# akashsengupta1997/STRAPS-3DHumanShapePose

Measured on AMD Instinct MI355X. Metric: bodies/sec, higher is better.
Workload: dtype fp32 (encoder convolutions as exact bf16x3 operand splits (six bf16 products per term); in-step SMPL blend contraction and skinning as 3-product fp16 splits (fp16x3_lbs: 22-bit operands); fp32 accumulate throughout)

## Files before the change

include/straps_hip.h:

```cpp
#ifndef STRAPS_HIP_H
#define STRAPS_HIP_H

#include <stddef.h>
#include <stdint.h>

#ifdef __cplusplus
extern "C" {
#endif

#define STRAPS_ABI_VERSION 12

#define STRAPS_OK 0
#define STRAPS_EINVAL 1
#define STRAPS_EHIP 2
#define STRAPS_EUNSUPPORTED 3

int straps_abi_version(void);
int straps_selftest_mfma_peak(const float* seed512, float* out, int blocks, int iters, void* stream);
int straps_selftest_mfma_bf16(float* out, unsigned long long* clk2, int blocks, int iters, void* stream);
int straps_selftest_mfma_bf16_dense(float* out, unsigned long long* clk2, int blocks, int iters, int data, void* stream);
const char* straps_last_error(void);
int straps_device_count(void);
int straps_wall_clock_khz(void);
int straps_set_clock_accumulator(unsigned long long* acc2);
// ... 85 lines not shown
#define STRAPS_SMPL_V 6890
#define STRAPS_SMPL_VPAD 6912
#define STRAPS_SMPL_TILES 216
#define STRAPS_SMPL_KP 224
#define STRAPS_SMPL_NJ 24
#define STRAPS_SMPL_NEXTRA 45
#define STRAPS_SMPL_NPICK 21
#define STRAPS_SMPL_NJOINTS_OUT 90

typedef struct {
    const float* blend_frag;
    const float* j_template;
    const float* j_shapedirs;
    const int32_t* parents;
    const int32_t* depth;
    int32_t max_depth;
    int32_t skin_k;
    const float* skin_w;
    const int32_t* skin_j;
    const int32_t* vj_ptr;
    int32_t n_tiles;
    int32_t reserved0;
    const int32_t* pick_ids;
    const float* blend_frag_t;
    const int32_t* children;
    const int32_t* jrt_ptr;
    const int32_t* jrt_code;
    const float* jrt_w;
    const int32_t* dj_ptr;
    const int32_t* dj_code;
    const float* dj_w;
    const void* blend_frag_h;
    float blend_h_unscale;
    int32_t reserved1;
    const void* skin_frag_p;
} straps_smpl_model_t;

#define STRAPS_SMPL_KERNEL_WIDE 0x100
#define STRAPS_SMPL_KERNEL_NARROW 0x200
#define STRAPS_SMPL_KERNEL_WIDE_BUILTIN 0x400
#define STRAPS_SMPL_EXACT_F32 0
#define STRAPS_SMPL_SPLIT_F16 1
#define STRAPS_SMPL_SPLIT_F16_LBS 2
#define STRAPS_SMPL_SPLIT_F16_LBS_PD16 3
#define STRAPS_SMPL_SPLIT_F16_LBS_P16 4

size_t straps_smpl_workspace_bytes(const straps_smpl_model_t* model, long long batch);
int straps_smpl_fwd(const straps_smpl_model_t* model, const float* betas, const float* rotmats,
                    float* verts, float* joints, void* workspace, long long batch, int chunks, int mode,
                    void* stream);

size_t straps_smpl_bwd_workspace_bytes(long long batch, int chunks);
int straps_smpl_bwd(const straps_smpl_model_t* model, const float* betas, const float* rotmats,
                    const float* dverts, const float* djoints, float* dbetas, float* drotmats,
                    void* workspace, long long batch, int chunks, void* stream);
int straps_smpl_bwd_aa(const straps_smpl_model_t* model, const float* betas, const float* rotmats,
                       const float* full_pose_aa, const float* dverts, const float* djoints, float* dbetas,
                       float* dfull_pose_aa, float* drotmats, void* workspace, long long batch, int chunks,
                       void* stream);

int straps_conv_dgrad(const float* dy_nhwc, const float* w_crsk, const float* addend,
                      float* dx_nhwc, int batch, int h, int w, int cin, int cout, int kh, int kw,
                      int stride, int pad, int tile_cfg, void* stream);

int straps_split3_bf16(const float* x, unsigned short* planes, long long n, long long plane_stride,
                       void* stream);
int straps_split3_bf16_cm(const float* x, unsigned short* planes, long long rows, int c,
                          long long plane_stride, void* stream);
int straps_conv_x3_stat_blocks(int batch, int h, int w, int cin, int cout, int kh, int kw, int stride,
                               int pad, int tile_cfg);

int straps_conv_x3f_supported(int cin, int cout, int kh, int kw, int stride, int pad);
int straps_conv_fwd_x3f(const float* x, const float* a_scale, const float* a_shift, int a_relu, const unsigned short* w3,
                        long long w_plane_stride, const float* scale, const float* shift, const float* residual, int relu,
                        float* y, float* stats_partial, int batch, int h, int w, int cin, int cout, int kh, int kw, int stride,
                        int pad, int tile_cfg, void* stream);
int straps_conv_x3f_stat_blocks(int batch, int h, int w, int cin, int cout, int kh, int kw, int stride, int pad, int tile_cfg);
int straps_conv_dgrad_x3f(const float* dy, const unsigned short* w3_crsk, long long w_plane_stride, const float* addend,
                          const unsigned* addend_bits, float* dx, int batch, int h, int w, int cin, int cout, int kh, int kw,
                          int stride, int pad, int tile_cfg, const float* bn_raw, const unsigned* bn_out_bits,
                          const float* bn_mask_scale, const float* bn_mask_shift, const float* bn_mean, const float* bn_invstd,
                          double* bn_partials, void* stream);
int straps_conv_dgrad_x3f_bn_blocks(int batch, int h, int w, int cin, int cout, int kh, int kw, int stride, int pad, int tile_cfg);
size_t straps_conv_wgrad_x3f_workspace_bytes(int batch, int h, int w, int cin, int cout, int kh, int kw, int stride, int pad);
int straps_conv_wgrad_x3f(const float* x, const float* a_scale, const float* a_shift, int a_relu, const float* dy, float* dw_oihw,
                          void* workspace, int batch, int h, int w, int cin, int cout, int kh, int kw, int stride, int pad,
                          int accumulate, void* stream);
int straps_conv_fwd_x3(const unsigned short* x3, long long x_plane_stride,
                       const unsigned short* w3_krsc, long long w_plane_stride, const float* scale,
                       const float* shift, const float* residual, int relu, float* y_nhwc,
                       float* stats_partial, int batch, int h, int w, int cin, int cout, int kh,
                       int kw, int stride, int pad, int tile_cfg, void* stream);
int straps_conv_fwd_x3p(const unsigned short* x3, long long x_plane_stride,
                        const unsigned short* w3_krsc, long long w_plane_stride, const float* scale,
                        const float* shift, const float* residual, int relu, float* y_nhwc,
                        unsigned short* y_planes, long long y_plane_stride, int batch, int h, int w,
                        int cin, int cout, int kh, int kw, int stride, int pad, int tile_cfg, void* stream);
int straps_split_bf16_cm(const float* x, unsigned short* plane, long long rows, int c, void* stream);
int straps_pack_conv_weight_bf16(const float* w_oihw, unsigned short* w_plane, int cout, int cin, int kh, int kw, void* stream);
int straps_conv_bf16_tile_choice(int batch, int h, int w, int cin, int cout, int kh, int kw, int stride, int pad);
int straps_conv_fwd_bf16(const unsigned short* x1, const unsigned short* w1_krsc, const float* scale, const float* shift,
                         const float* residual, int relu, float* y_nhwc, unsigned short* y_plane, int batch, int h, int w,
                         int cin, int cout, int kh, int kw, int stride, int pad, int tile_cfg, void* stream);
int straps_conv_dgrad_x3(const unsigned short* dy3, long long dy_plane_stride,
                         const unsigned short* w3_crsk, long long w_plane_stride,
                         const float* addend, float* dx_nhwc, int batch, int h, int w, int cin,
                         int cout, int kh, int kw, int stride, int pad, int tile_cfg, void* stream);
int straps_bn_apply_x3(const float* raw, const float* scale, const float* shift, const float* residual,
                       int relu, float* y, unsigned short* y_planes, long long plane_stride,
                       long long rows, int c, void* stream);
int straps_bn_relu_maxpool_fwd_x3(const float* raw, const float* scale, const float* shift,
                                  float* y_pool, uint8_t* idx, unsigned short* y_planes,
                                  long long plane_stride, int batch, int h, int w, int c, void* stream);
int straps_bn_bwd_x3(const float* dy, const float* yact, const float* raw, const float* save_mean,
                     const float* save_invstd, const float* gamma, const float* mask_scale,
                     const float* mask_shift, float* dgamma, float* dbeta, float* draw, float* dz_out,
                     unsigned short* draw_planes, long long plane_stride, void* workspace,
                     long long rows, int c, int accumulate, void* stream);
int straps_conv_dgrad_x3_bn_blocks(int batch, int h, int w, int cin, int cout, int kh, int kw, int stride,
                                   int pad, int tile_cfg);
int straps_conv_dgrad_x3_bn(const unsigned short* dy3, long long dy_plane_stride,
                            const unsigned short* w3_crsk, long long w_plane_stride, const float* addend,
                            float* dx_nhwc, int batch, int h, int w, int cin, int cout, int kh, int kw,
                            int stride, int pad, int tile_cfg, const float* bn_raw, const float* bn_out,
                            const float* bn_mask_scale, const float* bn_mask_shift, const float* bn_mean,
                            const float* bn_invstd, double* bn_partials, void* stream);
int straps_bn_bwd_finish_x3(const float* dy, const float* yact, const float* raw, const float* save_mean,
                            const float* save_invstd, const float* gamma, const float* mask_scale,
                            const float* mask_shift, float* dgamma, float* dbeta, float* draw, float* dz_out,
                            unsigned short* draw_planes, long long plane_stride, const double* partials,
                            int nblk, void* workspace, long long rows, int c, int accumulate, void* stream);
int straps_bn_apply_bits_x3(const float* raw, const float* scale, const float* shift, const float* residual, float* y,
                            unsigned short* y_planes, long long plane_stride, unsigned* relu_bits, long long rows,
                            int c, void* stream);
int straps_bn_bwd_bits_x3(const float* dy, const unsigned* relu_bits, const float* raw, const float* save_mean,
                          const float* save_invstd, const float* gamma, float* dgamma, float* dbeta, float* draw,
                          unsigned short* draw_planes, long long plane_stride, void* workspace, long long rows, int c,
                          int accumulate, void* stream);
int straps_bn_bwd_finish_bits_x3(const float* dy, const unsigned* relu_bits, const float* raw, const float* save_mean,
                                 const float* save_invstd, const float* gamma, float* dgamma, float* dbeta, float* draw,
                                 unsigned short* draw_planes, long long plane_stride, const double* partials, int nblk,
                                 void* workspace, long long rows, int c, int accumulate, void* stream);
int straps_conv_dgrad_x3_bits(const unsigned short* dy3, long long dy_plane_stride, const unsigned short* w3_crsk,
                              long long w_plane_stride, const float* addend, float* dx_nhwc, int batch, int h, int w,
                              int cin, int cout, int kh, int kw, int stride, int pad, int tile_cfg,
                              const unsigned* addend_bits, void* stream);
int straps_conv_dgrad_x3_bn_bits(const unsigned short* dy3, long long dy_plane_stride,
                                 const unsigned short* w3_crsk, long long w_plane_stride, const float* addend,
                                 float* dx_nhwc, int batch, int h, int w, int cin, int cout, int kh, int kw,
                                 int stride, int pad, int tile_cfg, const float* bn_raw, const float* bn_out,
                                 const float* bn_mask_scale, const float* bn_mask_shift, const float* bn_mean,
                                 const float* bn_invstd, double* bn_partials, const unsigned* addend_bits,
                                 const unsigned* bn_out_bits, void* stream);
int straps_conv_wgrad_x3_on_planes(int batch, int h, int w, int cin, int cout, int kh, int kw,
                                   int stride, int pad);
int straps_conv_wgrad_x3(const float* x_nhwc, const float* dy_nhwc, const unsigned short* x3,
                         long long x_plane_stride, const unsigned short* dy3, long long dy_plane_stride,
                         float* dw_oihw, void* workspace, int batch, int h, int w, int cin, int cout,
                         int kh, int kw, int stride, int pad, int accumulate, void* stream);


size_t straps_conv_wgrad_workspace_bytes(int batch, int h, int w, int cin, int cout, int kh,
                                         int kw, int stride, int pad);
int straps_conv_wgrad(const float* x_nhwc, const float* dy_nhwc, float* dw_oihw, void* workspace,
                      int batch, int h, int w, int cin, int cout, int kh, int kw, int stride,
                      int pad, int accumulate, void* stream);
size_t straps_stem_wgrad_workspace_bytes(int batch, int cin, int h, int w);
int straps_stem_wgrad(const float* x_nchw, const float* dy_nhwc, float* dw_oihw, void* workspace,
                      const uint32_t* nzmask , int batch, int cin,
                      int h, int w, int accumulate, void* stream);
#define STRAPS_STEM_DGRAD_MAX_CIN 64
size_t straps_stem_dgrad_weight_floats(int cin);
int straps_pack_stem_dgrad_weight(const float* w_oihw, float* w_pk, int cin, void* stream);
int straps_stem_dgrad(const float* dy_nhwc, const float* w_pk, float* dx_nchw, int batch, int cin, int h, int w,
                      int accumulate, void* stream);
int straps_bn_bwd_blocks(long long rows, int c);
size_t straps_bn_bwd_workspace_bytes(long long rows, int c);
int straps_bn_bwd(const float* dy, const float* yact, const float* raw, const float* save_mean,
                  const float* save_invstd, const float* gamma, const float* mask_scale,
                  const float* mask_shift, float* dgamma, float* dbeta, float* draw, float* dz_out,
                  void* workspace, long long rows, int c, int accumulate, void* stream);
int straps_bn_relu_maxpool_fwd(const float* raw_nhwc, const float* scale, const float* shift,
                               float* y_pool_nhwc, uint8_t* idx, int batch, int h, int w, int c,
                               void* stream);
int straps_bn_bwd_pooled(const float* dy_pool_nhwc, const uint8_t* idx, const float* raw,
                         const float* save_mean, const float* save_invstd, const float* gamma,
                         const float* mask_scale, const float* mask_shift, float* dgamma, float* dbeta,
                         float* draw, void* workspace, int batch, int h, int w, int c, int accumulate,
                         void* stream);
size_t straps_stem_tiles(int batch, int in_h, int in_w);
int straps_stem_tile_activity(const uint32_t* nzmask, uint8_t* tile_active, int batch, int cin, int in_h,
                              int in_w, void* stream);
int straps_bn_bwd_pooled_sparse(const float* dy_pool_nhwc, const uint8_t* idx, const float* raw,
                                const float* save_mean, const float* save_invstd, const float* gamma,
                                const float* mask_scale, const float* mask_shift, float* dgamma,
                                float* dbeta, float* draw, void* workspace, int batch, int h, int w, int c,
                                int accumulate, const uint8_t* tile_active, void* stream);
int straps_maxpool_fwd_idx(const float* x_nhwc, float* y_nhwc, uint8_t* idx, int batch, int h,
                           int w, int c, void* stream);
int straps_maxpool_bwd(const float* dy_nhwc, const uint8_t* idx, float* dx_nhwc, int batch, int h,
                       int w, int c, void* stream);
int straps_gap_bwd(const float* dfeat, float* dx_nhwc, int batch, int hw, int c, void* stream);
int straps_masked_copy(const float* x, int ldx, const float* mask, int ldmask, float* y, int ldy,
                       int m, int n, int accumulate, void* stream);
int straps_rot6d_bwd(const float* x6, long long ld, int per_row, const float* drot, float* dx6,
                     long long ldd, long long rows, void* stream);

int straps_build_proxy_input(const float* seg, const float* joints2d, float* out_nchw, int batch,
                             int nj, int wh, void* stream);
int straps_build_proxy_input_std(const float* seg, const float* joints2d, float* out_nchw, int batch,
                                 int nj, int wh, int std, void* stream);
int straps_build_proxy_input_nz(const float* seg, const float* joints2d, float* out_nchw, uint32_t* nzmask,
                                int batch, int nj, int wh, int std, void* stream);
size_t straps_loss_workspace_bytes(long long batch);
int straps_loss_fwd_bwd(const float* pred_verts, const float* pred_joints, const float* est,
                        int ld_est, const float* pred_rot, const float* tgt_verts,
                        const float* tgt_joints2d, const float* tgt_joints3d,
                        const float* tgt_shape, const float* tgt_rot, const float* log_vars,
                        float* loss_out, float* dverts, float* djoints, float* dest, float* drot,
                        float* dlogvar, void* workspace, long long batch, int img_wh, void* stream);
int straps_loss_fwd_bwd_gm(const float* pred_verts, const float* pred_joints, const float* est, int ld_est,
                           const float* pred_rot, const float* tgt_verts, const float* tgt_joints2d,
                           const float* tgt_joints3d, const float* tgt_shape, const float* tgt_rot,
                           const float* log_vars, float* loss_out, float* dverts, float* djoints, float* dest,
                           float* drot, float* dlogvar, void* workspace, long long batch, int img_wh,
                           const float* j2d_count_global, float count_scale, void* stream);
int straps_count_visible(const float* tgt_joints2d, float* out_count, long long batch, int nj, int img_wh,
                         void* stream);
int straps_mse_fwd(const float* pred, const float* tgt, const uint8_t* row_mask, long long rows,
                   int cols, float tgt_scale, float tgt_shift, float* out3, void* workspace,
                   void* stream);
int straps_mse_bwd(const float* pred, const float* tgt, const uint8_t* row_mask, long long rows,
                   int cols, float tgt_scale, float tgt_shift, const float* coef, float* grad,
                   void* stream);
int straps_augment_seg(const float* seg, const float* uniforms, const float* remove_prob,
                       float occlude_prob, int box_dim, float* out, int batch, int wh, void* stream);
int straps_philox_fill(unsigned long long seed, const long long* step_dev, long long step_host,
                       unsigned substream, float* out, long long n, int kind, void* stream);
int straps_counter_add(long long* counters, int n, long long delta, void* stream);
int straps_gather_f32(const float* src, const int* index, float* dst, int n, void* stream);
int straps_memset_zero(void* ptr, size_t bytes, void* stream);
int straps_augment_smpl(const float* pose_rows, long long n_rows, const float* u_index,
                        const float* orig_shape, const float* mean_shape, const float* shape_draws,
                        int shape_mode, const float* std_vector, double range_lo, double range_hi,
                        float* out_shape, float* out_rotmats, float* out_pose, long long batch,
                        void* stream);
int straps_augment_cam_t(const float* mean_cam_t, const float* normals_xy, const float* uniform_z,
                         double xy_std, double z_lo, double z_hi, float* out_cam_t, long long batch,
                         void* stream);
int straps_deviate_joints2d(const float* joints2d, const float* uniforms, double lo, double hi,
                            double hip_lo, double hip_hi, float* out, long long batch, void* stream);
int straps_deviate_verts2d(const float* verts, const float* uniforms, double lo, double hi, float* out,
                           long long nverts_total, void* stream);
int straps_project_targets(const float* joints, const float* cam_t, float fx, float fy, float cx,
                           float cy, float* joints2d, float* joints3d, long long batch, void* stream);
size_t straps_rasterize_workspace_bytes(long long batch, int nverts, int wh);
int straps_rasterize_parts(const float* verts, const int32_t* faces, const uint8_t* face_parts,
                           const float* cam_K, const float* cam_R, const float* cam_t, float* parts,
                           float* depth, void* workspace, long long batch, int nverts, int nfaces, int wh,
                           int cam_per_body, float near, float far, const float* vert_noise_u, double noise_lo,
                           double noise_hi, void* stream);
int straps_crop_resize(const float* seg, const float* joints2d, const float* uniforms,
                       double orig_scale_factor, double delta_scale_lo, double delta_scale_hi,
                       double delta_centre_lo, double delta_centre_hi, float* out_seg,
                       float* out_joints2d, int* boxes, int batch, int wh, int out_wh, int nj,
                       void* stream);
int straps_point_metrics(const float* pred, const float* target, float* out3, long long batch,
                         int npoints, void* stream);
int straps_adam_step(float* params, const float* grads, float* exp_avg, float* exp_avg_sq,
                     long long n, int step, float lr, float beta1, float beta2, float eps,
                     float grad_scale, const long long* step_dev, void* stream);

typedef struct {
    int layers;
    int in_channels;
    int ief_iters;
    int precision;
} straps_regressor_desc_t;
size_t straps_regressor_param_floats(const straps_regressor_desc_t* desc);
size_t straps_regressor_prepared_bytes(const straps_regressor_desc_t* desc);
int straps_regressor_prepare(const straps_regressor_desc_t* desc, const float* params, void* prepared, void* stream);
size_t straps_regressor_workspace_bytes(const straps_regressor_desc_t* desc, int batch, int h, int w);
int straps_regressor_fwd_infer(const straps_regressor_desc_t* desc, const void* prepared, const float* x, int batch, int h, int w,
                               float* est, int ld_est, float* rotmats, void* workspace, size_t workspace_bytes, void* stream);

size_t straps_regressor_train_param_floats(const straps_regressor_desc_t* desc);
size_t straps_regressor_bn_state_floats(const straps_regressor_desc_t* desc);
size_t straps_regressor_train_workspace_bytes(const straps_regressor_desc_t* desc, int batch, int h, int w);
int straps_regressor_fwd_train(const straps_regressor_desc_t* desc, const float* params, float* bn_state, const float* init_est,
                               const float* x, int batch, int h, int w, float* est, int ld_est,
                               void* workspace, size_t workspace_bytes, void* stream);
int straps_regressor_bwd(const straps_regressor_desc_t* desc, const float* params, const float* x, int batch, int h, int w,
                         const float* dest, int ld_dest, float* grads, float* dx,
                         void* workspace, size_t workspace_bytes, void* stream);
int straps_regressor_export_infer_params(const straps_regressor_desc_t* desc, const float* params, const float* bn_state,
                                         const float* init_est, float* infer_params, void* stream);

#define STRAPS_COMM_ID_BYTES 128
int straps_comm_unique_id(void* id128);
int straps_comm_init_rank(const void* id128, int nranks, int rank, void** comm);
int straps_comm_destroy(void* comm);
int straps_comm_size(void* comm);
const char* straps_comm_library(void);
int straps_allreduce_grads(float* flat_g, long long n, void* comm, void* stream);

#ifdef __cplusplus
// ... 4 lines not shown
```

straps-3dhumanshapepose_amd/autograd_ops.py:

```python
import ctypes as C

import torch

from . import hipabi
from .encoder_exec import encoder_forward
from .ief_module import EST_LD


def _empty_like(t):
    return torch.empty_like(t, memory_format=torch.contiguous_format)


class GradSink(dict):

    def __init__(self, views=None):
        super().__init__()
        self.views = views

    def buf(self, p, zero=False):
        if self.views is not None and p in self.views:
            return self.views[p]
        return torch.zeros_like(p) if zero else torch.empty_like(p)


class _SideStream:

    def __init__(self, stream):
        self.s, self.keep = stream, []

    def run(self, fn, *tensors):
        if self.s is None:
            return fn()
        self.keep.extend(tensors)
        self.s.wait_stream(torch.cuda.current_stream())
        with torch.cuda.stream(self.s):
            return fn()

    def join(self):
        if self.s is not None:
            torch.cuda.current_stream().wait_stream(self.s)
            self.keep.clear()


_FUSE_BN_SUMS = True
_SPARSE_STEM_TAIL = True


def _packed_dgrad_weight(net, conv):
    w = conv.weight

    def make():
        wd = w.detach().contiguous()
        out = torch.empty(wd.numel(), device=wd.device, dtype=torch.float32)
        hipabi.check(hipabi.lib().straps_pack_conv_weight_dgrad(hipabi.ptr(wd), hipabi.ptr(out), wd.shape[0], wd.shape[1], wd.shape[2],
                                                                wd.shape[3], hipabi.stream_ptr()), 'straps_pack_conv_weight_dgrad')
        return out
    return net._cached(('wd', id(conv)), [w], make)


def _bn_bwd(L, rec, dy, masked, want_dz, grads, planes_sink=None, keep_fp32=True, mask_bits=None):
    bn = rec['bn']
    raw, ss = rec['raw'], rec['stats']
    rows, Cc = raw.numel() // raw.shape[-1], raw.shape[-1]
    ws = torch.empty(L.straps_bn_bwd_workspace_bytes(rows, Cc) // 4, device=raw.device, dtype=torch.float32)
    dgamma, dbeta = grads.buf(bn.weight), grads.buf(bn.bias)
    keep_fp32 = keep_fp32 or planes_sink is None
    draw = _empty_like(raw) if keep_fp32 else raw.new_empty(0)
    dz = _empty_like(raw) if want_dz else None
    from_raw = masked and rec.get('residual') is None
    bits = mask_bits if mask_bits is not None else (rec.get('bits') if masked and not from_raw else None)
    if bits is not None and want_dz:
        raise RuntimeError('BatchNorm backward on ReLU bits writes no masked gradient (dz)')
    planes, ps = None, 0
    if planes_sink is not None:
        ps = (raw.numel() + 7) // 8 * 8
        planes = torch.empty(3, ps, device=raw.device, dtype=torch.int16)
        planes_sink[id(draw)] = (draw, planes, ps)
    flags = 2 if rec.get('frozen') else 0
    fused = rec.pop('bwd_partials', None)
    if bits is not None:
        args = (hipabi.ptr(dy), hipabi.ptr(bits), hipabi.ptr(raw), hipabi.ptr(ss[2]), hipabi.ptr(ss[3]), hipabi.ptr(bn.weight), hipabi.ptr(dgamma),
                hipabi.ptr(dbeta), hipabi.ptr(draw if keep_fp32 else None), hipabi.ptr(planes), ps)
        if fused is not None and fused[2] is dy and masked:
            hipabi.check(L.straps_bn_bwd_finish_bits_x3(*args, hipabi.ptr(fused[0]), fused[1], hipabi.ptr(ws), rows, Cc, flags, hipabi.stream_ptr()),
                         'straps_bn_bwd_finish_bits_x3')
        else:
            hipabi.check(L.straps_bn_bwd_bits_x3(*args, hipabi.ptr(ws), rows, Cc, flags, hipabi.stream_ptr()), 'straps_bn_bwd_bits_x3')
    elif fused is not None and fused[2] is dy and masked:
        hipabi.check(L.straps_bn_bwd_finish_x3(hipabi.ptr(dy), hipabi.ptr(rec['out'] if not from_raw else None), hipabi.ptr(raw), hipabi.ptr(ss[2]),
                                               hipabi.ptr(ss[3]), hipabi.ptr(bn.weight), hipabi.ptr(ss[0] if from_raw else None),
                                               hipabi.ptr(ss[1] if from_raw else None), hipabi.ptr(dgamma), hipabi.ptr(dbeta),
                                               hipabi.ptr(draw if keep_fp32 else None), hipabi.ptr(dz), hipabi.ptr(planes), ps, hipabi.ptr(fused[0]),
                                               fused[1], hipabi.ptr(ws), rows, Cc, flags, hipabi.stream_ptr()), 'straps_bn_bwd_finish_x3')
    else:
        hipabi.check(L.straps_bn_bwd_x3(hipabi.ptr(dy), hipabi.ptr(rec['out'] if masked and not from_raw else None), hipabi.ptr(raw), hipabi.ptr(ss[2]),
                                        hipabi.ptr(ss[3]), hipabi.ptr(bn.weight), hipabi.ptr(ss[0] if from_raw else None),
                                        hipabi.ptr(ss[1] if from_raw else None), hipabi.ptr(dgamma), hipabi.ptr(dbeta), hipabi.ptr(draw if keep_fp32 else None),
                                        hipabi.ptr(dz), hipabi.ptr(planes), ps, hipabi.ptr(ws), rows, Cc, flags, hipabi.stream_ptr()), 'straps_bn_bwd')
    grads[bn.weight] = dgamma
    grads[bn.bias] = dbeta
    return draw, dz


def _conv_wgrad(L, rec, draw, grads, planes_sink=None):
    conv = rec['conv']
    B, H, W, Cin, Cout, k, stride, pad, Ho, Wo = rec['geom']
    dw = grads.buf(conv.weight)
    if rec.get('fmode'):
        a_bn = rec.get('a_bn')
        wsf = torch.empty(max(L.straps_conv_wgrad_x3f_workspace_bytes(B, H, W, Cin, Cout, k, k, stride, pad) // 4, 1), device=draw.device, dtype=torch.float32)
        hipabi.check(L.straps_conv_wgrad_x3f(hipabi.ptr(rec['x']), hipabi.ptr(a_bn[0] if a_bn is not None else None), hipabi.ptr(a_bn[1] if a_bn is not None else None),
                                             int(a_bn is not None), hipabi.ptr(draw), hipabi.ptr(dw), hipabi.ptr(wsf), B, H, W, Cin, Cout, k, k, stride, pad, 0,
                                             hipabi.stream_ptr()), 'straps_conv_wgrad_x3f')
        grads[conv.weight] = dw
        return
    ws = torch.empty(L.straps_conv_wgrad_workspace_bytes(B, H, W, Cin, Cout, k, k, stride, pad) // 4, device=draw.device, dtype=torch.float32)
    fp = lambda t: hipabi.ptr(t if t is not None and t.numel() else None)
    xh = rec.get('x3')
    gh = planes_sink.get(id(draw)) if planes_sink is not None else None
    if xh is not None and gh is not None and xh[0] is rec['x'] and gh[0] is draw:
        hipabi.check(L.straps_conv_wgrad_x3(fp(rec['x']), fp(draw), hipabi.ptr(xh[1]), xh[2], hipabi.ptr(gh[1]), gh[2], hipabi.ptr(dw),
                                            hipabi.ptr(ws), B, H, W, Cin, Cout, k, k, stride, pad, 0, hipabi.stream_ptr()), 'straps_conv_wgrad_x3')
    else:
        hipabi.check(L.straps_conv_wgrad(hipabi.ptr(rec['x']), hipabi.ptr(draw), hipabi.ptr(dw), hipabi.ptr(ws), B, H, W, Cin, Cout, k, k, stride,
                                         pad, 0, hipabi.stream_ptr()), 'straps_conv_wgrad')
    grads[conv.weight] = dw


def _conv_dgrad(L, net, rec, draw, addend, planes_sink=None, bn_next=None, addend_bits=None):
    conv = rec['conv']
    B, H, W, Cin, Cout, k, stride, pad, Ho, Wo = rec['geom']
    dx = torch.empty(B, H, W, Cin, device=draw.device, dtype=torch.float32)
    if rec.get('fmode'):
        if not draw.numel():
            raise RuntimeError('fp32-operand data gradient: the fp32 gradient was not materialised')
        w3, wps = net._packed_weight_x3(conv, dgrad=True)
        raw = nbits = msc = msh = mean = invstd = part = None
        if bn_next is not None and _FUSE_BN_SUMS:
            ssn = bn_next['stats']
            from_raw = bn_next.get('residual') is None
            nbits = None if from_raw else bn_next.get('bits')
            if from_raw or nbits is not None:
                nblk = L.straps_conv_dgrad_x3f_bn_blocks(B, H, W, Cin, Cout, k, k, stride, pad, 0)
                part = torch.empty(nblk, Cin, 2, device=dx.device, dtype=torch.float64)
                raw, mean, invstd = bn_next['raw'], ssn[2], ssn[3]
                if from_raw:
                    msc, msh = ssn[0], ssn[1]
        if bn_next is None or not _FUSE_BN_SUMS or part is not None:
            hipabi.check(L.straps_conv_dgrad_x3f(hipabi.ptr(draw), hipabi.ptr(w3), wps, hipabi.ptr(addend), hipabi.ptr(addend_bits), hipabi.ptr(dx), B, H, W, Cin, Cout,
                                                 k, k, stride, pad, 0, hipabi.ptr(raw), hipabi.ptr(nbits), hipabi.ptr(msc), hipabi.ptr(msh), hipabi.ptr(mean),
                                                 hipabi.ptr(invstd), hipabi.ptr(part), hipabi.stream_ptr()), 'straps_conv_dgrad_x3f')
            if part is not None:
                bn_next['bwd_partials'] = (part, nblk, dx)
            return dx
    if getattr(net, 'conv_precision', 'fp32') == 'bf16x3':
        if not draw.numel() and (planes_sink is None or planes_sink.get(id(draw)) is None):
            raise RuntimeError('data gradient: neither the fp32 gradient nor its planes exist')
        hit = planes_sink.get(id(draw)) if planes_sink is not None else None
        if hit is not None and hit[0] is draw:
            g3, gps = hit[1], hit[2]
        else:
            from .encoder_exec import split3
            g3, gps = split3(L, draw)
        w3, wps = net._packed_weight_x3(conv, dgrad=True)
        if bn_next is not None and _FUSE_BN_SUMS:
            ssn = bn_next['stats']
            from_raw = bn_next.get('residual') is None
            nblk = L.straps_conv_dgrad_x3_bn_blocks(B, H, W, Cin, Cout, k, k, stride, pad, 0)
            part = torch.empty(nblk, Cin, 2, device=dx.device, dtype=torch.float64)
            nbits = None if from_raw else bn_next.get('bits')
            if addend_bits is not None or nbits is not None:
                hipabi.check(L.straps_conv_dgrad_x3_bn_bits(hipabi.ptr(g3), gps, hipabi.ptr(w3), wps, hipabi.ptr(addend), hipabi.ptr(dx), B, H, W, Cin,
                                                            Cout, k, k, stride, pad, 0, hipabi.ptr(bn_next['raw']),
                                                            hipabi.ptr(None if from_raw or nbits is not None else bn_next['out']),
                                                            hipabi.ptr(ssn[0] if from_raw else None), hipabi.ptr(ssn[1] if from_raw else None),
                                                            hipabi.ptr(ssn[2]), hipabi.ptr(ssn[3]), hipabi.ptr(part), hipabi.ptr(addend_bits),
                                                            hipabi.ptr(nbits), hipabi.stream_ptr()), 'straps_conv_dgrad_x3_bn_bits')
                bn_next['bwd_partials'] = (part, nblk, dx)
                return dx
            hipabi.check(L.straps_conv_dgrad_x3_bn(hipabi.ptr(g3), gps, hipabi.ptr(w3), wps, hipabi.ptr(addend), hipabi.ptr(dx), B, H, W, Cin, Cout,
                                                   k, k, stride, pad, 0, hipabi.ptr(bn_next['raw']), hipabi.ptr(None if from_raw else bn_next['out']),
                                                   hipabi.ptr(ssn[0] if from_raw else None), hipabi.ptr(ssn[1] if from_raw else None),
                                                   hipabi.ptr(ssn[2]), hipabi.ptr(ssn[3]), hipabi.ptr(part), hipabi.stream_ptr()),
                         'straps_conv_dgrad_x3_bn')
            bn_next['bwd_partials'] = (part, nblk, dx)
            return dx
        if addend_bits is not None:
            hipabi.check(L.straps_conv_dgrad_x3_bits(hipabi.ptr(g3), gps, hipabi.ptr(w3), wps, hipabi.ptr(addend), hipabi.ptr(dx), B, H, W, Cin, Cout,
                                                     k, k, stride, pad, 0, hipabi.ptr(addend_bits), hipabi.stream_ptr()), 'straps_conv_dgrad_x3_bits')
            return dx
        hipabi.check(L.straps_conv_dgrad_x3(hipabi.ptr(g3), gps, hipabi.ptr(w3), wps, hipabi.ptr(addend), hipabi.ptr(dx), B, H, W, Cin, Cout,
                                            k, k, stride, pad, 0, hipabi.stream_ptr()), 'straps_conv_dgrad_x3')
        return dx
    if addend_bits is not None:
        raise RuntimeError('ReLU bits exist only on the bf16x3 route')
    hipabi.check(L.straps_conv_dgrad(hipabi.ptr(draw), hipabi.ptr(_packed_dgrad_weight(net, conv)), hipabi.ptr(addend), hipabi.ptr(dx), B, H, W,
                                     Cin, Cout, k, k, stride, pad, 0, hipabi.stream_ptr()), 'straps_conv_dgrad')
    return dx


def encoder_backward(net, tape, dfeat, views=None, side_stream=None, after_layer3=None, want_dx=False, param_grads=True):
    L = hipabi.lib()
    grads = GradSink(views)
    side = _SideStream(side_stream)
    sink = {} if getattr(net, 'conv_precision', 'fp32') == 'bf16x3' else None

    def sink_of(rec):
        return None if rec.get('fmode') else sink

    def keep(rec):
        if sink is None or rec.get('x3') is None:
            return True
        B, H, W, Cin, Cout, k, stride, pad, Ho, Wo = rec['geom']
        return not L.straps_conv_wgrad_x3_on_planes(B, H, W, Cin, Cout, k, k, stride, pad)
    rec = tape['gap']
    B, HW, Cf = rec['geom']
    dy = _empty_like(rec['x'])
    hipabi.check(L.straps_gap_bwd(hipabi.ptr(dfeat.contiguous()), hipabi.ptr(dy), B, HW, Cf, hipabi.stream_ptr()), 'straps_gap_bwd')
    units = [u for li in range(1, 5) for u in getattr(net, 'layer%d' % li)]
    for li in range(4, 0, -1):
        for unit in reversed(list(getattr(net, 'layer%d' % li))):
            pairs = unit.conv_bn_pairs()
            ui = units.index(unit)
            prev_last = tape[id(units[ui - 1].conv_bn_pairs()[-1][0])] if ui > 0 else None
            rec = tape[id(pairs[-1][0])]
            ubits = rec.get('bits') if sink is not None else None
            dskip_bits = None
            if ubits is not None:
                draw, _ = _bn_bwd(L, rec, dy, True, False, grads, sink_of(rec), keep(rec))
                dz = dy
            else:
                draw, dz = _bn_bwd(L, rec, dy, True, True, grads, sink_of(rec), keep(rec))
            if param_grads:
                side.run(lambda rec=rec, draw=draw: _conv_wgrad(L, rec, draw, grads, sink), draw)
            if unit.downsample is not None:
                recd = tape[id(unit.downsample[0])]
                drawd, _ = _bn_bwd(L, recd, dz, False, False, grads, sink_of(recd), keep(recd), mask_bits=ubits)
                if param_grads:
                    side.run(lambda recd=recd, drawd=drawd: _conv_wgrad(L, recd, drawd, grads, sink), drawd)
                dskip = _conv_dgrad(L, net, recd, drawd, None, sink)
            else:
                dskip, dskip_bits = dz, ubits
            for ci in range(len(pairs) - 1, 0, -1):
                rec_prev = tape[id(pairs[ci - 1][0])]
                dt = _conv_dgrad(L, net, tape[id(pairs[ci][0])], draw, None, sink, bn_next=rec_prev if sink is not None else None)
                rec = rec_prev
                draw, _ = _bn_bwd(L, rec, dt, True, False, grads, sink_of(rec), keep(rec))
                if param_grads:
                    side.run(lambda rec=rec, draw=draw: _conv_wgrad(L, rec, draw, grads, sink), draw)
            dy = _conv_dgrad(L, net, tape[id(pairs[0][0])], draw, dskip, sink, bn_next=prev_last if sink is not None else None,
                             addend_bits=dskip_bits)
        if li == 3 and after_layer3 is not None:
            side.join()
            after_layer3()
    rec = tape['maxpool']
    B, H, W, Cc, Hp, Wp = rec['geom']
    if rec['kind'] == 'maxpool_fused':
        idx = rec['idx']
        rec = tape['stem']
        bn, raw, ss = rec['bn'], rec['raw'], rec['stats']
        ws = torch.empty(L.straps_bn_bwd_workspace_bytes(B * H * W, Cc) // 4, device=raw.device, dtype=torch.float32)
        dgamma, dbeta = grads.buf(bn.weight), grads.buf(bn.bias)
        draw = _empty_like(raw)
        tact = None
        if rec.get('nzmask') is not None and _SPARSE_STEM_TAIL and not want_dx:
            _, Cin0, Hin, Win = rec['geom'][:4]
            tact = torch.empty(L.straps_stem_tiles(B, Hin, Win), device=raw.device, dtype=torch.uint8)
            hipabi.check(L.straps_stem_tile_activity(hipabi.ptr(rec['nzmask']), hipabi.ptr(tact), B, Cin0, Hin, Win, hipabi.stream_ptr()),
                         'straps_stem_tile_activity')
        hipabi.check(L.straps_bn_bwd_pooled_sparse(hipabi.ptr(dy), hipabi.ptr(idx), hipabi.ptr(raw), hipabi.ptr(ss[2]), hipabi.ptr(ss[3]),
                                                   hipabi.ptr(bn.weight), hipabi.ptr(ss[0]), hipabi.ptr(ss[1]), hipabi.ptr(dgamma), hipabi.ptr(dbeta),
                                                   hipabi.ptr(draw), hipabi.ptr(ws), B, H, W, Cc, 2 if rec.get('frozen') else 0, hipabi.ptr(tact),
                                                   hipabi.stream_ptr()), 'straps_bn_bwd_pooled_sparse')
        grads[bn.weight] = dgamma
        grads[bn.bias] = dbeta
    else:
        dstem = _empty_like(rec['x'])
        hipabi.check(L.straps_maxpool_bwd(hipabi.ptr(dy), hipabi.ptr(rec['idx']), hipabi.ptr(dstem), B, H, W, Cc, hipabi.stream_ptr()),
                     'straps_maxpool_bwd')
        rec = tape['stem']
        draw, _ = _bn_bwd(L, rec, dstem, True, False, grads)
    B, Cin, H, W, Ho, Wo = rec['geom']
    dx = None
    if want_dx:
        dx = torch.empty(B, Cin, H, W, device=draw.device, dtype=torch.float32)
        hipabi.check(L.straps_stem_dgrad(hipabi.ptr(draw), hipabi.ptr(net._packed_stem_dgrad_weight()), hipabi.ptr(dx), B, Cin, H, W, 0,
                                         hipabi.stream_ptr()), 'straps_stem_dgrad')
    if param_grads:
        ws = torch.empty(L.straps_stem_wgrad_workspace_bytes(B, Cin, H, W) // 4, device=draw.device, dtype=torch.float32)
        dw = grads.buf(net.conv1.weight)
        hipabi.check(L.straps_stem_wgrad(hipabi.ptr(rec['x']), hipabi.ptr(draw), hipabi.ptr(dw), hipabi.ptr(ws), hipabi.ptr(rec.get('nzmask')),
                                         B, Cin, H, W, 0, hipabi.stream_ptr()), 'straps_stem_wgrad')
        grads[net.conv1.weight] = dw
    side.join()
    return (grads, dx) if want_dx else grads


def ief_backward(ief, feat, tape, dest, views=None, param_grads=True):
    sink = GradSink(views)
    L, st = hipabi.lib(), hipabi.stream_ptr()
    pk = ief._packed(feat.device)
    B, F = feat.shape
    H1, H2, P = ief.fc1.out_features, ief.fc2.out_features, ief.num_output_params
    dev = feat.device
    T = len(tape)
    e = lambda *s: torch.empty(*s, device=dev, dtype=torch.float32)
    D = hipabi.gemm_desc
    ests, h1s, h2s = tape[0]['stacks']
    assert ests.shape == (T + 1, B, EST_LD) and h1s.shape == (T, B, H1) and h2s.shape == (T, B, H2)
    dW3, db3 = sink.buf(ief.fc3.weight), sink.buf(ief.fc3.bias)
    dW2, db2 = sink.buf(ief.fc2.weight), sink.buf(ief.fc2.bias)
    dW1, db1 = sink.buf(ief.fc1.weight), sink.buf(ief.fc1.bias)
    dests = e(T + 1, B, EST_LD)
    dsrc = dest if dest.stride(-1) == 1 and dest.dim() == 2 else dest.contiguous()
    hipabi.check(L.straps_masked_copy(hipabi.ptr(dsrc), dsrc.stride(0), None, 0, hipabi.ptr(dests[T]), EST_LD, B, EST_LD, 0, st), 'ief dest slot')
    dh2s, dh1s, dc1 = e(T, B, H2), e(T, B, H1), e(B, H1)
    w3, w2 = ief.fc3.weight, ief.fc2.weight
    for it in reversed(range(T)):
        hipabi.gemm_multi([D(dests[it + 1], EST_LD, 1, w3, H2, 1, dh2s[it], H2, B, H2, P, mask=h2s[it], ldmask=H2)])
        hipabi.gemm_multi([D(dh2s[it], H2, 1, w2, H1, 1, dh1s[it], H1, B, H1, H2, mask=h1s[it], ldmask=H1,
                             c2=dc1, ldc2=H1, accumulate2=int(it != T - 1))])
        hipabi.gemm_multi([D(dh1s[it], H1, 1, pk['w1e'], EST_LD, 1, dests[it], EST_LD, B, P, H1, addend=dests[it + 1], ldadd=EST_LD)])
    one = pk['one']
    dfeat = e(B, F)
    if not param_grads:
        hipabi.gemm_multi([D(dc1, H1, 1, pk['w1f'], F, 1, dfeat, F, B, F, H1)])
        return dfeat, {}
    KB = T * B
    hipabi.gemm_multi([
        D(dh2s, 1, H2, h1s, H1, 1, dW2, H1, H2, H1, KB),
        D(dc1, 1, H1, feat, F, 1, dW1, F + P, H1, F, B),
        D(dh1s, 1, H1, ests, EST_LD, 1, dW1.data_ptr() + 4 * F, F + P, H1, P, KB),
        D(dests[1], 1, EST_LD, h2s, H2, 1, dW3, H2, P, H2, KB),
        D(dc1, H1, 1, pk['w1f'], F, 1, dfeat, F, B, F, H1),
        D(one, 0, 0, dh2s, H2, 1, db2, H2, 1, H2, KB),
        D(one, 0, 0, dests[1], EST_LD, 1, db3, P, 1, P, KB),
        D(one, 0, 0, dc1, H1, 1, db1, H1, 1, H1, B)])
    grads = {ief.fc1.weight: dW1, ief.fc1.bias: db1, ief.fc2.weight: dW2, ief.fc2.bias: db2, ief.fc3.weight: dW3, ief.fc3.bias: db3}
    return dfeat, grads


class _RegressorFn(torch.autograd.Function):

    @staticmethod
    def forward(ctx, reg, x, *params):
        enc_tape, ief_tape = {}, []
        with torch.no_grad():
            feat = encoder_forward(reg.image_encoder, x, enc_tape)
            est = reg.ief_module.forward_estimate(feat, ief_tape)
        ctx.reg, ctx.feat, ctx.enc_tape, ctx.ief_tape, ctx.params = reg, feat, enc_tape, ief_tape, params
        return est

    @staticmethod
    def backward(ctx, dest):
        reg = ctx.reg
        want_dx, pg = ctx.needs_input_grad[1], any(ctx.needs_input_grad[2:])
        dfeat, g_ief = ief_backward(reg.ief_module, ctx.feat, ctx.ief_tape, dest, param_grads=pg)
        g_enc = encoder_backward(reg.image_encoder, ctx.enc_tape, dfeat, want_dx=want_dx, param_grads=pg)
        g_enc, dx = g_enc if want_dx else (g_enc, None)
        g_enc.update(g_ief)
        out = [g_enc.get(p) if need else None for p, need in zip(ctx.params, ctx.needs_input_grad[2:])]
        ctx.enc_tape = ctx.ief_tape = None
        return (None, dx) + tuple(out)


def regressor_autograd(reg, x):
    hipabi.require_gpu_tensor(x, 'regressor input', torch.float32)
    params = list(reg.parameters())
    est = _RegressorFn.apply(reg, x, *params)
    P = reg.ief_module.num_output_params
    return est[:, :3], est[:, 3:3 + 24 * 6], est[:, 3 + 24 * 6:P]


class _EncoderFn(torch.autograd.Function):

    @staticmethod
    def forward(ctx, net, x, *params):
        tape = {}
        with torch.no_grad():
            feat = encoder_forward(net, x, tape)
        ctx.net, ctx.tape, ctx.params = net, tape, params
        return feat

    @staticmethod
    def backward(ctx, dfeat):
        want_dx = ctx.needs_input_grad[1]
        g = encoder_backward(ctx.net, ctx.tape, dfeat, want_dx=want_dx, param_grads=any(ctx.needs_input_grad[2:]))
        g, dx = g if want_dx else (g, None)
        ctx.tape = None
        return (None, dx) + tuple(g.get(p) if need else None for p, need in zip(ctx.params, ctx.needs_input_grad[2:]))


def encoder_autograd(net, x):
    hipabi.require_gpu_tensor(x, 'encoder input', torch.float32)
    return _EncoderFn.apply(net, x, *list(net.parameters()))


class _IefFn(torch.autograd.Function):
    @staticmethod
    def forward(ctx, ief, feat, *params):
        tape = []
        with torch.no_grad():
            est = ief.forward_estimate(feat, tape)
        ctx.ief, ctx.feat, ctx.tape, ctx.params = ief, feat.detach().contiguous(), tape, params
# ... 119 lines not shown
```

straps-3dhumanshapepose_amd/csrc/conv_igemm.h:

```cpp
#pragma once
#include "common.h"
#include <type_traits>
#include <utility>

namespace {

struct ConvP {
    const float* x;
    const float* w;
    const float* scale;
    const float* shift;
    const float* res;
    float* y;
    float* stats;
    int H, W, Cin, Cout, relu;
    int stride;
    int OH, OW, omul;
    int NT, wtaps;
    long long xps, wps;
    int xrows, yrows;
    const float* bnr_raw;
    const float* bnr_out;
    const float* bnr_sc;
    const float* bnr_sh;
    const float* bnr_mean;
    const float* bnr_invstd;
    double* bnr_part;
    const unsigned* bnr_bits;
    const unsigned* res_bits;
    int bnr_base[4];
    unsigned short* yplanes;
    long long yps;
    const float* a_scale;
    const float* a_shift;
    int a_relu;
    int abl;
    unsigned long long* clk;
    int epi;
    struct Class {
        int Mh, Mw;
        int M, MT;
        int oah, oaw;
        int ntaps;
        int tap_w[9], tap_dh[9], tap_dw[9];
    } cls[4];
    int ncls;
};

struct ClkSample { unsigned long long c0, w0; };
__device__ __forceinline__ void clk_begin(const ConvP& p, ClkSample& s) {
    s.c0 = 0; s.w0 = 0;
    if (p.clk) { s.c0 = __builtin_amdgcn_s_memtime(); s.w0 = __builtin_amdgcn_s_memrealtime(); }
}
__device__ __forceinline__ void clk_end(const ConvP& p, const ClkSample& s) {
    if (p.clk && blockIdx.x == 0 && blockIdx.y == 0 && threadIdx.x == 0) {
        atomicAdd(p.clk, (unsigned long long)__builtin_amdgcn_s_memtime() - s.c0);
        atomicAdd(p.clk + 1, (unsigned long long)__builtin_amdgcn_s_memrealtime() - s.w0);
    }
}

__device__ __forceinline__ void epi_lds_barrier() {
    asm volatile("s_waitcnt lgkmcnt(0)" ::: "memory");
    __builtin_amdgcn_s_barrier();
    asm volatile("" ::: "memory");
}

template <int BM, int BN, int WGM, int WGN, bool BNR, int NYPL = 3>
__device__ __forceinline__ void igemm_store_rows_impl(const ConvP& p, const ConvP::Class& c, const f32x16 (&acc)[BM / WGM / 32][BN / WGN / 32], int m0,
                                                      int n0, float (&s1)[BN / WGN / 32], float (&s2)[BN / WGN / 32], double (&d1)[BN / WGN / 32],
                                                      double (&d2)[BN / WGN / 32]) {
    constexpr int WTM = BM / WGM, WTN = BN / WGN, MI = WTM / 32, NI = WTN / 32;
    const int tid = threadIdx.x, lane = tid & 63, wave = tid >> 6;
    const int wm = wave / WGN, wn = wave % WGN;
    const int cMh = c.Mh, cMw = c.Mw, cM = c.M, coah = c.oah, coaw = c.oaw;
    const int MhMw = cMh * cMw;
    const bool remap = p.omul != 1 || coah != 0 || coaw != 0 || p.OH != cMh || p.OW != cMw;
    float sc[NI], sh[NI];
#pragma unroll
    for (int j = 0; j < NI; ++j) {
        const int n = n0 + wn * WTN + j * 32 + (lane & 31);
        sc[j] = p.scale ? p.scale[n] : 1.f;
        sh[j] = p.shift ? p.shift[n] : 0.f;
        s1[j] = 0.f;
        s2[j] = 0.f;
    }
    [[maybe_unused]] float bsc[NI], bsh[NI], bmu[NI];
    [[maybe_unused]] const bool bnr = BNR && p.bnr_raw != nullptr;
    if constexpr (BNR) {
        if (bnr) {
#pragma unroll
            for (int j = 0; j < NI; ++j) {
                const int n = n0 + wn * WTN + j * 32 + (lane & 31);
                bsc[j] = (p.bnr_out || p.bnr_bits) ? 0.f : p.bnr_sc[n];
                bsh[j] = (p.bnr_out || p.bnr_bits) ? 0.f : p.bnr_sh[n];
                bmu[j] = p.bnr_mean[n];
                d1[j] = 0.0;
                d2[j] = 0.0;
            }
        }
    }
    const bool full = m0 + BM <= cM;
    auto rows = [&](auto full_c) {
        constexpr bool FULL = decltype(full_c)::value;
#pragma unroll
        for (int i = 0; i < MI; ++i) {
            const int mb = m0 + wm * WTM + i * 32 + 4 * (lane >> 5);
            int b_ = 0, ho_ = 0, wo_ = 0;
            if (remap) {
                b_ = mb / MhMw;
                const int rem = mb - b_ * MhMw;
                ho_ = rem / cMw;
                wo_ = rem - ho_ * cMw;
            }
            int pixr[16];
#pragma unroll
            for (int r = 0; r < 16; ++r) {
                pixr[r] = mb + (r & 3) + 8 * (r >> 2);
                if (remap) {
                    pixr[r] = (b_ * p.OH + ho_ * p.omul + coah) * p.OW + wo_ * p.omul + coaw;
                    wo_ += (r & 3) == 3 ? 5 : 1;
                    while (wo_ >= cMw) {
                        wo_ -= cMw;
                        if (++ho_ == cMh) { ho_ = 0; ++b_; }
                    }
                }
            }
            float rv[16][NI];
            if (p.res) {
#pragma unroll
                for (int r = 0; r < 16; ++r)
#pragma unroll
                    for (int j = 0; j < NI; ++j) {
                        const int m = mb + (r & 3) + 8 * (r >> 2);
                        rv[r][j] = (FULL || m < cM) ? p.res[pixr[r] * p.Cout + n0 + wn * WTN + j * 32 + (lane & 31)] : 0.f;
                    }
                if (p.res_bits) {
#pragma unroll
                    for (int r = 0; r < 16; ++r)
#pragma unroll
                        for (int j = 0; j < NI; ++j) {
                            const int m = mb + (r & 3) + 8 * (r >> 2);
                            const unsigned wd = (FULL || m < cM) ? p.res_bits[pixr[r] * (p.Cout >> 5) + ((n0 + wn * WTN + j * 32) >> 5)] : 0u;
                            rv[r][j] = ((wd >> (lane & 31)) & 1u) ? rv[r][j] : 0.f;
                        }
                }
            }
#pragma unroll
            for (int hb = 0; hb < 2; ++hb) {
                [[maybe_unused]] float xr[8][NI], yo[8][NI];
                if constexpr (BNR) {
                    if (bnr) {
#pragma unroll
                        for (int q = 0; q < 8; ++q)
#pragma unroll
                            for (int j = 0; j < NI; ++j) {
                                const int r = hb * 8 + q;
                                const int m = mb + (r & 3) + 8 * (r >> 2);
                                const int o = pixr[r] * p.Cout + n0 + wn * WTN + j * 32 + (lane & 31);
                                xr[q][j] = (FULL || m < cM) ? p.bnr_raw[o] : 0.f;
                                if (p.bnr_bits)
                                    yo[q][j] = (FULL || m < cM) ? __uint_as_float(p.bnr_bits[pixr[r] * (p.Cout >> 5) + ((n0 + wn * WTN + j * 32) >> 5)]) : 0.f;
                                else
                                    yo[q][j] = (p.bnr_out && (FULL || m < cM)) ? p.bnr_out[o] : 0.f;
                            }
                    }
                }
#pragma unroll
                for (int q = 0; q < 8; ++q) {
                    const int r = hb * 8 + q;
                    const int m = mb + (r & 3) + 8 * (r >> 2);
                    if (FULL || m < cM) {
#pragma unroll
                        for (int j = 0; j < NI; ++j) {
                            const int o = pixr[r] * p.Cout + n0 + wn * WTN + j * 32 + (lane & 31);
                            float v = acc[i][j][r];
                            s1[j] += v;
                            s2[j] = fmaf(v, v, s2[j]);
                            if (p.scale) v = fmaf(v, sc[j], sh[j]);
                            if (p.res) v += rv[r][j];
                            if (p.relu) v = fmaxf(v, 0.f);
                            if (!BNR || p.y) p.y[o] = v;
                            if constexpr (BNR) {
                                if (p.yplanes) {
                                    if constexpr (NYPL == 1) {
                                        p.yplanes[cm_index(pixr[r], n0 + wn * WTN + j * 32 + (lane & 31), p.yrows)] = bf16_rn(v);
                                    } else {
                                    u16 b1, b2, b3;
                                    split3(v, b1, b2, b3);
                                    const long long oc = cm_index(pixr[r], n0 + wn * WTN + j * 32 + (lane & 31), p.yrows);
                                    p.yplanes[oc] = b1;
                                    p.yplanes[p.yps + oc] = b2;
                                    p.yplanes[2 * p.yps + oc] = b3;
                                    }
                                }
                                if (bnr) {
                                    const bool on = p.bnr_bits ? (((__float_as_uint(yo[q][j]) >> (lane & 31)) & 1u) != 0)
                                                               : (p.bnr_out ? yo[q][j] > 0.f : fmaf(xr[q][j], bsc[j], bsh[j]) > 0.f);
                                    const float g = on ? v : 0.f;
                                    d1[j] += (double)g;
// ... 260 lines not shown
        d2[j] = 0.0;
    }
    auto pixel = [&](int m) {
        m = m < M ? m : M - 1;
        if (!remap) return m;
        const int MhMw = c.Mh * c.Mw;
        const int b_ = m / MhMw, rem = m - b_ * MhMw;
        const int ho_ = rem / c.Mw, wo_ = rem - ho_ * c.Mw;
        return (b_ * p.OH + ho_ * p.omul + c.oah) * p.OW + wo_ * p.omul + c.oaw;
    };
#pragma unroll
    for (int g = 0; g < NU / UG; ++g) {
        float rv[UG][16], xr[UG][16];
        unsigned aw[UG], ow[UG];
        int po[UG][16];
#pragma unroll
        for (int u = 0; u < UG; ++u) {
            const int i = (g * UG + u) / NI, j = (g * UG + u) % NI;
            const int mrow = m0 + wm * WTM + i * 32;
            aw[u] = 0xffffffffu; ow[u] = 0xffffffffu;
            {
                const long long wi = (long long)pixel(mrow + (lane & 31)) * CW + ((cb + j * 32) >> 5);
                if (has_abits) aw[u] = p.res_bits[wi];
                if (has_obits) ow[u] = p.bnr_bits[wi];
            }
            const int coff = cb + j * 32 + (lane & 31);
            if (!remap && full) {
#pragma unroll
                for (int r = 0; r < 16; ++r) po[u][r] = (mrow + (r & 3) + 8 * (r >> 2) + half4) * Cout + coff;
            } else {
#pragma unroll
                for (int r = 0; r < 16; ++r) po[u][r] = pixel(mrow + (r & 3) + 8 * (r >> 2) + half4) * Cout + coff;
            }
#pragma unroll
            for (int r = 0; r < 16; ++r) {
                rv[u][r] = has_add ? p.res[po[u][r]] : 0.f;
                xr[u][r] = bnr ? p.bnr_raw[po[u][r]] : 0.f;
            }
        }
#pragma unroll
        for (int u = 0; u < UG; ++u) {
            const int i = (g * UG + u) / NI, j = (g * UG + u) % NI;
            const int mrow = m0 + wm * WTM + i * 32;
            float sg = 0.f, sgx = 0.f;
#pragma unroll
            for (int r = 0; r < 16; ++r) {
                const int rr = (r & 3) + 8 * (r >> 2);
                const unsigned long long am = (unsigned long long)(unsigned)__builtin_amdgcn_readlane((int)aw[u], rr) |
                                              ((unsigned long long)(unsigned)__builtin_amdgcn_readlane((int)aw[u], rr + 4) << 32);
                const float v = acc[i][j][r] + lane_masked(rv[u][r], am);
                const bool ok = full || mrow + rr + half4 < M;
                if (bnr) {
                    float gq;
                    if (has_obits) {
                        const unsigned long long om = (unsigned long long)(unsigned)__builtin_amdgcn_readlane((int)ow[u], rr) |
                                                      ((unsigned long long)(unsigned)__builtin_amdgcn_readlane((int)ow[u], rr + 4) << 32);
                        gq = lane_masked(v, om);
                    } else {
                        gq = fmaf(xr[u][r], bsc[j], bsh[j]) > 0.f ? v : 0.f;
                    }
                    if (!ok) gq = 0.f;
                    sg += gq;
                    sgx = fmaf(gq, xr[u][r] - bmu[j], sgx);
                }
                if (ok) p.y[po[u][r]] = v;
            }
            d1[j] += (double)sg;
            d2[j] += (double)sgx;
        }
    }
}

template <int BM, int BN, int WGM, int WGN, bool PRESUM = false>
struct LeanDgradEpilogue {
    static constexpr int WTM = BM / WGM, WTN = BN / WGN, MI = WTM / 32, NI = WTN / 32, NU = MI * NI, DEPTH = NU > 1 ? 2 : 1;
    static constexpr int PF = (WGM * WGN >= 8 && NU > 2) ? 1 : DEPTH;
    struct Unit { float rv[16], xr[16]; unsigned aw, ow; };
    Unit u[DEPTH];
    int m0, n0, lane, wm, wn, M, Cout, half4, cb;
    bool full, remap, has_add, has_abits, bnr, has_obits, pre;
    const float *g_res, *g_raw;
    const unsigned *g_abits, *g_obits;
    float* g_y;
    int cMh, cMw, OH, OW, omul, oah, oaw;

    __device__ __forceinline__ void init(const ConvP& p, const ConvP::Class& c, int m0_, int n0_) {
        const int wave = threadIdx.x >> 6;
        m0 = m0_; n0 = n0_; lane = threadIdx.x & 63;
        wm = __builtin_amdgcn_readfirstlane(wave / WGN); wn = __builtin_amdgcn_readfirstlane(wave % WGN);
        M = c.M; Cout = p.Cout; half4 = 4 * (lane >> 5); cb = n0 + wn * WTN;
        full = m0 + BM <= M;
        remap = p.omul != 1 || c.oah != 0 || c.oaw != 0 || p.OH != c.Mh || p.OW != c.Mw;
        has_add = p.res != nullptr; has_abits = p.res_bits != nullptr; bnr = p.bnr_raw != nullptr; has_obits = p.bnr_bits != nullptr;
        g_res = p.res; g_raw = p.bnr_raw; g_abits = p.res_bits; g_obits = p.bnr_bits; g_y = p.y;
        cMh = c.Mh; cMw = c.Mw; OH = p.OH; OW = p.OW; omul = p.omul; oah = c.oah; oaw = c.oaw;
        pre = false;
    }
    __device__ __forceinline__ int pixel(int m) const {
        m = m < M ? m : M - 1;
        if (!remap) return m;
        const int MhMw = cMh * cMw;
        const int b_ = m / MhMw, rem = m - b_ * MhMw;
        const int ho_ = rem / cMw, wo_ = rem - ho_ * cMw;
        return (b_ * OH + ho_ * omul + oah) * OW + wo_ * omul + oaw;
    }
    __device__ __forceinline__ void issue(int k, Unit& un) const {
        const int i = k / NI, j = k % NI;
        const int mrow = m0 + wm * WTM + i * 32;
        un.aw = 0xffffffffu; un.ow = 0xffffffffu;
        {
            const long long wi = (long long)pixel(mrow + (lane & 31)) * (Cout >> 5) + ((cb + j * 32) >> 5);
            if (has_abits) un.aw = g_abits[wi];
            if (has_obits) un.ow = g_obits[wi];
        }
        const int coff = cb + j * 32 + (lane & 31);
        int pix[16];
        pixels(mrow, pix);
#pragma unroll
        for (int r = 0; r < 16; ++r) {
            un.rv[r] = has_add ? g_res[pix[r] * Cout + coff] : 0.f;
            un.xr[r] = bnr ? g_raw[pix[r] * Cout + coff] : 0.f;
        }
    }
    __device__ __forceinline__ void pixels(int mrow, int (&pix)[16]) const {
        const int mb = mrow + half4;
        if (!remap) {
#pragma unroll
            for (int r = 0; r < 16; ++r) { const int m = mb + (r & 3) + 8 * (r >> 2); pix[r] = (full || m < M) ? m : M - 1; }
        } else {
            const int MhMw = cMh * cMw;
            int mm = mb < M ? mb : M - 1;
            int b_ = mm / MhMw;
            const int rem = mm - b_ * MhMw;
            int ho_ = rem / cMw, wo_ = rem - ho_ * cMw;
            const int plast = full ? 0 : pixel(M - 1);
#pragma unroll
            for (int r = 0; r < 16; ++r) {
                pix[r] = (full || mb + (r & 3) + 8 * (r >> 2) < M) ? (b_ * OH + ho_ * omul + oah) * OW + wo_ * omul + oaw : plast;
                wo_ += (r & 3) == 3 ? 5 : 1;
                while (wo_ >= cMw) {
                    wo_ -= cMw;
                    if (++ho_ == cMh) { ho_ = 0; ++b_; }
                }
            }
        }
    }
    __device__ __forceinline__ void prefetch() {
        epi_static_for<PF>([&](auto kc) { issue(decltype(kc)::value, u[decltype(kc)::value]); });
        pre = true;
    }
    template <bool PRE = true>
    __device__ __forceinline__ void finish(const ConvP& p, const ConvP::Class&, const f32x16 (&acc)[MI][NI], float (&)[NI], float (&)[NI], double (&d1)[NI],
                                           double (&d2)[NI]) {
        float bmu[NI], bsc[NI], bsh[NI];
#pragma unroll
        for (int j = 0; j < NI; ++j) {
            const int n = cb + j * 32 + (lane & 31);
            bmu[j] = bnr ? p.bnr_mean[n] : 0.f;
            bsc[j] = (bnr && !has_obits) ? p.bnr_sc[n] : 0.f;
            bsh[j] = (bnr && !has_obits) ? p.bnr_sh[n] : 0.f;
            d1[j] = 0.0;
            d2[j] = 0.0;
        }
        if (!pre) epi_static_for<PF>([&](auto kc) { issue(decltype(kc)::value, u[decltype(kc)::value]); });
        epi_static_for<DEPTH - PF>([&](auto kc) { issue(decltype(kc)::value + PF, u[decltype(kc)::value + PF]); });
        epi_static_for<NU>([&](auto kc) {
            constexpr int k = decltype(kc)::value, i = k / NI, j = k % NI;
            Unit& un = u[k % DEPTH];
            const int mrow = m0 + wm * WTM + i * 32;
            const int coff = cb + j * 32 + (lane & 31);
            int pix[16];
            pixels(mrow, pix);
            float sg = 0.f, sgx = 0.f;
            epi_static_for<16>([&](auto rc) {
                constexpr int r = decltype(rc)::value, rr = (r & 3) + 8 * (r >> 2);
                const unsigned long long am = (unsigned long long)(unsigned)__builtin_amdgcn_readlane((int)un.aw, rr) |
                                              ((unsigned long long)(unsigned)__builtin_amdgcn_readlane((int)un.aw, rr + 4) << 32);
                const float v = acc[i][j][r] + lane_masked(un.rv[r], am);
                const bool ok = full || mrow + rr + half4 < M;
                if (bnr) {
                    float gq;
                    if (has_obits) {
                        const unsigned long long om = (unsigned long long)(unsigned)__builtin_amdgcn_readlane((int)un.ow, rr) |
                                                      ((unsigned long long)(unsigned)__builtin_amdgcn_readlane((int)un.ow, rr + 4) << 32);
                        gq = lane_masked(v, om);
                    } else {
                        gq = fmaf(un.xr[r], bsc[j], bsh[j]) > 0.f ? v : 0.f;
                    }
                    if (!ok) gq = 0.f;
                    if constexpr (PRESUM) {
                        sg += gq;
                        sgx = fmaf(gq, un.xr[r] - bmu[j], sgx);
                    } else {
                        d1[j] += (double)gq;
                        d2[j] += (double)gq * ((double)un.xr[r] - (double)bmu[j]);
                    }
                }
                if (ok) g_y[pix[r] * Cout + coff] = v;
            });
            if constexpr (PRESUM) { d1[j] += (double)sg; d2[j] += (double)sgx; }
            if constexpr (k + DEPTH < NU) issue(k + DEPTH, un);
        });
    }
};

inline int lean_epilogue_choice(const ConvP& p) {
    if (p.yplanes || p.bnr_out || !p.y || p.scale || p.relu) return 0;
    const ConvP::Class& c = p.cls[0];
    const bool remap = p.omul != 1 || c.oah != 0 || c.oaw != 0 || p.OH != c.Mh || p.OW != c.Mw;
    if (!p.res && !p.bnr_raw && !p.res_bits) return (p.ncls == 1 && !remap) ? 1 : 0;
    if (!p.stats && (p.res || p.bnr_raw) && (!p.res_bits || p.res)) {
        for (int i = 0; i < p.ncls; ++i)
            if (p.cls[i].ntaps == 0) return 0;
        return 2;
    }
    return 0;
}

template <int BM, int BN, int WGM, int WGN, int EPI>
struct X3Epilogue {
    __device__ __forceinline__ void init(const ConvP&, const ConvP::Class&, int, int) {}
    __device__ __forceinline__ void prefetch() {}
    template <bool PRE = true>
    __device__ __forceinline__ void finish(const ConvP&, const ConvP::Class&, const f32x16 (&)[BM / WGM / 32][BN / WGN / 32], float (&)[BN / WGN / 32],
                                           float (&)[BN / WGN / 32], double (&)[BN / WGN / 32], double (&)[BN / WGN / 32]) {}
};
template <int BM, int BN, int WGM, int WGN>
struct X3Epilogue<BM, BN, WGM, WGN, 0> : IgemmEpilogue<BM, BN, WGM, WGN> {};
template <int BM, int BN, int WGM, int WGN>
struct X3Epilogue<BM, BN, WGM, WGN, 2> : LeanDgradEpilogue<BM, BN, WGM, WGN, false> {};
template <int BM, int BN, int WGM, int WGN>
struct X3Epilogue<BM, BN, WGM, WGN, 3> : IgemmEpilogue<BM, BN, WGM, WGN> {
    template <bool PRE = true>
    __device__ __forceinline__ void finish(const ConvP& p, const ConvP::Class& c, const f32x16 (&acc)[BM / WGM / 32][BN / WGN / 32], float (&s1)[BN / WGN / 32],
                                           float (&s2)[BN / WGN / 32], double (&d1)[BN / WGN / 32], double (&d2)[BN / WGN / 32]) {
        if (!this->look) {
            igemm_store_rows_impl<BM, BN, WGM, WGN, true, 1>(p, c, acc, this->m0, this->n0, s1, s2, d1, d2);
            return;
        }
        this->template run<PRE>(acc, s1, s2, d1, d2);
    }
};

template <int BM, int BN, int WGM = 2, int WGN = 2>
__device__ __forceinline__ void igemm_store_rows(const ConvP& p, const ConvP::Class& c, const f32x16 (&acc)[BM / WGM / 32][BN / WGN / 32], int m0, int n0,
                                                 float (&s1)[BN / WGN / 32], float (&s2)[BN / WGN / 32]) {
    double d1[BN / WGN / 32], d2[BN / WGN / 32];
    igemm_store_rows_impl<BM, BN, WGM, WGN, false>(p, c, acc, m0, n0, s1, s2, d1, d2);
}

template <int BM, int BN, int WGM = 2, int WGN = 2>
__device__ __forceinline__ void igemm_store_bnr(const ConvP& p, const double (&bd1)[BN / WGN / 32], const double (&bd2)[BN / WGN / 32], int blk, int n0,
                                                float* smem) {
    constexpr int WTN = BN / WGN, NI = WTN / 32;
    const int tid = threadIdx.x, lane = tid & 63, wave = tid >> 6;
    const int wm = wave / WGN, wn = wave % WGN;
    if (!p.bnr_raw) return;
    epi_lds_barrier();
    double* red = reinterpret_cast<double*>(smem);
#pragma unroll
    for (int j = 0; j < NI; ++j) {
        const double u1 = bd1[j] + __shfl_xor(bd1[j], 32, 64);
        const double u2 = bd2[j] + __shfl_xor(bd2[j], 32, 64);
        if (lane < 32) {
            const int c = wn * WTN + j * 32 + lane;
            red[(wm * BN + c) * 2 + 0] = u1;
            red[(wm * BN + c) * 2 + 1] = u2;
        }
    }
    epi_lds_barrier();
    if (tid < BN) {
        double t1 = red[tid * 2 + 0], t2 = red[tid * 2 + 1];
#pragma unroll
        for (int w = 1; w < WGM; ++w) { t1 += red[(w * BN + tid) * 2 + 0]; t2 += red[(w * BN + tid) * 2 + 1]; }
        double* o = p.bnr_part + ((long long)blk * p.Cout + n0 + tid) * 2;
        o[0] = t1;
        o[1] = t2 * (double)p.bnr_invstd[n0 + tid];
    }
}

template <int BM, int BN, int WGM = 2, int WGN = 2>
__device__ __forceinline__ void igemm_store_stats(const ConvP& p, const float (&s1)[BN / WGN / 32], const float (&s2)[BN / WGN / 32], int mt, int n0, float* smem) {
    constexpr int WTN = BN / WGN, NI = WTN / 32;
    const int tid = threadIdx.x, lane = tid & 63, wave = tid >> 6;
    const int wm = wave / WGN, wn = wave % WGN;
    if (p.stats) {
        epi_lds_barrier();
        float* red = smem;
#pragma unroll
        for (int j = 0; j < NI; ++j) {
            const float u1 = s1[j] + __shfl_xor(s1[j], 32, 64);
            const float u2 = s2[j] + __shfl_xor(s2[j], 32, 64);
            if (lane < 32) {
                const int c = wn * WTN + j * 32 + lane;
                red[(wm * BN + c) * 2 + 0] = u1;
                red[(wm * BN + c) * 2 + 1] = u2;
            }
        }
        epi_lds_barrier();
        if (tid < BN) {
            float* o = p.stats + ((long long)mt * p.Cout + n0 + tid) * 2;
            float t1 = red[tid * 2 + 0], t2 = red[tid * 2 + 1];
#pragma unroll
            for (int w = 1; w < WGM; ++w) { t1 += red[(w * BN + tid) * 2 + 0]; t2 += red[(w * BN + tid) * 2 + 1]; }
            o[0] = t1;
            o[1] = t2;
        }
    }
}

inline int conv_fwd_problem(ConvP& p, const float* scale, const float* shift, const float* residual, int relu, float* y, float* stats_partial,
                            int batch, int h, int wdt, int cin, int cout, int kh, int kw, int stride, int pad) {
    p.scale = scale; p.shift = shift; p.res = residual; p.y = y; p.stats = stats_partial;
    p.bnr_raw = p.bnr_out = p.bnr_sc = p.bnr_sh = p.bnr_mean = p.bnr_invstd = nullptr; p.bnr_part = nullptr; p.bnr_bits = p.res_bits = nullptr;
    p.yplanes = nullptr; p.yps = 0; p.clk = straps_clk_acc_current(); p.epi = STRAPS_TOOL_ENV_INT("STRAPS_EPI", 1);
    p.a_scale = p.a_shift = nullptr; p.a_relu = 0; p.abl = 0;
    p.H = h; p.W = wdt; p.Cin = cin; p.Cout = cout; p.relu = relu; p.stride = stride;
    ConvP::Class& c = p.cls[0];
    p.ncls = 1;
    c.Mh = (h + 2 * pad - kh) / stride + 1;
    c.Mw = (wdt + 2 * pad - kw) / stride + 1;
    p.OH = c.Mh; p.OW = c.Mw; p.omul = 1; c.oah = 0; c.oaw = 0;
    c.ntaps = p.wtaps = kh * kw;
    for (int r = 0; r < kh; ++r)
        for (int s = 0; s < kw; ++s) { c.tap_w[r * kw + s] = r * kw + s; c.tap_dh[r * kw + s] = r - pad; c.tap_dw[r * kw + s] = s - pad; }
    const long long M = (long long)batch * c.Mh * c.Mw;
    STRAPS_REQUIRE(M < (1LL << 31) && (long long)batch * h * wdt * cin < (1LL << 31) && M * cout < (1LL << 31),
                   "straps_conv_fwd: tensors must stay below 2^31 elements (32-bit offsets)");
    c.M = (int)M;
    p.xrows = batch * h * wdt;
    p.yrows = (int)M;
    return STRAPS_OK;
}

inline int conv_dgrad_problem(ConvP& p, const float* addend, float* dx, int batch, int h, int wdt, int cin, int cout, int kh, int kw,
                              int stride, int pad) {
    const int ho = (h + 2 * pad - kh) / stride + 1, wo = (wdt + 2 * pad - kw) / stride + 1;
    const int padh = kh - 1 - pad, padw = kw - 1 - pad;
    p.scale = nullptr; p.shift = nullptr; p.res = addend; p.y = dx; p.stats = nullptr;
    p.bnr_raw = p.bnr_out = p.bnr_sc = p.bnr_sh = p.bnr_mean = p.bnr_invstd = nullptr; p.bnr_part = nullptr; p.bnr_bits = p.res_bits = nullptr;
    p.yplanes = nullptr; p.yps = 0; p.clk = straps_clk_acc_current(); p.epi = STRAPS_TOOL_ENV_INT("STRAPS_EPI", 1);
    p.a_scale = p.a_shift = nullptr; p.a_relu = 0; p.abl = 0;
    p.H = ho; p.W = wo; p.Cin = cout; p.Cout = cin; p.relu = 0; p.stride = 1;
    p.OH = h; p.OW = wdt; p.wtaps = kh * kw;
    p.omul = stride;
    p.xrows = batch * ho * wo;
    p.yrows = batch * h * wdt;
    p.ncls = 0;
    for (int ph = 0; ph < stride; ++ph) {
        for (int pw = 0; pw < stride; ++pw) {
            ConvP::Class& c = p.cls[p.ncls];
            c.Mh = (h - ph + stride - 1) / stride;
            c.Mw = (wdt - pw + stride - 1) / stride;
            if (c.Mh <= 0 || c.Mw <= 0) continue;
            c.oah = ph; c.oaw = pw;
            c.ntaps = 0;
            for (int r = 0; r < kh; ++r) {
                const int nh = ph - padh + r;
                if (((nh % stride) + stride) % stride) continue;
                for (int s = 0; s < kw; ++s) {
                    const int nw = pw - padw + s;
                    if (((nw % stride) + stride) % stride) continue;
                    c.tap_w[c.ntaps] = r * kw + s;
                    c.tap_dh[c.ntaps] = (nh - (((nh % stride) + stride) % stride)) / stride;
                    c.tap_dw[c.ntaps] = (nw - (((nw % stride) + stride) % stride)) / stride;
                    if (nh < 0) c.tap_dh[c.ntaps] = -((-nh) / stride);
                    if (nw < 0) c.tap_dw[c.ntaps] = -((-nw) / stride);
                    ++c.ntaps;
                }
            }
            const long long M = (long long)batch * c.Mh * c.Mw;
            STRAPS_REQUIRE(M < (1LL << 31) && (long long)batch * ho * wo * cout < (1LL << 31) && (long long)batch * h * wdt * cin < (1LL << 31),
                           "straps_conv_dgrad: tensors must stay below 2^31 elements (32-bit offsets)");
            c.M = (int)M;
            ++p.ncls;
        }
    }
    for (int a = 1; a < p.ncls; ++a)
        for (int b = a; b > 0 && (long long)p.cls[b].ntaps * p.cls[b].M > (long long)p.cls[b - 1].ntaps * p.cls[b - 1].M; --b) {
            const ConvP::Class t = p.cls[b];
            p.cls[b] = p.cls[b - 1];
            p.cls[b - 1] = t;
        }
    return STRAPS_OK;
}

}
```

straps-3dhumanshapepose_amd/csrc/conv_x3.hip:

```cpp
#include "conv_x3_kernels.h"

int straps_internal_dispatch_x3_lean(const void* p, int halo, int cfg, int epi, hipStream_t st);

namespace {

inline int pick_tile_x3(int cfg, long long M, int cout, int kdim, int& bm, int& bn, int ncls = 1, bool one_tap = false) {
    (void)kdim;
    cfg &= 15;
    if (cfg == 6) cfg = 4;
    if (cfg == 0) {
        const long long t128 = ((M + 127) / 128) * (cout / 128);
        if (cout % 128 != 0) cfg = 11;
        else if (t128 / ncls < STRAPS_TOOL_ENV_INT("STRAPS_X3_SMALL_T128", 128)) cfg = 3;
        else if (ncls > 1) cfg = t128 / ncls >= 512 ? 12 : t128 / ncls >= 256 ? (one_tap ? 9 : 12) : 11;
        else cfg = t128 >= 512 ? 12 : t128 >= 256 ? 5 : 7;
        {
            const int f = STRAPS_TOOL_ENV_INT("STRAPS_X3_RULE_CFG", 0);
            if (f > 0 && cout % 128 == 0 && t128 / ncls >= 128) cfg = f;
            const int lo = STRAPS_TOOL_ENV_INT("STRAPS_X3_LOW_CFG", 0);
            if (lo > 0 && ncls == 1 && cout % 128 == 0 && t128 >= 128 && t128 < 256) cfg = lo;
        }
    }
    if (cout % 128 != 0 && cfg != 3 && cfg != 7 && cfg != 10 && cfg != 11) cfg = 2;
    bm = (cfg == 4 || cfg == 6 || cfg == 12) ? 256 : cfg == 3 ? 64 : 128;
    bn = (cfg == 2 || cfg == 3 || cfg == 7 || cfg == 10 || cfg == 11) ? 64 : 128;
    return cfg;
}

inline int halo_choice(const ConvP& p, int tile_cfg) {
    if ((tile_cfg & 15) != 0 || (tile_cfg & 256)) return 0;
    const int slots = halo_patch_slots(p);
    const bool all = (tile_cfg & 512) != 0;
    const long long t128 = (long long)(p.cls[0].M / 128) * (p.Cout / 128);
    if (slots > 0 && p.Cout % 128 != 0 && slots <= 272 && (!all || (tile_cfg & 1024))) return 3;
    if (slots > 0 && p.Cout % 128 == 0 && slots <= 208 && (all || (t128 >= 256 && t128 < 512))) return 1;
    if (slots > 0 && p.Cout % 128 != 0 && slots <= 272 && all) return 2;
    return 0;
}

template <int ABL>
int dispatch_x3_abl(const ConvP& p, int cfg, hipStream_t st) {
    switch (cfg) {
        case 1: return launch_x3<128, 128, 4, 2, 3, ABL>(p, st);
        case 2: return launch_x3<128, 64, 2, 2, 2, ABL>(p, st);
        case 3: return launch_x3<64, 64, 2, 2, 3, ABL>(p, st);
        case 4: return launch_x3<256, 128, 4, 2, 2, ABL>(p, st);
        case 5: return launch_x3<128, 128, 2, 2, 3, ABL>(p, st);
        case 8: return launch_x3<128, 128, 2, 2, 3, 0, true>(p, st);
        case 9: return launch_x3<128, 128, 4, 2, 3, 0, true>(p, st);
        case 10: return launch_x3<128, 64, 2, 2, 3, 0, true>(p, st);
        case 11: return launch_x3<128, 64, 2, 2, 2, 0, true>(p, st);
        case 12: return launch_x3<256, 128, 4, 2, 2, 0, true>(p, st);
        default: return launch_x3<128, 64, 2, 2, 3, ABL>(p, st);
    }
}

int dispatch_x3(const ConvP& p, int tile_cfg, hipStream_t st) {
    int bm, bn, kdim = 0;
    long long M = 0;
    for (int i = 0; i < p.ncls; ++i) {
        M += p.cls[i].M;
        if (p.cls[i].ntaps * p.Cin > kdim) kdim = p.cls[i].ntaps * p.Cin;
    }
    const int halo = halo_choice(p, tile_cfg);
    if ((tile_cfg & 15) == 0 && !(tile_cfg & (64 | 128)) && STRAPS_TOOL_ENV_INT("STRAPS_X3_LEAN", 1)) {
        int epi = lean_epilogue_choice(p);
        if (epi == 2 && !STRAPS_TOOL_ENV_INT("STRAPS_X3_LEAN_DGRAD", 1)) epi = 0;
        if (epi) {
            const int cfg = halo ? 0 : pick_tile_x3(tile_cfg, M, p.Cout, kdim, bm, bn, p.ncls, kdim == p.Cin);
            if (halo == 1 || halo == 3 || (!halo && (cfg == 3 || cfg == 5 || cfg == 7 || cfg == 9 || cfg == 11 || cfg == 12)))
                return straps_internal_dispatch_x3_lean(&p, halo, cfg, epi, st);
        }
    }
    if (halo == 1) return launch_x3h<128, 128, 2, 2, 3, 208>(p, st);
    if (halo == 2) return launch_x3h<128, 64, 2, 2, 3, 272>(p, st);
    if (halo == 3) return launch_x3h<128, 64, 2, 2, 2, 272, 1>(p, st);
    const int cfg = pick_tile_x3(tile_cfg, M, p.Cout, kdim, bm, bn, p.ncls, kdim == p.Cin);
#ifdef STRAPS_TOOLS
    if ((tile_cfg & 192) == 192) return dispatch_x3_abl<3>(p, cfg, st);
    if (tile_cfg & 64) return dispatch_x3_abl<1>(p, cfg, st);
    if (tile_cfg & 128) return dispatch_x3_abl<2>(p, cfg, st);
#endif
    return dispatch_x3_abl<0>(p, cfg, st);
}

__global__ __launch_bounds__(256) void split3_kernel(const float* __restrict__ x, u16* __restrict__ o, long long n, long long ps) {
    const long long i4 = ((long long)blockIdx.x * 256 + threadIdx.x) * 4;
    if (i4 + 3 < n) {
        store_planes4(o, ps, i4, *reinterpret_cast<const f32x4*>(x + i4));
    } else {
        for (long long i = i4; i < n; ++i) {
            u16 b1, b2, b3;
            split3(x[i], b1, b2, b3);
            o[i] = b1; o[ps + i] = b2; o[2 * ps + i] = b3;
        }
    }
}

__global__ __launch_bounds__(256) void split3_cm_kernel(const float* __restrict__ x, u16* __restrict__ o, long long rows, int C, long long ps) {
    const int C4 = C >> 2;
    const long long n4 = rows * C4;
    for (long long i = (long long)blockIdx.x * 256 + threadIdx.x; i < n4; i += (long long)gridDim.x * 256) {
        const long long r = i / C4;
        const int c4 = (int)(i - r * C4);
        store_planes4_cm(o, ps, r, c4 * 4, rows, *reinterpret_cast<const f32x4*>(x + i * 4));
    }
}

}

extern "C" int straps_split3_bf16_cm(const float* x, unsigned short* planes, long long rows, int c, long long plane_stride, void* stream) {
    STRAPS_REQUIRE(x && planes, "straps_split3_bf16_cm: null pointer");
    STRAPS_REQUIRE(rows > 0 && c > 0 && c % 32 == 0, "straps_split3_bf16_cm: need rows > 0 and c %% 32 == 0 (rows=%lld c=%d)", rows, c);
    STRAPS_REQUIRE(plane_stride >= rows * c && plane_stride % 8 == 0, "straps_split3_bf16_cm: plane_stride must be >= rows*c and a multiple of 8");
    STRAPS_REQUIRE((reinterpret_cast<uintptr_t>(x) & 15) == 0 && (reinterpret_cast<uintptr_t>(planes) & 15) == 0, "straps_split3_bf16_cm: pointers must be 16-byte aligned");
    const long long n4 = rows * (c >> 2);
    const long long g = (n4 + 255) / 256;
    hipLaunchKernelGGL(split3_cm_kernel, dim3((unsigned)(g > 16384 ? 16384 : g)), dim3(256), 0, (hipStream_t)stream, x, planes, rows, c, plane_stride);
    STRAPS_CHECK_LAUNCH("split3_cm_kernel");
    return STRAPS_OK;
}

extern "C" int straps_split3_bf16(const float* x, unsigned short* planes, long long n, long long plane_stride, void* stream) {
    STRAPS_REQUIRE(x && planes, "straps_split3_bf16: null pointer");
    STRAPS_REQUIRE(n >= 0 && plane_stride >= n && plane_stride % 8 == 0, "straps_split3_bf16: plane_stride must be >= n and a multiple of 8");
    if (n == 0) return STRAPS_OK;
    STRAPS_REQUIRE((reinterpret_cast<uintptr_t>(x) & 15) == 0 && (reinterpret_cast<uintptr_t>(planes) & 15) == 0, "straps_split3_bf16: pointers must be 16-byte aligned");
    hipLaunchKernelGGL(split3_kernel, dim3(cdiv(n, 1024)), dim3(256), 0, (hipStream_t)stream, x, planes, n, plane_stride);
    STRAPS_CHECK_LAUNCH("split3_kernel");
    return STRAPS_OK;
}

extern "C" int straps_conv_fwd_x3(const unsigned short* x3, long long x_plane_stride, const unsigned short* w3, long long w_plane_stride,
                                  const float* scale, const float* shift, const float* residual, int relu, float* y, float* stats_partial,
                                  int batch, int h, int wdt, int cin, int cout, int kh, int kw, int stride, int pad, int tile_cfg, void* stream) {
    STRAPS_REQUIRE(x3 && w3 && y, "straps_conv_fwd_x3: null pointer");
    STRAPS_REQUIRE(batch > 0 && h > 0 && wdt > 0, "straps_conv_fwd_x3: empty input %dx%dx%d", batch, h, wdt);
    STRAPS_REQUIRE(cin % 32 == 0 && cout % 64 == 0, "straps_conv_fwd_x3: need cin%%32==0 and cout%%64==0 (cin=%d cout=%d)", cin, cout);
    STRAPS_REQUIRE(kh >= 1 && kw >= 1 && kh * kw <= 9 && stride >= 1 && pad >= 0, "straps_conv_fwd_x3: bad filter geometry");
    STRAPS_REQUIRE((scale == nullptr) == (shift == nullptr), "straps_conv_fwd_x3: scale and shift must be given together");
    STRAPS_REQUIRE(x_plane_stride % 8 == 0 && w_plane_stride % 8 == 0, "straps_conv_fwd_x3: plane strides must be multiples of 8 elements");
    ConvP p;
    p.x = reinterpret_cast<const float*>(x3); p.w = reinterpret_cast<const float*>(w3);
    p.xps = x_plane_stride; p.wps = w_plane_stride;
    const int rc = conv_fwd_problem(p, scale, shift, residual, relu, y, stats_partial, batch, h, wdt, cin, cout, kh, kw, stride, pad);
    if (rc != STRAPS_OK) return rc;
    return dispatch_x3(p, tile_cfg, (hipStream_t)stream);
}

extern "C" int straps_conv_fwd_x3p(const unsigned short* x3, long long x_plane_stride, const unsigned short* w3, long long w_plane_stride,
                                   const float* scale, const float* shift, const float* residual, int relu, float* y, unsigned short* y_planes,
                                   long long y_plane_stride, int batch, int h, int wdt, int cin, int cout, int kh, int kw, int stride, int pad,
                                   int tile_cfg, void* stream) {
    STRAPS_REQUIRE(x3 && w3 && y_planes, "straps_conv_fwd_x3p: null pointer");
    STRAPS_REQUIRE(batch > 0 && h > 0 && wdt > 0, "straps_conv_fwd_x3p: empty input %dx%dx%d", batch, h, wdt);
    STRAPS_REQUIRE(cin % 32 == 0 && cout % 64 == 0, "straps_conv_fwd_x3p: need cin%%32==0 and cout%%64==0 (cin=%d cout=%d)", cin, cout);
    STRAPS_REQUIRE(kh >= 1 && kw >= 1 && kh * kw <= 9 && stride >= 1 && pad >= 0, "straps_conv_fwd_x3p: bad filter geometry");
    STRAPS_REQUIRE((scale == nullptr) == (shift == nullptr), "straps_conv_fwd_x3p: scale and shift must be given together");
    STRAPS_REQUIRE(x_plane_stride % 8 == 0 && w_plane_stride % 8 == 0 && y_plane_stride % 8 == 0, "straps_conv_fwd_x3p: plane strides must be multiples of 8 elements");
    ConvP p;
    p.x = reinterpret_cast<const float*>(x3); p.w = reinterpret_cast<const float*>(w3);
    p.xps = x_plane_stride; p.wps = w_plane_stride;
    const int rc = conv_fwd_problem(p, scale, shift, residual, relu, y, nullptr, batch, h, wdt, cin, cout, kh, kw, stride, pad);
    if (rc != STRAPS_OK) return rc;
    STRAPS_REQUIRE(y_plane_stride >= (long long)p.cls[0].M * cout, "straps_conv_fwd_x3p: y_plane_stride smaller than the output");
    p.yplanes = y_planes; p.yps = y_plane_stride;
    return dispatch_x3(p, tile_cfg, (hipStream_t)stream);
}

static int conv_dgrad_x3_impl(const unsigned short* dy3, long long dy_plane_stride, const unsigned short* w3_crsk, long long w_plane_stride,
                              const float* addend, const unsigned* addend_bits, float* dx, int batch, int h, int wdt, int cin, int cout, int kh, int kw,
                              int stride, int pad, int tile_cfg, void* stream) {
    STRAPS_REQUIRE(dy3 && w3_crsk && dx, "straps_conv_dgrad_x3: null pointer");
    STRAPS_REQUIRE(!addend_bits || (addend && cin % 32 == 0), "straps_conv_dgrad_x3_bits: the ReLU bits mask an addend (and need cin %% 32 == 0)");
    STRAPS_REQUIRE(cout % 32 == 0 && cin % 64 == 0, "straps_conv_dgrad_x3: need cout%%32==0 and cin%%64==0 (cin=%d cout=%d)", cin, cout);
    STRAPS_REQUIRE(stride == 1 || stride == 2, "straps_conv_dgrad_x3: stride must be 1 or 2");
    STRAPS_REQUIRE(kh * kw <= 9 && kh - 1 - pad >= 0 && kw - 1 - pad >= 0, "straps_conv_dgrad_x3: unsupported filter geometry");
    STRAPS_REQUIRE(dy_plane_stride % 8 == 0 && w_plane_stride % 8 == 0, "straps_conv_dgrad_x3: plane strides must be multiples of 8 elements");
    ConvP p;
    p.x = reinterpret_cast<const float*>(dy3); p.w = reinterpret_cast<const float*>(w3_crsk);
    p.xps = dy_plane_stride; p.wps = w_plane_stride;
    const int rc = conv_dgrad_problem(p, addend, dx, batch, h, wdt, cin, cout, kh, kw, stride, pad);
    if (rc != STRAPS_OK) return rc;
    p.res_bits = addend_bits;
    return p.ncls ? dispatch_x3(p, tile_cfg, (hipStream_t)stream) : STRAPS_OK;
}

extern "C" int straps_conv_dgrad_x3(const unsigned short* dy3, long long dy_plane_stride, const unsigned short* w3_crsk, long long w_plane_stride,
                                    const float* addend, float* dx, int batch, int h, int wdt, int cin, int cout, int kh, int kw, int stride,
                                    int pad, int tile_cfg, void* stream) {
    return conv_dgrad_x3_impl(dy3, dy_plane_stride, w3_crsk, w_plane_stride, addend, nullptr, dx, batch, h, wdt, cin, cout, kh, kw, stride, pad, tile_cfg,
                              stream);
}

extern "C" int straps_conv_dgrad_x3_bits(const unsigned short* dy3, long long dy_plane_stride, const unsigned short* w3_crsk, long long w_plane_stride,
                                         const float* addend, float* dx, int batch, int h, int wdt, int cin, int cout, int kh, int kw, int stride,
                                         int pad, int tile_cfg, const unsigned* addend_bits, void* stream) {
    STRAPS_REQUIRE(addend_bits, "straps_conv_dgrad_x3_bits: null bit mask");
    return conv_dgrad_x3_impl(dy3, dy_plane_stride, w3_crsk, w_plane_stride, addend, addend_bits, dx, batch, h, wdt, cin, cout, kh, kw, stride, pad,
                              tile_cfg, stream);
}

static int dgrad_x3_blocks(const ConvP& p, int tile_cfg) {
    if (halo_choice(p, tile_cfg)) return p.cls[0].M / 128;
    int bm, bn, kdim = 0;
    long long M = 0;
    for (int i = 0; i < p.ncls; ++i) {
        M += p.cls[i].M;
        if (p.cls[i].ntaps * p.Cin > kdim) kdim = p.cls[i].ntaps * p.Cin;
    }
    pick_tile_x3(tile_cfg, M, p.Cout, kdim, bm, bn, p.ncls, kdim == p.Cin);
    int blocks = 0;
    for (int i = 0; i < p.ncls; ++i) blocks += (p.cls[i].M + bm - 1) / bm;
    return blocks;
}

extern "C" int straps_conv_dgrad_x3_bn_blocks(int batch, int h, int w, int cin, int cout, int kh, int kw, int stride, int pad, int tile_cfg) {
    ConvP p;
    p.x = nullptr; p.w = nullptr; p.xps = p.wps = 0;
    if (!(stride == 1 || stride == 2) || kh * kw > 9 || kh - 1 - pad < 0 || kw - 1 - pad < 0) return -1;
    if (conv_dgrad_problem(p, nullptr, nullptr, batch, h, w, cin, cout, kh, kw, stride, pad) != STRAPS_OK) return -1;
    return dgrad_x3_blocks(p, tile_cfg);
}

static int conv_dgrad_x3_bn_impl(const unsigned short* dy3, long long dy_plane_stride, const unsigned short* w3_crsk, long long w_plane_stride,
                                 const float* addend, const unsigned* addend_bits, float* dx, int batch, int h, int wdt, int cin, int cout, int kh, int kw,
                                 int stride, int pad, int tile_cfg, const float* bn_raw, const float* bn_out, const unsigned* bn_out_bits,
                                 const float* bn_mask_scale, const float* bn_mask_shift, const float* bn_mean, const float* bn_invstd,
                                 double* bn_partials, void* stream) {
    STRAPS_REQUIRE(dy3 && w3_crsk && dx, "straps_conv_dgrad_x3_bn: null pointer");
    STRAPS_REQUIRE(bn_raw && bn_mean && bn_invstd && bn_partials && (bn_out || bn_out_bits || (bn_mask_scale && bn_mask_shift)),
                   "straps_conv_dgrad_x3_bn: the BatchNorm tensors (raw, mean, invstd, partials, and out / its bits or mask scale / shift) are required");
    STRAPS_REQUIRE(!addend_bits || addend, "straps_conv_dgrad_x3_bn_bits: the ReLU bits mask an addend");
    STRAPS_REQUIRE(!(addend_bits || bn_out_bits) || cin % 32 == 0, "straps_conv_dgrad_x3_bn_bits: bit masks need cin %% 32 == 0 (cin=%d)", cin);
    STRAPS_REQUIRE(cout % 32 == 0 && cin % 64 == 0, "straps_conv_dgrad_x3_bn: need cout%%32==0 and cin%%64==0 (cin=%d cout=%d)", cin, cout);
    STRAPS_REQUIRE(stride == 1 || stride == 2, "straps_conv_dgrad_x3_bn: stride must be 1 or 2");
    STRAPS_REQUIRE(kh * kw <= 9 && kh - 1 - pad >= 0 && kw - 1 - pad >= 0, "straps_conv_dgrad_x3_bn: unsupported filter geometry");
    STRAPS_REQUIRE(dy_plane_stride % 8 == 0 && w_plane_stride % 8 == 0, "straps_conv_dgrad_x3_bn: plane strides must be multiples of 8 elements");
    ConvP p;
    p.x = reinterpret_cast<const float*>(dy3); p.w = reinterpret_cast<const float*>(w3_crsk);
    p.xps = dy_plane_stride; p.wps = w_plane_stride;
    const int rc = conv_dgrad_problem(p, addend, dx, batch, h, wdt, cin, cout, kh, kw, stride, pad);
    if (rc != STRAPS_OK) return rc;
    p.bnr_raw = bn_raw; p.bnr_out = bn_out; p.bnr_sc = bn_mask_scale; p.bnr_sh = bn_mask_shift; p.bnr_mean = bn_mean; p.bnr_invstd = bn_invstd;
    p.bnr_part = bn_partials;
    p.bnr_bits = bn_out_bits; p.res_bits = addend_bits;
    return p.ncls ? dispatch_x3(p, tile_cfg, (hipStream_t)stream) : STRAPS_OK;
}

extern "C" int straps_conv_dgrad_x3_bn(const unsigned short* dy3, long long dy_plane_stride, const unsigned short* w3_crsk, long long w_plane_stride,
                                       const float* addend, float* dx, int batch, int h, int wdt, int cin, int cout, int kh, int kw, int stride,
                                       int pad, int tile_cfg, const float* bn_raw, const float* bn_out, const float* bn_mask_scale,
                                       const float* bn_mask_shift, const float* bn_mean, const float* bn_invstd, double* bn_partials, void* stream) {
    return conv_dgrad_x3_bn_impl(dy3, dy_plane_stride, w3_crsk, w_plane_stride, addend, nullptr, dx, batch, h, wdt, cin, cout, kh, kw, stride, pad, tile_cfg,
                                 bn_raw, bn_out, nullptr, bn_mask_scale, bn_mask_shift, bn_mean, bn_invstd, bn_partials, stream);
}

extern "C" int straps_conv_dgrad_x3_bn_bits(const unsigned short* dy3, long long dy_plane_stride, const unsigned short* w3_crsk, long long w_plane_stride,
                                            const float* addend, float* dx, int batch, int h, int wdt, int cin, int cout, int kh, int kw, int stride,
                                            int pad, int tile_cfg, const float* bn_raw, const float* bn_out, const float* bn_mask_scale,
                                            const float* bn_mask_shift, const float* bn_mean, const float* bn_invstd, double* bn_partials,
                                            const unsigned* addend_bits, const unsigned* bn_out_bits, void* stream) {
    return conv_dgrad_x3_bn_impl(dy3, dy_plane_stride, w3_crsk, w_plane_stride, addend, addend_bits, dx, batch, h, wdt, cin, cout, kh, kw, stride, pad,
                                 tile_cfg, bn_raw, bn_out, bn_out_bits, bn_mask_scale, bn_mask_shift, bn_mean, bn_invstd, bn_partials, stream);
}

extern "C" int straps_conv_x3_stat_blocks(int batch, int h, int w, int cin, int cout, int kh, int kw, int stride, int pad, int tile_cfg) {
    ConvP p;
    p.x = nullptr; p.w = nullptr; p.xps = p.wps = 0;
    if (conv_fwd_problem(p, nullptr, nullptr, nullptr, 0, nullptr, nullptr, batch, h, w, cin, cout, kh, kw, stride, pad) != STRAPS_OK) return -1;
    const long long M = p.cls[0].M;
    if (halo_choice(p, tile_cfg)) return (int)(M / 128);
    int bm, bn;
    pick_tile_x3(tile_cfg, M, cout, kh * kw * cin, bm, bn);
    return (int)((M + bm - 1) / bm);
}
```

straps-3dhumanshapepose_amd/csrc/conv_x3_kernels.h:

```cpp
#pragma once
#include "conv_igemm.h"

namespace {

typedef __bf16 bf16x8 __attribute__((ext_vector_type(8)));

__device__ __forceinline__ f32x16 mfma_bf16(bf16x8 a, bf16x8 b, f32x16 c) { return __builtin_amdgcn_mfma_f32_32x32x16_bf16(a, b, c, 0, 0, 0); }

__device__ __attribute__((aligned(16))) float k_zero16_x3[4] = {0.f, 0.f, 0.f, 0.f};

__device__ __forceinline__ int swz3(int r) { return (r >> 3) & 3; }

template <int BM, int BN, int WGM, int WGN, int NST, int ABL = 0, bool PIPE = false, int EPI = 0, int PL = 0>
__global__ __launch_bounds__(64 * WGM * WGN) void conv_igemm_x3_kernel(ConvP p) {
    const ConvP::Class& c = p.cls[blockIdx.y];
    const int cMh = c.Mh, cMw = c.Mw, cM = c.M, cMT = c.MT, cntaps = c.ntaps;
    if ((int)blockIdx.x >= cMT * p.NT) return;
    ClkSample clk;
    clk_begin(p, clk);
    constexpr int NW = WGM * WGN, RPP = 16 * NW;
    constexpr int WTM = BM / WGM, WTN = BN / WGN, MI = WTM / 32, NI = WTN / 32;
    constexpr int AP = BM / RPP, BP = BN / RPP;
    static_assert(BM % RPP == 0 && BN % RPP == 0 && WTM % 32 == 0 && WTN % 32 == 0, "tile / wave grid mismatch");
    constexpr int NSB = PL ? PL : 3;
    constexpr int NPROD = PL ? PL : 6;
    constexpr int KD = PL ? PL : 1;
    constexpr int NPIECE = NSB * (AP + BP);
    constexpr int NMFMA = 2 * NPROD * MI * NI;
    constexpr int GAP = NMFMA / NPIECE > 0 ? NMFMA / NPIECE : 1;
    extern __shared__ __attribute__((aligned(16))) float smem[];
    u16* As = reinterpret_cast<u16*>(smem);
    u16* Bs = As + NST * NSB * BM * 32;

    const int tid = threadIdx.x, lane = tid & 63, wave = tid >> 6;
    const int wm = wave / WGN, wn = wave % WGN;
    const int bid = xcd_remap(blockIdx.x, cMT * p.NT);
    const int nt = bid % p.NT, mt = bid / p.NT;
    const int m0 = mt * BM, n0 = nt * BN;
    const int lr = tid >> 2;
    const int lc = (tid & 3) ^ swz3(lr);
    const u16* xg = reinterpret_cast<const u16*>(p.x);
    const u16* wg = reinterpret_cast<const u16*>(p.w);
    X3Epilogue<BM, BN, WGM, WGN, EPI> ep;
    ep.init(p, c, m0, n0);

    int a_hi0[AP], a_wi0[AP], a_base[AP];
    const int MhMw = cMh * cMw;
#pragma unroll
    for (int q = 0; q < AP; ++q) {
        const int m = m0 + lr + RPP * q;
        if (m < cM) {
            const int b = m / MhMw;
            const int rem = m - b * MhMw;
            const int ho = rem / cMw, wo = rem - ho * cMw;
            a_hi0[q] = ho * p.stride;
            a_wi0[q] = wo * p.stride;
            a_base[q] = ((b * p.H + a_hi0[q]) * p.W + a_wi0[q]) * 32 + lc * 8;
        } else {
            a_hi0[q] = -(1 << 28);
            a_wi0[q] = 0;
            a_base[q] = 0;
        }
    }
    const u16* wrow[BP];
#pragma unroll
    for (int q = 0; q < BP; ++q) wrow[q] = wg + (n0 + lr + RPP * q) * 32 + lc * 8;

    const int cchunks = (p.Cin >> 5) / KD;
    const int nchunks = cntaps * cchunks;
    const int wave_u = __builtin_amdgcn_readfirstlane(wave);
    const int a_cstep = p.xrows * 32 * KD, b_cstep = p.Cout * 32 * KD;

    const u16* a_src[AP];
    long long a_ps[AP];
    int a_inc[AP];
    const u16* b_src[BP];
    int n_tap = 0, n_cc = 0;
    const int tl = lane < 9 ? lane : 0;
    const int v_dh = c.tap_dh[tl], v_dw = c.tap_dw[tl], v_tw = c.tap_w[tl];
    const u16* zsrc = reinterpret_cast<const u16*>(k_zero16_x3);
    asm volatile("" : "+s"(zsrc));
    auto setup_tap = [&](int tap) {
        const int dh = __builtin_amdgcn_readlane(v_dh, tap), dw = __builtin_amdgcn_readlane(v_dw, tap), tw = __builtin_amdgcn_readlane(v_tw, tap);
        const int toff = (dh * p.W + dw) * 32;
#pragma unroll
        for (int i = 0; i < AP; ++i) {
            const int hi = a_hi0[i] + dh, wi = a_wi0[i] + dw;
            const bool ok = (unsigned)hi < (unsigned)p.H && (unsigned)wi < (unsigned)p.W;
            a_src[i] = ok ? xg + (a_base[i] + toff) : zsrc;
            a_ps[i] = ok ? p.xps : 0;
            a_inc[i] = ok ? a_cstep : 0;
        }
#pragma unroll
        for (int i = 0; i < BP; ++i) b_src[i] = wrow[i] + (long long)tw * cchunks * b_cstep;
    };
    auto piece = [&](int stage, int idx) {
        if constexpr (ABL == 2 || ABL == 3) return;
        const int plane = idx / (AP + BP), r = idx % (AP + BP);
        if (r < AP) {
            __builtin_amdgcn_global_load_lds((const __attribute__((address_space(1))) void*)(a_src[r] + plane * a_ps[r]),
                                             (__attribute__((address_space(3))) void*)(As + ((stage * NSB + plane) * BM + RPP * r + 16 * wave_u) * 32), 16, 0, 0);
        } else {
            __builtin_amdgcn_global_load_lds((const __attribute__((address_space(1))) void*)(b_src[r - AP] + plane * p.wps),
                                             (__attribute__((address_space(3))) void*)(Bs + ((stage * NSB + plane) * BN + RPP * (r - AP) + 16 * wave_u) * 32), 16, 0, 0);
        }
    };
    auto advance = [&]() {
#pragma unroll
        for (int i = 0; i < AP; ++i) a_src[i] += a_inc[i];
#pragma unroll
        for (int i = 0; i < BP; ++i) b_src[i] += b_cstep;
        if (++n_cc == cchunks) {
            n_cc = 0;
            if (++n_tap < cntaps) setup_tap(n_tap);
        }
    };

    f32x16 acc[MI][NI];
#pragma unroll
    for (int i = 0; i < MI; ++i)
#pragma unroll
        for (int j = 0; j < NI; ++j)
#pragma unroll
            for (int r = 0; r < 16; ++r) acc[i][j][r] = 0.f;

    if (nchunks > 0) setup_tap(0);
#pragma unroll
    for (int s = 0; s < (PIPE ? NST : NST - 1); ++s)
        if (s < nchunks) {
#pragma unroll
            for (int idx = 0; idx < NPIECE; ++idx) piece(s, idx);
            advance();
        }
    int fo[2];
#pragma unroll
    for (int kk = 0; kk < 2; ++kk) fo[kk] = (lane & 31) * 32 + (((kk * 2 + (lane >> 5)) ^ swz3(lane & 31)) << 3);

    constexpr int TA[6] = {1, 0, 2, 0, 1, 0};
    constexpr int TB[6] = {1, 2, 0, 1, 0, 0};

    auto chunk = [&](int stage, int nstage, auto more_c, auto inflight_c, auto last_c) {
        constexpr bool MORE = decltype(more_c)::value;
        constexpr int INFLIGHT = decltype(inflight_c)::value;
        asm volatile("s_waitcnt vmcnt(%0)" ::"n"(INFLIGHT) : "memory");
        __builtin_amdgcn_s_barrier();
        asm volatile("" ::: "memory");
        if constexpr (decltype(last_c)::value) ep.prefetch();
        const u16* Ab = As + (stage * NSB * BM + wm * WTM) * 32;
        const u16* Bb = Bs + (stage * NSB * BN + wn * WTN) * 32;
        int cnt = 0;
#pragma unroll
        for (int kk = 0; kk < 2; ++kk) {
            bf16x8 a[MI][NSB], b[NI][NSB];
            if constexpr (ABL == 3) {
#pragma unroll
                for (int pl = 0; pl < NSB; ++pl) {
#pragma unroll
                    for (int i = 0; i < MI; ++i) asm volatile("" : "=v"(a[i][pl]));
#pragma unroll
                    for (int j = 0; j < NI; ++j) asm volatile("" : "=v"(b[j][pl]));
                }
            }
#pragma unroll
            for (int pl = 0; pl < NSB && ABL != 3; ++pl) {
#pragma unroll
                for (int i = 0; i < MI; ++i) a[i][pl] = *reinterpret_cast<const bf16x8*>(Ab + (pl * BM + i * 32) * 32 + fo[kk]);
#pragma unroll
                for (int j = 0; j < NI; ++j) b[j][pl] = *reinterpret_cast<const bf16x8*>(Bb + (pl * BN + j * 32) * 32 + fo[kk]);
            }
#pragma unroll
            for (int t = 0; t < NPROD; ++t)
#pragma unroll
                for (int i = 0; i < MI; ++i)
#pragma unroll
                    for (int j = 0; j < NI; ++j) {
                        if constexpr (ABL != 1) acc[i][j] = mfma_bf16(a[i][PL ? t : TA[t]], b[j][PL ? t : TB[t]], acc[i][j]);
                        if (MORE && cnt % GAP == GAP - 1 && cnt / GAP < NPIECE) piece(nstage, cnt / GAP);
                        ++cnt;
                    }
        }
        if (MORE) {
#pragma unroll
            for (int idx = NMFMA / GAP; idx < NPIECE; ++idx) piece(nstage, idx);
            advance();
        }
    };
    if constexpr (PIPE) {
        bf16x8 fa[2][MI][NSB], fb[2][NI][NSB];
        auto load_frags = [&](int stage, int kk, int set) {
            const u16* Ab = As + (stage * NSB * BM + wm * WTM) * 32;
            const u16* Bb = Bs + (stage * NSB * BN + wn * WTN) * 32;
#pragma unroll
            for (int pl = 0; pl < NSB; ++pl) {
#pragma unroll
                for (int i = 0; i < MI; ++i) fa[set][i][pl] = *reinterpret_cast<const bf16x8*>(Ab + (pl * BM + i * 32) * 32 + fo[kk]);
#pragma unroll
                for (int j = 0; j < NI; ++j) fb[set][j][pl] = *reinterpret_cast<const bf16x8*>(Bb + (pl * BN + j * 32) * 32 + fo[kk]);
            }
        };
        constexpr int HALF = NMFMA / 2, GAP2 = HALF / NPIECE > 0 ? HALF / NPIECE : 1;
        auto mfma_block = [&](int set, int nstage, auto more_c) {
            constexpr bool more = decltype(more_c)::value;
            int cnt = 0;
#pragma unroll
            for (int t = 0; t < NPROD; ++t)
#pragma unroll
                for (int i = 0; i < MI; ++i)
#pragma unroll
                    for (int j = 0; j < NI; ++j) {
                        acc[i][j] = mfma_bf16(fa[set][i][PL ? t : TA[t]], fb[set][j][PL ? t : TB[t]], acc[i][j]);
                        if (set == 1 && cnt % GAP2 == GAP2 - 1 && cnt / GAP2 < NPIECE) { if (more) piece(nstage, cnt / GAP2); }
                        ++cnt;
                    }
            if (set == 1 && more) {
#pragma unroll
                for (int idx = HALF / GAP2; idx < NPIECE; ++idx) piece(nstage, idx);
                advance();
            }
        };
        if (nchunks > 0) {
            if (nchunks >= NST) asm volatile("s_waitcnt vmcnt(%0)" ::"n"((NST - 1) * NPIECE) : "memory");
            else asm volatile("s_waitcnt vmcnt(0)" ::: "memory");
            __builtin_amdgcn_s_barrier();
            asm volatile("" ::: "memory");
            load_frags(0, 0, 0);
        }
        int stage = 0;
        auto body = [&](int q, auto more_c, auto last_c) {
            const int nxt = stage + 1 == NST ? 0 : stage + 1;
            load_frags(stage, 1, 1);
            __builtin_amdgcn_sched_barrier(0);
            mfma_block(0, 0, std::false_type{});
            __builtin_amdgcn_sched_barrier(0);
            if constexpr (!decltype(last_c)::value) {
                if (q + NST - 1 < nchunks) asm volatile("s_waitcnt vmcnt(%0)" ::"n"((NST - 2) * NPIECE) : "memory");
                else asm volatile("s_waitcnt vmcnt(0)" ::: "memory");
                asm volatile("s_waitcnt lgkmcnt(0)" ::: "memory");
                __builtin_amdgcn_s_barrier();
                asm volatile("" ::: "memory");
                load_frags(nxt, 0, 0);
            } else {
                ep.prefetch();
            }
            __builtin_amdgcn_sched_barrier(0);
            mfma_block(1, stage, more_c);
            __builtin_amdgcn_sched_barrier(0);
            stage = nxt;
        };
        int q = 0;
        for (; q + NST < nchunks; ++q) body(q, std::true_type{}, std::false_type{});
        for (; q + 1 < nchunks; ++q) body(q, std::false_type{}, std::false_type{});
        if (q < nchunks) body(q, std::false_type{}, std::true_type{});
    } else {
    int stage = 0, nstage = NST - 1;
    auto next = [&]() {
        stage = stage + 1 == NST ? 0 : stage + 1;
        nstage = nstage + 1 == NST ? 0 : nstage + 1;
    };
    int q = 0;
    for (; q + NST - 1 < nchunks; ++q) { chunk(stage, nstage, std::true_type{}, std::integral_constant<int, (NST - 2) * NPIECE>{}, std::false_type{}); next(); }
    if constexpr (NST == 3) {
        if (q + 1 < nchunks) { chunk(stage, nstage, std::false_type{}, std::integral_constant<int, NPIECE>{}, std::false_type{}); next(); ++q; }
    }
    if (q < nchunks) chunk(stage, nstage, std::false_type{}, std::integral_constant<int, 0>{}, std::true_type{});
    }

    float s1[NI], s2[NI];
    double bd1[NI], bd2[NI];
    if constexpr (EPI == 1) {
        lean_epilogue_fwd<BM, BN, WGM, WGN>(p, acc, m0, n0, c.M, s1, s2);
        igemm_store_stats<BM, BN, WGM, WGN>(p, s1, s2, mt, n0, smem);
    } else if constexpr (EPI == 2) {
        ep.finish(p, c, acc, s1, s2, bd1, bd2);
        igemm_store_bnr<BM, BN, WGM, WGN>(p, bd1, bd2, p.bnr_base[blockIdx.y] + mt, n0, smem);
    } else {
        ep.finish(p, c, acc, s1, s2, bd1, bd2);
        igemm_store_stats<BM, BN, WGM, WGN>(p, s1, s2, mt, n0, smem);
        igemm_store_bnr<BM, BN, WGM, WGN>(p, bd1, bd2, p.bnr_base[blockIdx.y] + mt, n0, smem);
    }
    clk_end(p, clk);
}

template <int BM, int BN, int WGM, int WGN, int NST, int PS, int PBUF = 2, int EPI = 0, int PL = 0>
__global__ __launch_bounds__(64 * WGM * WGN) void conv_igemm_x3h_kernel(ConvP p) {
    const ConvP::Class& c = p.cls[0];
    const int cntaps = c.ntaps;
    ClkSample clk;
    clk_begin(p, clk);
    constexpr int NW = WGM * WGN, NTH = 64 * NW, RPP = 16 * NW;
    constexpr int WTM = BM / WGM, WTN = BN / WGN, MI = WTM / 32, NI = WTN / 32;
    constexpr int BP = BN / RPP;
    static_assert(BN % RPP == 0 && WTM % 32 == 0 && WTN % 32 == 0 && PS % 16 == 0, "tile / wave grid mismatch");
    constexpr int NSB = PL ? PL : 3;
    constexpr int NPROD = PL ? PL : 6;
    constexpr int KD = PL ? PL : 1;
    constexpr int NPB = NSB * BP;
    constexpr int NPA = (PS * 4 + NTH - 1) / NTH;
    constexpr int NMFMA = 2 * NPROD * MI * NI;
    constexpr int GAP = NMFMA / NPB > 0 ? NMFMA / NPB : 1;
    extern __shared__ __attribute__((aligned(16))) float smem[];
    static_assert(PBUF == 1 || PBUF == 2, "one or two patch buffers");
    u16* As = reinterpret_cast<u16*>(smem);
    u16* Bs = As + PBUF * NSB * PS * 32;

    const int tid = threadIdx.x, lane = tid & 63, wave = tid >> 6;
    const int wm = wave / WGN, wn = wave % WGN;
    const int bid = xcd_remap(blockIdx.x, c.MT * p.NT);
    const int nt = bid % p.NT, mt = bid / p.NT;
    const int m0 = mt * BM, n0 = nt * BN;
    const u16* xg = reinterpret_cast<const u16*>(p.x);
    const u16* wg = reinterpret_cast<const u16*>(p.w);
    const int wave_u = __builtin_amdgcn_readfirstlane(wave);
    X3Epilogue<BM, BN, WGM, WGN, EPI> ep;
    ep.init(p, c, m0, n0);

    const int HW = p.H * p.W, PW = p.W + 2;
    const int nimg = BM >= HW ? BM / HW : 1;
    const int rows_t = BM >= HW ? p.H : BM / p.W;
    const int pslots = (rows_t + 2) * PW;
    const int nslots = nimg * pslots;
    const int b0 = m0 / HW, row0 = (m0 - b0 * HW) / p.W;

    int poff[NPA];
#pragma unroll
    for (int pi = 0; pi < NPA; ++pi) {
        const int slot = pi * (NTH / 4) + (tid >> 2);
        const int im = slot / pslots, rem = slot - im * pslots;
        const int py = rem / PW, px = rem - py * PW;
        const int sr = row0 + py - 1, sc = px - 1;
        const bool ok = slot < nslots && (unsigned)sr < (unsigned)p.H && (unsigned)sc < (unsigned)p.W;
        poff[pi] = ok ? (((b0 + im) * p.H + sr) * p.W + sc) * 32 + (((tid & 3) ^ ((slot >> 2) & 3)) << 3) : -1;
    }
    const u16* zsrc = reinterpret_cast<const u16*>(k_zero16_x3);
    asm volatile("" : "+s"(zsrc));
    auto patch_dma = [&](int cc) {
        u16* dst = As + (PBUF == 2 ? (cc & 1) : 0) * (NSB * PS * 32);
#pragma unroll
        for (int pi = 0; pi < NPA; ++pi) {
            if (pi * (NTH / 4) + 16 * wave_u >= nslots) break;
            if (pi * (NTH / 4) + 16 * wave_u >= PS) break;
            const bool ok = poff[pi] >= 0;
            const u16* src = ok ? xg + (poff[pi] + (long long)(cc * KD) * p.xrows * 32) : zsrc;
            const long long ps = ok ? p.xps : 0;
#pragma unroll
            for (int pl = 0; pl < NSB; ++pl)
                __builtin_amdgcn_global_load_lds((const __attribute__((address_space(1))) void*)(src + pl * ps),
                                                 (__attribute__((address_space(3))) void*)(dst + (pl * PS + pi * (NTH / 4) + 16 * wave_u) * 32), 16, 0, 0);
        }
    };

    const int lr = tid >> 2;
    const int lc = (tid & 3) ^ swz3(lr);
    const u16* wrow[BP];
#pragma unroll
    for (int q = 0; q < BP; ++q) wrow[q] = wg + (n0 + lr + RPP * q) * 32 + lc * 8;
    const int cchunks = (p.Cin >> 5) / KD;
    const int nsteps = cntaps * cchunks;
    const int tl = lane < 9 ? lane : 0;
    const int v_tw = c.tap_w[tl];
    const int v_sh = (c.tap_dh[tl] + 1) * PW + c.tap_dw[tl] + 1;
    int i_tap = 0, i_cc = 0;
    auto piece = [&](int stage, int idx) {
        const int plane = idx / BP, r = idx % BP;
        const int tw = __builtin_amdgcn_readlane(v_tw, i_tap);
        __builtin_amdgcn_global_load_lds((const __attribute__((address_space(1))) void*)(wrow[r] + (long long)((tw * cchunks + i_cc) * KD) * p.Cout * 32 + plane * p.wps),
                                         (__attribute__((address_space(3))) void*)(Bs + ((stage * NSB + plane) * BN + RPP * r + 16 * wave_u) * 32), 16, 0, 0);
    };
    auto advance = [&]() {
        if (++i_tap == cntaps) { i_tap = 0; ++i_cc; }
    };

    f32x16 acc[MI][NI];
#pragma unroll
    for (int i = 0; i < MI; ++i)
#pragma unroll
        for (int j = 0; j < NI; ++j)
#pragma unroll
            for (int r = 0; r < 16; ++r) acc[i][j][r] = 0.f;

    int a_slot[MI];
#pragma unroll
    for (int i = 0; i < MI; ++i) {
        const int il = wm * WTM + i * 32 + (lane & 31);
        const int im = il / (rows_t * p.W), rem = il - im * (rows_t * p.W);
        const int y = rem / p.W, x = rem - y * p.W;
        a_slot[i] = im * pslots + y * PW + x;
    }
    int fo[2];
#pragma unroll
    for (int kk = 0; kk < 2; ++kk) fo[kk] = (lane & 31) * 32 + (((kk * 2 + (lane >> 5)) ^ swz3(lane & 31)) << 3);
    const int kh2 = lane >> 5;

    if (nsteps > 0) patch_dma(0);
#pragma unroll
    for (int s = 0; s < NST - 1; ++s)
        if (s < nsteps) {
#pragma unroll
            for (int idx = 0; idx < NPB; ++idx) piece(s, idx);
            advance();
        }
    constexpr int TA[6] = {1, 0, 2, 0, 1, 0};
    constexpr int TB[6] = {1, 2, 0, 1, 0, 0};
    int c_tap = 0, c_cc = 0;
    auto step = [&](int stage, int nstage, auto more_c, auto inflight_c, auto last_c) {
        constexpr bool MORE = decltype(more_c)::value;
        constexpr int INFLIGHT = decltype(inflight_c)::value;
        asm volatile("s_waitcnt vmcnt(%0)" ::"n"(INFLIGHT) : "memory");
        __builtin_amdgcn_s_barrier();
        asm volatile("" ::: "memory");
        if constexpr (PBUF == 2) {
            if (c_tap == 0 && c_cc + 1 < cchunks) patch_dma(c_cc + 1);
        } else {
            if (c_tap == 0 && c_cc > 0) {
                patch_dma(c_cc);
                asm volatile("s_waitcnt vmcnt(0)" ::: "memory");
                __builtin_amdgcn_s_barrier();
                asm volatile("" ::: "memory");
            }
        }
        if constexpr (decltype(last_c)::value) ep.prefetch();
        const u16* Ap = As + (PBUF == 2 ? (c_cc & 1) : 0) * (NSB * PS * 32);
        const u16* Bb = Bs + (stage * NSB * BN + wn * WTN) * 32;
        const int tsh = __builtin_amdgcn_readlane(v_sh, c_tap);
        int ao[MI][2];
#pragma unroll
        for (int i = 0; i < MI; ++i) {
            const int sl = a_slot[i] + tsh;
#pragma unroll
            for (int kk = 0; kk < 2; ++kk) ao[i][kk] = sl * 32 + (((kk * 2 + kh2) ^ ((sl >> 2) & 3)) << 3);
        }
        int cnt = 0;
#pragma unroll
        for (int kk = 0; kk < 2; ++kk) {
            bf16x8 a[MI][NSB], b[NI][NSB];
#pragma unroll
            for (int pl = 0; pl < NSB; ++pl) {
#pragma unroll
                for (int i = 0; i < MI; ++i) a[i][pl] = *reinterpret_cast<const bf16x8*>(Ap + pl * PS * 32 + ao[i][kk]);
#pragma unroll
                for (int j = 0; j < NI; ++j) b[j][pl] = *reinterpret_cast<const bf16x8*>(Bb + (pl * BN + j * 32) * 32 + fo[kk]);
            }
#pragma unroll
            for (int t = 0; t < NPROD; ++t)
#pragma unroll
                for (int i = 0; i < MI; ++i)
#pragma unroll
                    for (int j = 0; j < NI; ++j) {
                        acc[i][j] = mfma_bf16(a[i][PL ? t : TA[t]], b[j][PL ? t : TB[t]], acc[i][j]);
                        if (MORE && cnt % GAP == GAP - 1 && cnt / GAP < NPB) piece(nstage, cnt / GAP);
                        ++cnt;
                    }
        }
        if (MORE) {
#pragma unroll
            for (int idx = NMFMA / GAP; idx < NPB; ++idx) piece(nstage, idx);
            advance();
        }
        if (++c_tap == cntaps) { c_tap = 0; ++c_cc; }
    };
    int stage = 0, nstage = NST - 1;
    auto next = [&]() {
        stage = stage + 1 == NST ? 0 : stage + 1;
        nstage = nstage + 1 == NST ? 0 : nstage + 1;
    };
    int q = 0;
    for (; q + NST - 1 < nsteps; ++q) { step(stage, nstage, std::true_type{}, std::integral_constant<int, (NST - 2) * NPB>{}, std::false_type{}); next(); }
    if constexpr (NST == 3) {
        if (q + 1 < nsteps) { step(stage, nstage, std::false_type{}, std::integral_constant<int, NPB>{}, std::false_type{}); next(); ++q; }
    }
    if (q < nsteps) step(stage, nstage, std::false_type{}, std::integral_constant<int, 0>{}, std::true_type{});

    float s1[NI], s2[NI];
    double bd1[NI], bd2[NI];
    if constexpr (EPI == 1) {
        lean_epilogue_fwd<BM, BN, WGM, WGN>(p, acc, m0, n0, c.M, s1, s2);
        igemm_store_stats<BM, BN, WGM, WGN>(p, s1, s2, mt, n0, smem);
    } else if constexpr (EPI == 2) {
        ep.finish(p, c, acc, s1, s2, bd1, bd2);
        igemm_store_bnr<BM, BN, WGM, WGN>(p, bd1, bd2, p.bnr_base[blockIdx.y] + mt, n0, smem);
    } else {
        ep.finish(p, c, acc, s1, s2, bd1, bd2);
        igemm_store_stats<BM, BN, WGM, WGN>(p, s1, s2, mt, n0, smem);
        igemm_store_bnr<BM, BN, WGM, WGN>(p, bd1, bd2, p.bnr_base[blockIdx.y] + mt, n0, smem);
    }
    clk_end(p, clk);
}

template <int BM, int BN, int WGM, int WGN, int NST, int PS, int PBUF = 2, int EPI = 0, int PL = 0>
int launch_x3h(const ConvP& p0, hipStream_t st) {
    ConvP p = p0;
    p.NT = p.Cout / BN;
    p.cls[0].MT = p.cls[0].M / BM;
    p.bnr_base[0] = 0;
    const size_t lds = ((size_t)PBUF * (PL ? PL : 3) * PS + (size_t)NST * (PL ? PL : 3) * BN) * 32 * sizeof(u16);
    STRAPS_RAISE_LDS((conv_igemm_x3h_kernel<BM, BN, WGM, WGN, NST, PS, PBUF, EPI, PL>), lds, "conv_igemm_x3h_kernel");
    hipLaunchKernelGGL((conv_igemm_x3h_kernel<BM, BN, WGM, WGN, NST, PS, PBUF, EPI, PL>), dim3(p.cls[0].MT * p.NT, 1), dim3(64 * WGM * WGN), lds, st, p);
    STRAPS_CHECK_LAUNCH("conv_igemm_x3h_kernel");
    return STRAPS_OK;
}

inline int halo_patch_slots(const ConvP& p) {
    constexpr int BM = 128;
    if (p.ncls != 1 || p.stride != 1 || p.omul != 1) return 0;
    const ConvP::Class& c = p.cls[0];
    if (c.ntaps != 9 || c.Mh != p.H || c.Mw != p.W || p.OH != p.H || p.OW != p.W || c.oah != 0 || c.oaw != 0 || c.M % BM != 0) return 0;
    for (int t = 0; t < 9; ++t)
        if (c.tap_dh[t] < -1 || c.tap_dh[t] > 1 || c.tap_dw[t] < -1 || c.tap_dw[t] > 1) return 0;
    const int HW = p.H * p.W;
    if (BM >= HW) { if (BM % HW != 0) return 0; return (BM / HW) * (p.H + 2) * (p.W + 2); }
    if (BM % p.W != 0 || HW % BM != 0) return 0;
    return (BM / p.W + 2) * (p.W + 2);
}

template <int BM, int BN, int WGM, int WGN, int NST, int ABL = 0, bool PIPE = false, int EPI = 0, int PL = 0>
int launch_x3(const ConvP& p0, hipStream_t st) {
    ConvP p = p0;
    p.NT = p.Cout / BN;
    int maxblk = 0;
    int base = 0;
    for (int i = 0; i < p.ncls; ++i) {
        p.cls[i].MT = (p.cls[i].M + BM - 1) / BM;
        if (p.cls[i].MT * p.NT > maxblk) maxblk = p.cls[i].MT * p.NT;
        p.bnr_base[i] = base;
        base += p.cls[i].MT;
    }
    const size_t lds = (size_t)NST * (PL ? PL : 3) * (BM + BN) * 32 * sizeof(u16);
    STRAPS_RAISE_LDS((conv_igemm_x3_kernel<BM, BN, WGM, WGN, NST, ABL, PIPE, EPI, PL>), lds, "conv_igemm_x3_kernel");
    hipLaunchKernelGGL((conv_igemm_x3_kernel<BM, BN, WGM, WGN, NST, ABL, PIPE, EPI, PL>), dim3(maxblk, p.ncls), dim3(64 * WGM * WGN), lds, st, p);
    STRAPS_CHECK_LAUNCH("conv_igemm_x3_kernel");
    return STRAPS_OK;
}

}
```

straps-3dhumanshapepose_amd/csrc/regressor_train.hip:

```cpp
#include <algorithm>
#include <cstring>

#include "regressor_net.h"

namespace {

constexpr long long kX3fMinRows = 16384;
constexpr size_t kNone = ~(size_t)0;

struct Layer : Conv, Extent {
    long long rows;
    bool fmode;
    bool keep, planes, defer, bits;
    bool keep_grad;
    int nblk;
    size_t x, x3;
    long long x_ps;
    const Layer* a_bn;
    size_t raw, ss, out, out3, bitsb;
    long long out_ps;
};

struct Plan : Net {
    bool x3;
    int B, stem_nblk;
    Geometry geo;
    Layer lay[kMaxConvs];
    bool pool_planes;
    long long amax;
    size_t wstem, wsd, table, one, krsc, crsk, w1f, w1e, w3;
    size_t nz, stem_raw, stem_ss, pool, pool3, idx;
    long long pool_ps;
    size_t feat, c1, ests, h1s, h2s, fpart;
    size_t g[2], dz, dskip, dt, draw, draw3, drawd, drawd3, part, bnws, wgws, tact, sdraw, swgws, dgb, dests, dh2s, dh1s, dc1, dfeat;
    size_t bytes;
    const Layer& unit_out(int ui) const { return lay[units[ui].c[units[ui].nconv - 1]]; }
};

bool x3f_mode(const Plan& p, const Layer& cv) {
    if (!p.x3 || !straps_conv_x3f_supported(cv.cin, cv.cout, cv.k, cv.k, cv.stride, cv.pad)) return false;
    return (long long)p.B * cv.Ho * cv.Wo >= kX3fMinRows;
}

void needs(const Plan& p, const Layer& cv, bool& f32, bool& planes) {
    if (x3f_mode(p, cv)) { f32 = true; planes = false; return; }
    f32 = !straps_conv_wgrad_x3_on_planes(p.B, cv.H, cv.W, cv.cin, cv.cout, cv.k, cv.k, cv.stride, cv.pad);
    planes = true;
}

bool make_plan(Plan& p, int B, int H, int W) {
    if (!make_geometry(p, B, H, W, p.geo)) return false;
    p.x3 = p.precision == 0;
    p.B = B;
    for (int i = 0; i < p.nconvs; ++i) {
        static_cast<Conv&>(p.lay[i]) = p.convs[i];
        static_cast<Extent&>(p.lay[i]) = p.geo.e[i];
    }
    size_t b = 0;
    auto take = [&](size_t bytes) { const size_t o = b; b = align_up(b + (bytes ? bytes : 1)); return o; };
    auto f32s = [&](long long n) { return take((size_t)n * sizeof(float)); };
    auto planes = [&](long long n) { return take(3 * (size_t)round8(n) * sizeof(unsigned short)); };
    p.wstem = f32s((long long)straps_stem_weight_floats(p.cin));
    p.wsd = p.cin <= STRAPS_STEM_DGRAD_MAX_CIN ? f32s((long long)straps_stem_dgrad_weight_floats(p.cin)) : kNone;
    p.table = take(kMaxConvs * sizeof(straps_pack_desc_t));
    p.one = f32s(1);
    if (p.x3) { p.krsc = take(3 * (size_t)p.ps * sizeof(unsigned short)); p.crsk = take(3 * (size_t)p.ps * sizeof(unsigned short)); }
    else { p.krsc = f32s(p.conv_total); p.crsk = f32s(p.conv_total); }
    p.w1f = f32s((long long)p.H1 * p.F);
    p.w1e = f32s((long long)p.H1 * kEstLd);
    p.w3 = f32s((long long)(kNumParams + 31) / 32 * 32 * p.H2);
    const long long stem_n = (long long)B * p.geo.Hs * p.geo.Ws * 64, pool_n = (long long)B * p.geo.Hp * p.geo.Wp * 64;
    p.nz = take(straps_stem_nzmask_words(B, p.cin, H, W) * sizeof(uint32_t));
    p.stem_raw = f32s(stem_n);
    p.stem_ss = f32s(4 * 64);
    p.pool = f32s(pool_n);
    p.idx = take((size_t)pool_n);
    p.stem_nblk = straps_stem_stat_blocks(B, H, W);
    long long fpart = (long long)p.stem_nblk * 64 * 2;
    p.amax = pool_n;
    {
        const Unit& u0 = p.units[0];
        bool all = x3f_mode(p, p.lay[u0.c[0]]) && (!u0.has_ds || x3f_mode(p, p.lay[u0.ds]));
        p.pool_planes = p.x3 && !all;
        p.pool3 = p.pool_planes ? planes(pool_n) : kNone;
        p.pool_ps = p.pool_planes ? round8(pool_n) : 0;
    }
    long long part_d = 1, bnws = straps_bn_bwd_workspace_bytes(stem_n, 64), wgws = 4;
    size_t in = p.pool, in3 = p.pool3;
    long long in_ps = p.pool_ps;
    auto tape = [&](Layer& cv) -> bool {
        const int ch = cv.H, cw = cv.W;
        cv.rows = (long long)B * cv.Ho * cv.Wo;
        cv.fmode = x3f_mode(p, cv);
        cv.nblk = cv.fmode ? straps_conv_x3f_stat_blocks(B, ch, cw, cv.cin, cv.cout, cv.k, cv.k, cv.stride, cv.pad, 0)
                 : p.x3    ? straps_conv_x3_stat_blocks(B, ch, cw, cv.cin, cv.cout, cv.k, cv.k, cv.stride, cv.pad, 0)
                           : straps_conv_stat_blocks(B, cv.Ho, cv.Wo, cv.cout, cv.k * cv.k * cv.cin, 0);
        if (cv.nblk <= 0) return false;
        fpart = std::max(fpart, (long long)cv.nblk * cv.cout * 2);
        const long long n = cv.rows * cv.cout;
        p.amax = std::max(p.amax, n);
        bnws = std::max(bnws, (long long)straps_bn_bwd_workspace_bytes(cv.rows, cv.cout));
        wgws = std::max(wgws, (long long)(cv.fmode ? straps_conv_wgrad_x3f_workspace_bytes(B, ch, cw, cv.cin, cv.cout, cv.k, cv.k, cv.stride, cv.pad)
                                                   : straps_conv_wgrad_workspace_bytes(B, ch, cw, cv.cin, cv.cout, cv.k, cv.k, cv.stride, cv.pad)));
        if (p.x3) {
            const int nb = cv.fmode ? straps_conv_dgrad_x3f_bn_blocks(B, ch, cw, cv.cin, cv.cout, cv.k, cv.k, cv.stride, cv.pad, 0)
                                    : straps_conv_dgrad_x3_bn_blocks(B, ch, cw, cv.cin, cv.cout, cv.k, cv.k, cv.stride, cv.pad, 0);
            part_d = std::max(part_d, (long long)nb * cv.cin * 2);
        }
        cv.raw = f32s(n);
        cv.ss = f32s(4LL * cv.cout);
        return true;
    };
    for (int ui = 0; ui < p.nunits; ++ui) {
        const Unit& u = p.units[ui];
        if (u.has_ds) {
            Layer& cv = p.lay[u.ds];
            if (!tape(cv)) return false;
            cv.x = in; cv.x3 = in3; cv.x_ps = in_ps; cv.a_bn = nullptr;
            cv.keep = true; cv.planes = false; cv.defer = false; cv.bits = false;
            cv.out = f32s(cv.rows * cv.cout); cv.out3 = kNone; cv.out_ps = 0; cv.bitsb = kNone;
        }
        size_t t = in, t3 = in3;
        long long t_ps = in_ps;
        const Layer* a_bn = nullptr;
        for (int ci = 0; ci < u.nconv; ++ci) {
            Layer& cv = p.lay[u.c[ci]];
            if (!tape(cv)) return false;
            cv.x = t; cv.x3 = t3; cv.x_ps = t_ps; cv.a_bn = a_bn;
            bool keep = true, pl = true, defer = false;
            if (p.x3 && !cv.last) {
                needs(p, p.lay[u.c[ci + 1]], keep, pl);
                defer = keep && !pl;
            } else if (p.x3) {
                pl = false;
                if (ui + 1 < p.nunits) {
                    const Unit& nx = p.units[ui + 1];
                    bool f, q;
                    needs(p, p.lay[nx.c[0]], f, q);
                    pl = q;
                    if (nx.has_ds) { needs(p, p.lay[nx.ds], f, q); pl = pl || q; }
                }
            }
            cv.defer = defer;
            cv.bits = p.x3 && cv.last;
            if (defer) {
                cv.keep = false; cv.planes = false;
                cv.out = kNone; cv.out3 = kNone; cv.out_ps = 0; cv.bitsb = kNone;
                t = cv.raw; t3 = kNone; t_ps = 0; a_bn = &cv;
            } else {
                if (!p.x3) { keep = true; pl = false; }
                else keep = keep || !pl;
                cv.keep = keep; cv.planes = pl;
                cv.out = keep ? f32s(cv.rows * cv.cout) : kNone;
                cv.out3 = pl ? planes(cv.rows * cv.cout) : kNone;
                cv.out_ps = pl ? round8(cv.rows * cv.cout) : 0;
                cv.bitsb = cv.bits ? take((size_t)cv.rows * (cv.cout / 32) * sizeof(uint32_t)) : kNone;
                t = cv.out; t3 = cv.out3; t_ps = cv.out_ps; a_bn = nullptr;
            }
        }
        in = t; in3 = t3; in_ps = t_ps;
    }
    for (int i = 0; i < p.nconvs; ++i) {
        Layer& cv = p.lay[i];
        cv.keep_grad = !p.x3 || cv.fmode || !straps_conv_wgrad_x3_on_planes(B, cv.H, cv.W, cv.cin, cv.cout, cv.k, cv.k, cv.stride, cv.pad);
    }
    p.feat = f32s((long long)B * p.F);
    p.c1 = f32s((long long)B * p.H1);
    p.ests = f32s((long long)(p.iters + 1) * B * kEstLd);
    p.h1s = f32s((long long)p.iters * B * p.H1);
    p.h2s = f32s((long long)p.iters * B * p.H2);
    p.fpart = f32s(fpart);
    for (int i = 0; i < 2; ++i) p.g[i] = f32s(p.amax);
    p.dz = f32s(p.amax);
    p.dskip = f32s(p.amax);
    p.dt = f32s(p.amax);
    p.draw = f32s(p.amax);
    p.drawd = f32s(p.amax);
    p.draw3 = p.x3 ? planes(p.amax) : kNone;
    p.drawd3 = p.x3 ? planes(p.amax) : kNone;
    p.part = take((size_t)part_d * sizeof(double));
    p.bnws = take((size_t)bnws);
    p.wgws = take((size_t)wgws);
    p.tact = take(straps_stem_tiles(B, H, W));
    p.sdraw = f32s(stem_n);
    p.swgws = take(straps_stem_wgrad_workspace_bytes(B, p.cin, H, W));
    p.dgb = f32s(2 * 2048);
    p.dests = f32s((long long)(p.iters + 1) * B * kEstLd);
    p.dh2s = f32s((long long)p.iters * B * p.H2);
    p.dh1s = f32s((long long)p.iters * B * p.H1);
    p.dc1 = f32s((long long)B * p.H1);
    p.dfeat = f32s((long long)B * p.F);
    p.bytes = b;
    return true;
}
// ... 75 lines not shown
    const bool x3 = p.x3;
    unsigned short* krsc3 = ws.h(p.krsc);
    float* krsc = ws.f(p.krsc);

    RG_CALL(straps_pack_stem_weight(params + p.stem.w_off, ws.f(p.wstem), C, stream));
    PackTable tbl;
    memset(&tbl, 0, sizeof(tbl));
    for (int i = 0; i < p.nconvs; ++i) {
        const Conv& cv = p.convs[i];
        straps_pack_desc_t& e = tbl.d[i];
        e.src = params + cv.w_off;
        e.dst_krsc = x3 ? nullptr : ws.f(p.krsc) + cv.first;
        e.dst_crsk = x3 ? nullptr : ws.f(p.crsk) + cv.first;
        e.o = cv.cout; e.c = cv.cin; e.r = cv.k; e.s = cv.k;
        e.first = cv.first;
    }
    straps_pack_desc_t* table = (straps_pack_desc_t*)(ws.base + p.table);
    hipLaunchKernelGGL(write_table_kernel, dim3(1), dim3(64), 0, st, tbl, p.nconvs, table, ws.f(p.one));
    STRAPS_CHECK_LAUNCH("write_table_kernel");
    if (x3) RG_CALL(straps_pack_conv_weights_batched_x3(table, p.nconvs, p.conv_total, krsc3, ws.h(p.crsk), p.ps, stream));
    else RG_CALL(straps_pack_conv_weights_batched(table, p.nconvs, p.conv_total, stream));
    RG_CALL(straps_ief_pack(params + p.ief.fc1w, params + p.ief.fc3w, ws.f(p.w1f), ws.f(p.w1e), ws.f(p.w3), F, kNumParams, H1, H2, kEstLd, stream));

    uint32_t* nz = (uint32_t*)(ws.base + p.nz);
    float* part = ws.f(p.fpart);
    float* sss = ws.f(p.stem_ss);
    RG_CALL(straps_stem_nzmask(x, nz, B, C, h, w, stream));
    RG_CALL(straps_stem_fwd(x, ws.f(p.wstem), nullptr, nullptr, 0, ws.f(p.stem_raw), part, nz, B, C, h, w, stream));
    RG_CALL(finalize(params, bn_state, part, p.stem_nblk, 64, (long long)B * p.geo.Hs * p.geo.Ws, p.stem.gb_off, p.stem.rs_off, sss, st));
    if (p.pool_planes)
        RG_CALL(straps_bn_relu_maxpool_fwd_x3(ws.f(p.stem_raw), sss, sss + 64, ws.f(p.pool), (uint8_t*)(ws.base + p.idx), ws.h(p.pool3), p.pool_ps,
                                              B, p.geo.Hs, p.geo.Ws, 64, stream));
    else
        RG_CALL(straps_bn_relu_maxpool_fwd(ws.f(p.stem_raw), sss, sss + 64, ws.f(p.pool), (uint8_t*)(ws.base + p.idx), B, p.geo.Hs, p.geo.Ws, 64, stream));

    auto conv_fwd = [&](const Layer& cv) -> int {
        const float* sa = cv.a_bn ? ws.f(cv.a_bn->ss) : nullptr;
        if (cv.fmode)
            return straps_conv_fwd_x3f(ws.f(cv.x), sa, sa ? sa + cv.a_bn->cout : nullptr, cv.a_bn ? 1 : 0, krsc3 + cv.first, p.ps, nullptr, nullptr,
                                       nullptr, 0, ws.f(cv.raw), part, B, cv.H, cv.W, cv.cin, cv.cout, cv.k, cv.k, cv.stride, cv.pad, 0, stream);
        if (x3)
            return straps_conv_fwd_x3(ws.h(cv.x3), cv.x_ps, krsc3 + cv.first, p.ps, nullptr, nullptr, nullptr, 0, ws.f(cv.raw), part,
                                      B, cv.H, cv.W, cv.cin, cv.cout, cv.k, cv.k, cv.stride, cv.pad, 0, stream);
        return straps_conv_fwd(ws.f(cv.x), krsc + cv.first, nullptr, nullptr, nullptr, 0, ws.f(cv.raw), part, B, cv.H, cv.W, cv.cin, cv.cout,
                               cv.k, cv.k, cv.stride, cv.pad, 0, stream);
    };
    auto conv_bn = [&](const Layer& cv, const float* residual) -> int {
        RG_CALL(conv_fwd(cv));
        float* ss = ws.f(cv.ss);
        RG_CALL(finalize(params, bn_state, part, cv.nblk, cv.cout, cv.rows, cv.gb_off, cv.rs_off, ss, st));
        if (cv.defer) return STRAPS_OK;
        if (x3 && cv.relu) {
            if (cv.bits)
                return straps_bn_apply_bits_x3(ws.f(cv.raw), ss, ss + cv.cout, residual, ws.f(cv.out), ws.h(cv.out3), cv.out_ps, ws.u(cv.bitsb),
                                               cv.rows, cv.cout, stream);
            return straps_bn_apply_x3(ws.f(cv.raw), ss, ss + cv.cout, residual, 1, ws.f(cv.out), ws.h(cv.out3), cv.out_ps, cv.rows, cv.cout, stream);
        }
        return straps_bn_apply(ws.f(cv.raw), ss, ss + cv.cout, residual, cv.relu ? 1 : 0, ws.f(cv.out), cv.rows, cv.cout, stream);
    };
    for (int ui = 0; ui < p.nunits; ++ui) {
        const Unit& u = p.units[ui];
        const float* idt = ws.f(p.lay[u.c[0]].x);
        if (u.has_ds) {
            RG_CALL(conv_bn(p.lay[u.ds], nullptr));
            idt = ws.f(p.lay[u.ds].out);
        }
        for (int ci = 0; ci < u.nconv; ++ci) RG_CALL(conv_bn(p.lay[u.c[ci]], p.lay[u.c[ci]].last ? idt : nullptr));
    }

    RG_CALL(ief_forward(p, B, ws.f(p.unit_out(p.nunits - 1).out), p.geo.Hf * p.geo.Wf, init_est, ws.f(p.w1f), ws.f(p.w1e), params + p.ief.fc1b,
                        params + p.ief.fc2w, params + p.ief.fc2b, ws.f(p.w3), params + p.ief.fc3b, ws.f(p.feat), ws.f(p.c1), ws.f(p.ests),
                        ws.f(p.h1s), (long long)B * H1, ws.f(p.h2s), (long long)B * H2, est, ld_est, stream));
    return STRAPS_OK;
}

extern "C" int straps_regressor_bwd(const straps_regressor_desc_t* d, const float* params, const float* x, int batch, int h, int w,
                                    const float* dest, int ld_dest, float* grads, float* dx, void* workspace, size_t workspace_bytes,
                                    void* stream) {
    static const char* fn = "straps_regressor_bwd";
    Plan p;
    RG_CALL(check_common(fn, d, params, x, batch, h, w, workspace, p));
    STRAPS_REQUIRE(dest, "%s: null pointer `dest`", fn);
    STRAPS_REQUIRE(ld_dest >= kNumParams, "%s: `ld_dest` must be >= %d (got %d)", fn, kNumParams, ld_dest);
    STRAPS_REQUIRE(((uintptr_t)dest & 3) == 0 && ((uintptr_t)grads & 3) == 0 && ((uintptr_t)dx & 3) == 0,
                   "%s: `dest`, `grads` and `dx` must be float-aligned", fn);
    STRAPS_REQUIRE(!dx || p.cin <= STRAPS_STEM_DGRAD_MAX_CIN, "%s: `dx` needs `in_channels` <= %d (got %d)", fn, STRAPS_STEM_DGRAD_MAX_CIN, p.cin);
    STRAPS_REQUIRE(workspace_bytes >= p.bytes, "%s: `workspace_bytes` is %zu, this batch needs %zu (straps_regressor_train_workspace_bytes)", fn,
                   workspace_bytes, p.bytes);
    const Ws ws{(char*)workspace};
    const int B = batch, C = p.cin, F = p.F, H1 = p.H1, H2 = p.H2, T = p.iters, P = kNumParams;
    const bool x3 = p.x3, pg = grads != nullptr;
    const unsigned short* crsk3 = ws.h(p.crsk);
    const float* crsk = ws.f(p.crsk);
    float* dgb = ws.f(p.dgb);
    auto dgamma = [&](long long gb) { return pg ? grads + gb : dgb; };
    auto dbeta = [&](long long gb, int c) { return pg ? grads + gb + c : dgb + 2048; };

    float* dests = ws.f(p.dests);
    float* dh2s = ws.f(p.dh2s);
    float* dh1s = ws.f(p.dh1s);
    float* dc1 = ws.f(p.dc1);
    float* dfeat = ws.f(p.dfeat);
    const float* ests = ws.f(p.ests);
    const float* h1s = ws.f(p.h1s);
    const float* h2s = ws.f(p.h2s);
    RG_CALL(straps_masked_copy(dest, ld_dest, nullptr, 0, dests + (size_t)T * B * kEstLd, kEstLd, B, P, 0, stream));
    auto gd = [](const float* a, long long sam, long long sak, const float* b, long long sbk, long long sbn, float* c, int ldc, int m, int n, int k) {
        straps_gemm_desc_t g;
        memset(&g, 0, sizeof(g));
        g.a = a; g.sam = sam; g.sak = sak; g.b = b; g.sbk = sbk; g.sbn = sbn; g.c = c; g.ldc = ldc; g.m = m; g.n = n; g.k = k;
        return g;
    };
    for (int it = T - 1; it >= 0; --it) {
        float* dnext = dests + (size_t)(it + 1) * B * kEstLd;
        float* dh2 = dh2s + (size_t)it * B * H2;
        float* dh1 = dh1s + (size_t)it * B * H1;
        straps_gemm_desc_t g = gd(dnext, kEstLd, 1, params + p.ief.fc3w, H2, 1, dh2, H2, B, H2, P);
        g.mask = h2s + (size_t)it * B * H2; g.ldmask = H2;
        RG_CALL(straps_gemm_multi(&g, 1, stream));
        g = gd(dh2, H2, 1, params + p.ief.fc2w, H1, 1, dh1, H1, B, H1, H2);
        g.mask = h1s + (size_t)it * B * H1; g.ldmask = H1;
        g.c2 = dc1; g.ldc2 = H1; g.accumulate2 = it != T - 1;
        RG_CALL(straps_gemm_multi(&g, 1, stream));
        g = gd(dh1, H1, 1, ws.f(p.w1e), kEstLd, 1, dests + (size_t)it * B * kEstLd, kEstLd, B, P, H1);
        g.addend = dnext; g.ldadd = kEstLd;
        RG_CALL(straps_gemm_multi(&g, 1, stream));
    }
    if (!pg) {
        const straps_gemm_desc_t g = gd(dc1, H1, 1, ws.f(p.w1f), F, 1, dfeat, F, B, F, H1);
        RG_CALL(straps_gemm_multi(&g, 1, stream));
    } else {
        const int KB = T * B;
        const float* one = ws.f(p.one);
        const straps_gemm_desc_t g[8] = {
            gd(dh2s, 1, H2, h1s, H1, 1, grads + p.ief.fc2w, H1, H2, H1, KB),
            gd(dc1, 1, H1, ws.f(p.feat), F, 1, grads + p.ief.fc1w, F + P, H1, F, B),
            gd(dh1s, 1, H1, ests, kEstLd, 1, grads + p.ief.fc1w + F, F + P, H1, P, KB),
            gd(dests + (size_t)B * kEstLd, 1, kEstLd, h2s, H2, 1, grads + p.ief.fc3w, H2, P, H2, KB),
            gd(dc1, H1, 1, ws.f(p.w1f), F, 1, dfeat, F, B, F, H1),
            gd(one, 0, 0, dh2s, H2, 1, grads + p.ief.fc2b, H2, 1, H2, KB),
            gd(one, 0, 0, dests + (size_t)B * kEstLd, kEstLd, 1, grads + p.ief.fc3b, P, 1, P, KB),
            gd(one, 0, 0, dc1, H1, 1, grads + p.ief.fc1b, H1, 1, H1, B)};
        RG_CALL(straps_gemm_multi(g, 8, stream));
    }

    double* part = (double*)(ws.base + p.part);
    void* bnws = ws.base + p.bnws;
    void* wgws = ws.base + p.wgws;
    const Layer* pending = nullptr;
    int pending_nblk = 0;
    int cur = 0;
    RG_CALL(straps_gap_bwd(dfeat, ws.f(p.g[cur]), B, p.geo.Hf * p.geo.Wf, F, stream));

    auto bn_bwd = [&](const Layer& cv, const float* dy, bool masked, float* dz, const unsigned* mask_bits, size_t out_off, size_t out3_off) -> int {
        const float* ss = ws.f(cv.ss);
        const int c = cv.cout;
        const bool sink = x3 && !cv.fmode;
        float* draw = (cv.keep_grad || !sink) ? ws.f(out_off) : nullptr;
        unsigned short* planes = sink ? ws.h(out3_off) : nullptr;
        const long long ps = sink ? round8(cv.rows * c) : 0;
        const bool from_raw = masked && !cv.last;
        const unsigned* bits = mask_bits ? mask_bits : (masked && !from_raw ? ws.u(cv.bitsb) : nullptr);
        const bool fused = pending == &cv && masked;
        if (pending == &cv) pending = nullptr;
        float* dg = dgamma(cv.gb_off);
        float* db = dbeta(cv.gb_off, c);
        if (bits) {
            if (fused)
                return straps_bn_bwd_finish_bits_x3(dy, bits, ws.f(cv.raw), ss + 2 * c, ss + 3 * c, params + cv.gb_off, dg, db, draw, planes, ps, part,
                                                    pending_nblk, bnws, cv.rows, c, 0, stream);
            return straps_bn_bwd_bits_x3(dy, bits, ws.f(cv.raw), ss + 2 * c, ss + 3 * c, params + cv.gb_off, dg, db, draw, planes, ps, bnws,
                                         cv.rows, c, 0, stream);
        }
        if (fused)
            return straps_bn_bwd_finish_x3(dy, from_raw ? nullptr : ws.f(cv.out), ws.f(cv.raw), ss + 2 * c, ss + 3 * c, params + cv.gb_off,
                                           from_raw ? ss : nullptr, from_raw ? ss + c : nullptr, dg, db, draw, dz, planes, ps, part, pending_nblk, bnws,
                                           cv.rows, c, 0, stream);
        return straps_bn_bwd_x3(dy, masked && !from_raw ? ws.f(cv.out) : nullptr, ws.f(cv.raw), ss + 2 * c, ss + 3 * c, params + cv.gb_off,
                                from_raw ? ss : nullptr, from_raw ? ss + c : nullptr, dg, db, draw, dz, planes, ps, bnws, cv.rows, c, 0, stream);
    };
    auto wgrad = [&](const Layer& cv, size_t draw_off, size_t draw3_off) -> int {
        if (!pg) return STRAPS_OK;
        float* dw = grads + cv.w_off;
        if (cv.fmode) {
            const float* sa = cv.a_bn ? ws.f(cv.a_bn->ss) : nullptr;
            return straps_conv_wgrad_x3f(ws.f(cv.x), sa, sa ? sa + cv.a_bn->cout : nullptr, cv.a_bn ? 1 : 0, ws.f(draw_off), dw, wgws, B, cv.H, cv.W,
                                         cv.cin, cv.cout, cv.k, cv.k, cv.stride, cv.pad, 0, stream);
        }
        if (x3)
            return straps_conv_wgrad_x3(ws.f(cv.x), cv.keep_grad ? ws.f(draw_off) : nullptr, ws.h(cv.x3), cv.x_ps, ws.h(draw3_off), round8(cv.rows * cv.cout),
                                        dw, wgws, B, cv.H, cv.W, cv.cin, cv.cout, cv.k, cv.k, cv.stride, cv.pad, 0, stream);
        return straps_conv_wgrad(ws.f(cv.x), ws.f(draw_off), dw, wgws, B, cv.H, cv.W, cv.cin, cv.cout, cv.k, cv.k, cv.stride, cv.pad, 0, stream);
    };
    auto dgrad = [&](const Layer& cv, size_t draw_off, size_t draw3_off, const float* addend, const unsigned* addend_bits, const Layer* bn_next,
                     float* out) -> int {
        const long long gps = round8(cv.rows * cv.cout);
        if (cv.fmode) {
            const float *raw = nullptr, *msc = nullptr, *msh = nullptr, *mean = nullptr, *invstd = nullptr;
            const unsigned* nbits = nullptr;
            double* prt = nullptr;
            int nblk = 0;
            if (bn_next) {
                const float* ssn = ws.f(bn_next->ss);
                const int cn = bn_next->cout;
                const bool from_raw = !bn_next->last;
                nbits = from_raw ? nullptr : ws.u(bn_next->bitsb);
                if (from_raw || nbits) {
                    nblk = straps_conv_dgrad_x3f_bn_blocks(B, cv.H, cv.W, cv.cin, cv.cout, cv.k, cv.k, cv.stride, cv.pad, 0);
                    prt = part;
                    raw = ws.f(bn_next->raw); mean = ssn + 2 * cn; invstd = ssn + 3 * cn;
                    if (from_raw) { msc = ssn; msh = ssn + cn; }
                }
            }
            RG_CALL(straps_conv_dgrad_x3f(ws.f(draw_off), crsk3 + cv.first, p.ps, addend, addend_bits, out, B, cv.H, cv.W, cv.cin, cv.cout, cv.k, cv.k,
                                          cv.stride, cv.pad, 0, raw, nbits, msc, msh, mean, invstd, prt, stream));
            if (prt) { pending = bn_next; pending_nblk = nblk; }
            return STRAPS_OK;
        }
        if (x3) {
            const unsigned short* g3 = ws.h(draw3_off);
            const unsigned short* w3 = crsk3 + cv.first;
            if (bn_next) {
                const float* ssn = ws.f(bn_next->ss);
                const int cn = bn_next->cout;
                const bool from_raw = !bn_next->last;
                const int nblk = straps_conv_dgrad_x3_bn_blocks(B, cv.H, cv.W, cv.cin, cv.cout, cv.k, cv.k, cv.stride, cv.pad, 0);
                const unsigned* nbits = from_raw ? nullptr : ws.u(bn_next->bitsb);
                if (addend_bits || nbits)
                    RG_CALL(straps_conv_dgrad_x3_bn_bits(g3, gps, w3, p.ps, addend, out, B, cv.H, cv.W, cv.cin, cv.cout, cv.k, cv.k, cv.stride, cv.pad, 0,
                                                         ws.f(bn_next->raw), (from_raw || nbits) ? nullptr : ws.f(bn_next->out),
                                                         from_raw ? ssn : nullptr, from_raw ? ssn + cn : nullptr, ssn + 2 * cn, ssn + 3 * cn, part,
                                                         addend_bits, nbits, stream));
                else
                    RG_CALL(straps_conv_dgrad_x3_bn(g3, gps, w3, p.ps, addend, out, B, cv.H, cv.W, cv.cin, cv.cout, cv.k, cv.k, cv.stride, cv.pad, 0,
                                                    ws.f(bn_next->raw), from_raw ? nullptr : ws.f(bn_next->out), from_raw ? ssn : nullptr,
                                                    from_raw ? ssn + cn : nullptr, ssn + 2 * cn, ssn + 3 * cn, part, stream));
                pending = bn_next;
                pending_nblk = nblk;
                return STRAPS_OK;
            }
            if (addend_bits)
                return straps_conv_dgrad_x3_bits(g3, gps, w3, p.ps, addend, out, B, cv.H, cv.W, cv.cin, cv.cout, cv.k, cv.k, cv.stride, cv.pad, 0,
                                                 addend_bits, stream);
            return straps_conv_dgrad_x3(g3, gps, w3, p.ps, addend, out, B, cv.H, cv.W, cv.cin, cv.cout, cv.k, cv.k, cv.stride, cv.pad, 0, stream);
        }
        return straps_conv_dgrad(ws.f(draw_off), crsk + cv.first, addend, out, B, cv.H, cv.W, cv.cin, cv.cout, cv.k, cv.k, cv.stride, cv.pad, 0, stream);
    };
    for (int ui = p.nunits - 1; ui >= 0; --ui) {
        const Unit& u = p.units[ui];
        const Layer* prev_last = ui > 0 ? &p.unit_out(ui - 1) : nullptr;
        const Layer& lc = p.unit_out(ui);
        const float* dy = ws.f(p.g[cur]);
        const unsigned* ubits = x3 ? ws.u(lc.bitsb) : nullptr;
        const float* dz = dy;
        if (ubits) {
            RG_CALL(bn_bwd(lc, dy, true, nullptr, nullptr, p.draw, p.draw3));
        } else {
            RG_CALL(bn_bwd(lc, dy, true, ws.f(p.dz), nullptr, p.draw, p.draw3));
            dz = ws.f(p.dz);
        }
        RG_CALL(wgrad(lc, p.draw, p.draw3));
        const float* dskip = dz;
        const unsigned* dskip_bits = nullptr;
        if (u.has_ds) {
            const Layer& ds = p.lay[u.ds];
            RG_CALL(bn_bwd(ds, dz, false, nullptr, ubits, p.drawd, p.drawd3));
            RG_CALL(wgrad(ds, p.drawd, p.drawd3));
            RG_CALL(dgrad(ds, p.drawd, p.drawd3, nullptr, nullptr, nullptr, ws.f(p.dskip)));
            dskip = ws.f(p.dskip);
        } else {
            dskip_bits = ubits;
        }
        for (int ci = u.nconv - 1; ci > 0; --ci) {
            const Layer& prev = p.lay[u.c[ci - 1]];
            RG_CALL(dgrad(p.lay[u.c[ci]], p.draw, p.draw3, nullptr, nullptr, x3 ? &prev : nullptr, ws.f(p.dt)));
            RG_CALL(bn_bwd(prev, ws.f(p.dt), true, nullptr, nullptr, p.draw, p.draw3));
            RG_CALL(wgrad(prev, p.draw, p.draw3));
        }
        RG_CALL(dgrad(p.lay[u.c[0]], p.draw, p.draw3, dskip, dskip_bits, x3 ? prev_last : nullptr, ws.f(p.g[cur ^ 1])));
        cur ^= 1;
    }

    const float* sss = ws.f(p.stem_ss);
    const uint32_t* nz = (const uint32_t*)(ws.base + p.nz);
    uint8_t* tact = nullptr;
    if (!dx) {
        tact = (uint8_t*)(ws.base + p.tact);
        RG_CALL(straps_stem_tile_activity(nz, tact, B, C, h, w, stream));
    }
    float* sdraw = ws.f(p.sdraw);
    RG_CALL(straps_bn_bwd_pooled_sparse(ws.f(p.g[cur]), (const uint8_t*)(ws.base + p.idx), ws.f(p.stem_raw), sss + 128, sss + 192, params + p.stem.gb_off,
                                        sss, sss + 64, dgamma(p.stem.gb_off), dbeta(p.stem.gb_off, 64), sdraw, bnws, B, p.geo.Hs, p.geo.Ws, 64, 0, tact, stream));
    if (dx) {
        RG_CALL(straps_pack_stem_dgrad_weight(params + p.stem.w_off, ws.f(p.wsd), C, stream));
        RG_CALL(straps_stem_dgrad(sdraw, ws.f(p.wsd), dx, B, C, h, w, 0, stream));
    }
    if (pg) RG_CALL(straps_stem_wgrad(x, sdraw, grads + p.stem.w_off, ws.base + p.swgws, nz, B, C, h, w, 0, stream));
    return STRAPS_OK;
}

extern "C" int straps_regressor_export_infer_params(const straps_regressor_desc_t* d, const float* params, const float* bn_state,
                                                    const float* init_est, float* infer_params, void* stream) {
    static const char* fn = "straps_regressor_export_infer_params";
    const char* bad = check_desc(d, true);
    STRAPS_REQUIRE(!bad, "%s: %s", fn, bad);
    STRAPS_REQUIRE(params, "%s: null pointer `params`", fn);
    STRAPS_REQUIRE(bn_state, "%s: null pointer `bn_state`", fn);
    STRAPS_REQUIRE(init_est, "%s: null pointer `init_est`", fn);
    STRAPS_REQUIRE(infer_params, "%s: null pointer `infer_params`", fn);
    Net n;
    make_net(d, n);
    hipStream_t st = (hipStream_t)stream;
    auto copy = [&](long long dst, const float* src, long long count) -> int {
        const hipError_t e = hipMemcpyAsync(infer_params + dst, src, (size_t)count * sizeof(float), hipMemcpyDeviceToDevice, st);
        if (e != hipSuccess) {
            straps_set_error("%s: hipMemcpyAsync failed: %s", fn, hipGetErrorString(e));
            return STRAPS_EHIP;
        }
        return STRAPS_OK;
    };
    auto layer = [&](const Conv& cv) -> int {
        RG_CALL(copy(cv.inf_w, params + cv.w_off, cv.weights()));
        RG_CALL(copy(cv.inf_bn, params + cv.gb_off, 2LL * cv.cout));
        return copy(cv.inf_bn + 2LL * cv.cout, bn_state + cv.rs_off, 2LL * cv.cout);
    };
    RG_CALL(layer(n.stem));
    for (int i = 0; i < n.nconvs; ++i) RG_CALL(layer(n.convs[i]));
    RG_CALL(copy(n.ief_inf.fc1w, params + n.ief.fc1w, n.train_floats - n.ief.fc1w));
    RG_CALL(copy(n.inf_init, init_est, kNumParams));
    return STRAPS_OK;
}
```

straps-3dhumanshapepose_amd/hipabi.py:

```python
import ctypes as C
import os
import subprocess

_HERE = os.path.dirname(os.path.abspath(__file__))
CSRC = os.path.join(_HERE, 'csrc')
LIB_PATH = os.path.join(CSRC, 'libstraps_hip.so')
HEADER = os.path.join(os.path.dirname(_HERE), 'include', 'straps_hip.h')
SOURCES = ['abi.hip', 'augment.hip', 'pose.hip', 'ief.hip', 'elementwise.hip', 'conv.hip', 'conv_x3.hip', 'conv_x3_lean.hip', 'conv_bf16.hip', 'conv_x3f.hip', 'conv_wgrad_x3f.hip', 'stem.hip', 'stem_dgrad.hip', 'smpl.hip',
           'smpl_bwd.hip', 'backward.hip', 'train.hip', 'metrics.hip', 'image.hip', 'raster.hip', 'exchange.hip',
           'regressor.hip', 'regressor_train.hip']

_lib = None
LINK_LIBS = ['-ldl']
EXTRA_FLAGS = {'smpl.hip': ['-fno-slp-vectorize']}


def _existing_sources():
    return [os.path.join(CSRC, s) for s in SOURCES if os.path.isfile(os.path.join(CSRC, s))]


TOOLS_LIB_PATH = os.path.join(os.path.dirname(_HERE), 'tools', 'bin', 'libstraps_hip_tools.so')


def build(force=False, verbose=False, tools=False):
    srcs = _existing_sources()
    lib_path = TOOLS_LIB_PATH if tools else LIB_PATH
    if tools and not force and os.environ.get('STRAPS_TOOLS_NO_BUILD') == '1' and os.path.isfile(lib_path):
        import sys
        import time
        print('hipabi.build(tools=True): STRAPS_TOOLS_NO_BUILD=1 -- reusing %s (built %s)' % (lib_path, time.strftime('%Y-%m-%d %H:%M:%S', time.localtime(os.path.getmtime(lib_path)))),
              file=sys.stderr)
        return lib_path
    import glob
    hdrs = sorted(glob.glob(os.path.join(CSRC, '*.h'))) + [HEADER]
    deps = srcs + hdrs
    if not force and os.path.isfile(lib_path) and all(os.path.getmtime(lib_path) > os.path.getmtime(d) for d in deps):
        if not tools:
            _audit(lib_path, 'hipabi.build (library up to date)')
        return lib_path
    hipcc = os.environ.get('HIPCC', '/opt/rocm/bin/hipcc')
    flags = ['--offload-arch=gfx950', '-O3', '-std=c++17', '-fPIC'] + (['-DSTRAPS_TOOLS'] if tools else [])
    extra = dict(EXTRA_FLAGS)
    if tools and os.environ.get('STRAPS_TOOLS_SMPL_FLAGS'):
        extra['smpl.hip'] = extra.get('smpl.hip', []) + os.environ['STRAPS_TOOLS_SMPL_FLAGS'].split()
    if tools and os.environ.get('STRAPS_TOOLS_SMPL_BWD_FLAGS'):
        extra['smpl_bwd.hip'] = extra.get('smpl_bwd.hip', []) + os.environ['STRAPS_TOOLS_SMPL_BWD_FLAGS'].split()
    if tools and os.environ.get('STRAPS_TOOLS_RASTER_FLAGS'):
        extra['raster.hip'] = extra.get('raster.hip', []) + os.environ['STRAPS_TOOLS_RASTER_FLAGS'].split()
    objdir = os.path.join(os.path.dirname(TOOLS_LIB_PATH), 'build') if tools else os.path.join(CSRC, 'build')
    os.makedirs(objdir, exist_ok=True)
    jobs = []
    for s in srcs:
        o = os.path.join(objdir, os.path.basename(s)[:-4] + '.o')
        if force or not os.path.isfile(o) or any(os.path.getmtime(o) <= os.path.getmtime(d) for d in [s] + hdrs):
            cmd = [hipcc] + flags + extra.get(os.path.basename(s), []) + ['-c', s, '-o', o]
            if verbose:
                print(' '.join(cmd))
            jobs.append((cmd, subprocess.Popen(cmd, cwd=CSRC)))
    for cmd, p in jobs:
        if p.wait() != 0:
            raise subprocess.CalledProcessError(p.returncode, cmd)
    objs = [os.path.join(objdir, os.path.basename(s)[:-4] + '.o') for s in srcs]
    cmd = [hipcc, '--offload-arch=gfx950', '-fPIC', '-shared', '-o', lib_path] + objs + LINK_LIBS
    if verbose:
        print(' '.join(cmd))
    subprocess.run(cmd, check=True, cwd=CSRC)
    if not tools:
        _audit(lib_path, 'hipabi.build', fresh=True)
    return lib_path


def _audit(lib_path, what, fresh=False):
    from . import isa_audit
    if not fresh and isa_audit.stamp_ok(lib_path):
        return
    if not isa_audit.enforce(lib_path, what):
        import warnings
        warnings.warn('%s: llvm-objdump not found under %s -- the packed-operand-select audit of %s (DESIGN section 1: wrong results in lanes 48..63 on '
                      'MI355X) did NOT run; set STRAPS_LLVM_BIN or audit the library where it was built (tools/audit_packed_fp32.py)'
                      % (what, isa_audit.LLVM_BIN, lib_path), RuntimeWarning, stacklevel=3)


class SmplModelStruct(C.Structure):
    _fields_ = [('blend_frag', C.c_void_p), ('j_template', C.c_void_p), ('j_shapedirs', C.c_void_p),
                ('parents', C.c_void_p), ('depth', C.c_void_p), ('max_depth', C.c_int32), ('skin_k', C.c_int32),
                ('skin_w', C.c_void_p), ('skin_j', C.c_void_p), ('vj_ptr', C.c_void_p), ('n_tiles', C.c_int32),
                ('reserved0', C.c_int32), ('pick_ids', C.c_void_p), ('blend_frag_t', C.c_void_p), ('children', C.c_void_p),
                ('jrt_ptr', C.c_void_p), ('jrt_code', C.c_void_p), ('jrt_w', C.c_void_p), ('dj_ptr', C.c_void_p), ('dj_code', C.c_void_p),
                ('dj_w', C.c_void_p), ('blend_frag_h', C.c_void_p), ('blend_h_unscale', C.c_float), ('reserved1', C.c_int32), ('skin_frag_p', C.c_void_p)]


class PackDesc(C.Structure):
    _fields_ = [('src', C.c_void_p), ('dst_krsc', C.c_void_p), ('dst_crsk', C.c_void_p), ('o', C.c_int32), ('c', C.c_int32),
                ('r', C.c_int32), ('s', C.c_int32), ('first', C.c_longlong)]


class GemmDesc(C.Structure):
    _fields_ = [('a', C.c_void_p), ('sam', C.c_longlong), ('sak', C.c_longlong), ('b', C.c_void_p), ('sbk', C.c_longlong), ('sbn', C.c_longlong),
                ('c', C.c_void_p), ('ldc', C.c_int32), ('accumulate', C.c_int32), ('addend', C.c_void_p), ('ldadd', C.c_int32), ('reserved0', C.c_int32),
                ('mask', C.c_void_p), ('ldmask', C.c_int32), ('reserved1', C.c_int32), ('c2', C.c_void_p), ('ldc2', C.c_int32), ('accumulate2', C.c_int32),
                ('m', C.c_int32), ('n', C.c_int32), ('k', C.c_int32), ('reserved2', C.c_int32)]


def gemm_desc(a, sam, sak, b, sbk, sbn, c, ldc, m, n, k, accumulate=0, addend=None, ldadd=0, mask=None, ldmask=0, c2=None, ldc2=0, accumulate2=0):
    adr = lambda t: None if t is None else (t if isinstance(t, int) else t.data_ptr())
    return GemmDesc(adr(a), sam, sak, adr(b), sbk, sbn, adr(c), ldc, accumulate, adr(addend), ldadd, 0, adr(mask), ldmask, 0, adr(c2), ldc2, accumulate2,
                    m, n, k, 0)


def gemm_multi(descs):
    arr = (GemmDesc * len(descs))(*descs)
    check(lib().straps_gemm_multi(arr, len(descs), stream_ptr()), 'straps_gemm_multi')


class RegressorDesc(C.Structure):
    _fields_ = [('layers', C.c_int32), ('in_channels', C.c_int32), ('ief_iters', C.c_int32), ('precision', C.c_int32)]


_P, _I, _L, _F, _Z, _D = C.c_void_p, C.c_int, C.c_longlong, C.c_float, C.c_size_t, C.c_double

ABI_VERSION = 12
SIGNATURES = {
    'straps_abi_version': (_I, []),
    'straps_last_error': (C.c_char_p, []),
    'straps_device_count': (_I, []),
    'straps_wall_clock_khz': (_I, []),
    'straps_set_clock_accumulator': (_I, [_P]),
    'straps_selftest_mfma_peak': (_I, [_P, _P, _I, _I, _P]),
    'straps_selftest_mfma_bf16': (_I, [_P, _P, _I, _I, _P]),
    'straps_selftest_mfma_bf16_dense': (_I, [_P, _P, _I, _I, _I, _P]),
    'straps_pack_conv_weight': (_I, [_P, _P, _I, _I, _I, _I, _P]),
    'straps_pack_conv_weight_dgrad': (_I, [_P, _P, _I, _I, _I, _I, _P]),
    'straps_pack_conv_weights_batched': (_I, [_P, _I, _L, _P]),
    'straps_pack_conv_weights_batched_x3': (_I, [_P, _I, _L, _P, _P, _L, _P]),
    'straps_stem_weight_floats': (_Z, [_I]),
    'straps_pack_stem_weight': (_I, [_P, _P, _I, _P]),
    'straps_bn_fold': (_I, [_P, _P, _P, _P, _F, _P, _P, _I, _P]),
    'straps_bn_fold_stats': (_I, [_P, _P, _P, _P, _F, _P, _P, _P, _P, _I, _P]),
    'straps_stem_stat_blocks': (_I, [_I, _I, _I]),
    'straps_stem_nzmask_words': (_Z, [_I, _I, _I, _I]),
    'straps_stem_nzmask': (_I, [_P, _P, _I, _I, _I, _I, _P]),
    'straps_stem_fwd': (_I, [_P, _P, _P, _P, _I, _P, _P, _P, _I, _I, _I, _I, _P]),
    'straps_conv_trace_buffer': (_I, [_P]),
    'straps_split3_bf16': (_I, [_P, _P, _L, _L, _P]),
    'straps_split3_bf16_cm': (_I, [_P, _P, _L, _I, _L, _P]),
    'straps_conv_fwd_x3': (_I, [_P, _L, _P, _L, _P, _P, _P, _I, _P, _P, _I, _I, _I, _I, _I, _I, _I, _I, _I, _I, _P]),
    'straps_conv_fwd_x3p': (_I, [_P, _L, _P, _L, _P, _P, _P, _I, _P, _P, _L, _I, _I, _I, _I, _I, _I, _I, _I, _I, _I, _P]),
    'straps_conv_dgrad_x3': (_I, [_P, _L, _P, _L, _P, _P, _I, _I, _I, _I, _I, _I, _I, _I, _I, _I, _P]),
    'straps_split_bf16_cm': (_I, [_P, _P, _L, _I, _P]),
    'straps_pack_conv_weight_bf16': (_I, [_P, _P, _I, _I, _I, _I, _P]),
    'straps_conv_bf16_tile_choice': (_I, [_I] * 9),
    'straps_conv_fwd_bf16': (_I, [_P, _P, _P, _P, _P, _I, _P, _P] + [_I] * 10 + [_P]),
    'straps_conv_x3_stat_blocks': (_I, [_I] * 10),
    'straps_conv_x3f_supported': (_I, [_I] * 6),
    'straps_conv_fwd_x3f': (_I, [_P, _P, _P, _I, _P, _L, _P, _P, _P, _I, _P, _P] + [_I] * 10 + [_P]),
    'straps_conv_x3f_stat_blocks': (_I, [_I] * 10),
    'straps_conv_dgrad_x3f': (_I, [_P, _P, _L, _P, _P, _P] + [_I] * 10 + [_P] * 8),
    'straps_conv_dgrad_x3f_bn_blocks': (_I, [_I] * 10),
    'straps_conv_wgrad_x3f_workspace_bytes': (_Z, [_I] * 9),
    'straps_conv_wgrad_x3f': (_I, [_P, _P, _P, _I, _P, _P, _P] + [_I] * 10 + [_P]),
    'straps_bn_apply_x3': (_I, [_P, _P, _P, _P, _I, _P, _P, _L, _L, _I, _P]),
    'straps_bn_relu_maxpool_fwd_x3': (_I, [_P, _P, _P, _P, _P, _P, _L, _I, _I, _I, _I, _P]),
    'straps_conv_wgrad_x3_on_planes': (_I, [_I] * 9),
    'straps_conv_dgrad_x3_bn_blocks': (_I, [_I] * 10),
    'straps_conv_dgrad_x3_bn': (_I, [_P, _L, _P, _L, _P, _P, _I, _I, _I, _I, _I, _I, _I, _I, _I, _I, _P, _P, _P, _P, _P, _P, _P, _P]),
    'straps_bn_bwd_finish_x3': (_I, [_P] * 13 + [_L, _P, _I, _P, _L, _I, _I, _P]),
    'straps_conv_wgrad_x3': (_I, [_P, _P, _P, _L, _P, _L, _P, _P, _I, _I, _I, _I, _I, _I, _I, _I, _I, _I, _P]),
    'straps_bn_bwd_x3': (_I, [_P] * 13 + [_L, _P, _L, _I, _I, _P]),
    'straps_bn_apply_bits_x3': (_I, [_P, _P, _P, _P, _P, _P, _L, _P, _L, _I, _P]),
    'straps_bn_bwd_bits_x3': (_I, [_P] * 10 + [_L, _P, _L, _I, _I, _P]),
    'straps_bn_bwd_finish_bits_x3': (_I, [_P] * 10 + [_L, _P, _I, _P, _L, _I, _I, _P]),
    'straps_conv_dgrad_x3_bits': (_I, [_P, _L, _P, _L, _P, _P, _I, _I, _I, _I, _I, _I, _I, _I, _I, _I, _P, _P]),
    'straps_conv_dgrad_x3_bn_bits': (_I, [_P, _L, _P, _L, _P, _P, _I, _I, _I, _I, _I, _I, _I, _I, _I, _I, _P, _P, _P, _P, _P, _P, _P, _P, _P, _P]),
    'straps_conv_stat_blocks': (_I, [_I, _I, _I, _I, _I, _I]),
    'straps_conv_fwd': (_I, [_P, _P, _P, _P, _P, _I, _P, _P, _I, _I, _I, _I, _I, _I, _I, _I, _I, _I, _P]),
    'straps_maxpool_fwd': (_I, [_P, _P, _I, _I, _I, _I, _P]),
    'straps_gap_fwd': (_I, [_P, _P, _I, _I, _I, _P]),
    'straps_bn_stats_finalize': (_I, [_P, _I, _I, _L, _P, _P, _F, _F, _P, _P, _P, _P, _P, _P, _P]),
    'straps_bn_apply': (_I, [_P, _P, _P, _P, _I, _P, _L, _I, _P]),
    'straps_linear_fwd': (_I, [_P, _I, _P, _I, _P, _P, _P, _I, _I, _I, _I, _I, _P]),
    'straps_broadcast_rows': (_I, [_P, _I, _P, _I, _I, _P]),
    'straps_ief_pack': (_I, [_P, _P, _P, _P, _P, _I, _I, _I, _I, _I, _P]),
    'straps_gemm_multi': (_I, [C.POINTER(GemmDesc), _I, _P]),
    'straps_rot6d_fwd': (_I, [_P, _L, _I, _P, _L, _P]),
    'straps_rodrigues_fwd': (_I, [_P, _P, _L, _P]),
    'straps_rodrigues_bwd': (_I, [_P, _P, _P, _L, _P]),
    'straps_orthographic_project': (_I, [_P, _P, _I, _P, _L, _I, _P]),
    'straps_orthographic_project_bwd': (_I, [_P, _P, _I, _P, _P, _P, _L, _I, _P]),
    'straps_perspective_project': (_I, [_P, _P, _P, _P, _I, _P, _L, _I, _P]),
    'straps_smpl_workspace_bytes': (_Z, [C.POINTER(SmplModelStruct), _L]),
    'straps_smpl_fwd': (_I, [C.POINTER(SmplModelStruct), _P, _P, _P, _P, _P, _L, _I, _I, _P]),
    'straps_smpl_bwd_workspace_bytes': (_Z, [_L, _I]),
    'straps_smpl_bwd': (_I, [C.POINTER(SmplModelStruct), _P, _P, _P, _P, _P, _P, _P, _L, _I, _P]),
    'straps_smpl_bwd_aa': (_I, [C.POINTER(SmplModelStruct), _P, _P, _P, _P, _P, _P, _P, _P, _P, _L, _I, _P]),
    'straps_conv_dgrad': (_I, [_P, _P, _P, _P, _I, _I, _I, _I, _I, _I, _I, _I, _I, _I, _P]),
    'straps_conv_wgrad_workspace_bytes': (_Z, [_I, _I, _I, _I, _I, _I, _I, _I, _I]),
    'straps_conv_wgrad': (_I, [_P, _P, _P, _P, _I, _I, _I, _I, _I, _I, _I, _I, _I, _I, _P]),
    'straps_stem_wgrad_workspace_bytes': (_Z, [_I, _I, _I, _I]),
    'straps_stem_wgrad': (_I, [_P, _P, _P, _P, _P, _I, _I, _I, _I, _I, _P]),
    'straps_stem_dgrad_weight_floats': (_Z, [_I]),
    'straps_pack_stem_dgrad_weight': (_I, [_P, _P, _I, _P]),
    'straps_stem_dgrad': (_I, [_P, _P, _P, _I, _I, _I, _I, _I, _P]),
    'straps_bn_bwd_blocks': (_I, [_L, _I]),
    'straps_bn_bwd_workspace_bytes': (_Z, [_L, _I]),
    'straps_bn_bwd': (_I, [_P, _P, _P, _P, _P, _P, _P, _P, _P, _P, _P, _P, _P, _L, _I, _I, _P]),
    'straps_bn_relu_maxpool_fwd': (_I, [_P, _P, _P, _P, _P, _I, _I, _I, _I, _P]),
    'straps_bn_bwd_pooled': (_I, [_P, _P, _P, _P, _P, _P, _P, _P, _P, _P, _P, _P, _I, _I, _I, _I, _I, _P]),
    'straps_bn_bwd_pooled_sparse': (_I, [_P, _P, _P, _P, _P, _P, _P, _P, _P, _P, _P, _P, _I, _I, _I, _I, _I, _P, _P]),
    'straps_stem_tiles': (_Z, [_I, _I, _I]),
    'straps_stem_tile_activity': (_I, [_P, _P, _I, _I, _I, _I, _P]),
    'straps_maxpool_fwd_idx': (_I, [_P, _P, _P, _I, _I, _I, _I, _P]),
    'straps_maxpool_bwd': (_I, [_P, _P, _P, _I, _I, _I, _I, _P]),
    'straps_gap_bwd': (_I, [_P, _P, _I, _I, _I, _P]),
    'straps_masked_copy': (_I, [_P, _I, _P, _I, _P, _I, _I, _I, _I, _P]),
    'straps_rot6d_bwd': (_I, [_P, _L, _I, _P, _P, _L, _L, _P]),
    'straps_build_proxy_input': (_I, [_P, _P, _P, _I, _I, _I, _P]),
    'straps_build_proxy_input_std': (_I, [_P, _P, _P, _I, _I, _I, _I, _P]),
    'straps_build_proxy_input_nz': (_I, [_P, _P, _P, _P, _I, _I, _I, _I, _P]),
    'straps_loss_workspace_bytes': (_Z, [_L]),
    'straps_loss_fwd_bwd': (_I, [_P, _P, _P, _I, _P, _P, _P, _P, _P, _P, _P, _P, _P, _P, _P, _P, _P, _P, _L, _I, _P]),
    'straps_loss_fwd_bwd_gm': (_I, [_P, _P, _P, _I, _P, _P, _P, _P, _P, _P, _P, _P, _P, _P, _P, _P, _P, _P, _L, _I, _P, _F, _P]),
    'straps_count_visible': (_I, [_P, _P, _L, _I, _I, _P]),
    'straps_adam_step': (_I, [_P, _P, _P, _P, _L, _I, _F, _F, _F, _F, _F, _P, _P]),
    'straps_mse_fwd': (_I, [_P, _P, _P, _L, _I, _F, _F, _P, _P, _P]),
    'straps_mse_bwd': (_I, [_P, _P, _P, _L, _I, _F, _F, _P, _P, _P]),
    'straps_augment_seg': (_I, [_P, _P, _P, _F, _I, _P, _I, _I, _P]),
    'straps_rasterize_workspace_bytes': (_Z, [_L, _I, _I]),
    'straps_rasterize_parts': (_I, [_P, _P, _P, _P, _P, _P, _P, _P, _P, _L, _I, _I, _I, _I, _F, _F, _P, _D, _D, _P]),
    'straps_philox_fill': (_I, [C.c_ulonglong, _P, _L, C.c_uint, _P, _L, _I, _P]),
    'straps_counter_add': (_I, [_P, _I, _L, _P]),
    'straps_gather_f32': (_I, [_P, _P, _P, _I, _P]),
    'straps_memset_zero': (_I, [_P, _Z, _P]),
    'straps_augment_smpl': (_I, [_P, _L, _P, _P, _P, _P, _I, _P, _D, _D, _P, _P, _P, _L, _P]),
    'straps_augment_cam_t': (_I, [_P, _P, _P, _D, _D, _D, _P, _L, _P]),
    'straps_deviate_verts2d': (_I, [_P, _P, _D, _D, _P, _L, _P]),
    'straps_deviate_joints2d': (_I, [_P, _P, _D, _D, _D, _D, _P, _L, _P]),
    'straps_project_targets': (_I, [_P, _P, _F, _F, _F, _F, _P, _P, _L, _P]),
    'straps_point_metrics': (_I, [_P, _P, _P, _L, _I, _P]),
    'straps_crop_resize': (_I, [_P, _P, _P, _D, _D, _D, _D, _D, _P, _P, _P, _I, _I, _I, _I, _P]),
    'straps_comm_unique_id': (_I, [_P]),
    'straps_comm_init_rank': (_I, [_P, _I, _I, C.POINTER(C.c_void_p)]),
    'straps_comm_destroy': (_I, [_P]),
    'straps_comm_size': (_I, [_P]),
    'straps_comm_library': (C.c_char_p, []),
    'straps_allreduce_grads': (_I, [_P, _L, _P, _P]),
    'straps_regressor_param_floats': (_Z, [C.POINTER(RegressorDesc)]),
    'straps_regressor_prepared_bytes': (_Z, [C.POINTER(RegressorDesc)]),
    'straps_regressor_prepare': (_I, [C.POINTER(RegressorDesc), _P, _P, _P]),
    'straps_regressor_workspace_bytes': (_Z, [C.POINTER(RegressorDesc), _I, _I, _I]),
    'straps_regressor_fwd_infer': (_I, [C.POINTER(RegressorDesc), _P, _P, _I, _I, _I, _P, _I, _P, _P, _Z, _P]),
    'straps_regressor_train_param_floats': (_Z, [C.POINTER(RegressorDesc)]),
    'straps_regressor_bn_state_floats': (_Z, [C.POINTER(RegressorDesc)]),
    'straps_regressor_train_workspace_bytes': (_Z, [C.POINTER(RegressorDesc), _I, _I, _I]),
    'straps_regressor_fwd_train': (_I, [C.POINTER(RegressorDesc), _P, _P, _P, _P, _I, _I, _I, _P, _I, _P, _Z, _P]),
    'straps_regressor_bwd': (_I, [C.POINTER(RegressorDesc), _P, _P, _I, _I, _I, _P, _I, _P, _P, _P, _Z, _P]),
    'straps_regressor_export_infer_params': (_I, [C.POINTER(RegressorDesc), _P, _P, _P, _P, _P]),
}


def load(path=None):
    global _lib
    if _lib is not None and path is None:
        return _lib
    p = path or LIB_PATH
    if not os.path.isfile(p):
        raise RuntimeError('libstraps_hip.so is not built (%s missing): run `python -c "import __graft_entry__ as g; '
                           'g.build()"` -- this package has no CPU fallback' % p)
    if os.path.abspath(p) != os.path.abspath(TOOLS_LIB_PATH):
        _audit(p, 'hipabi.load')
    lib = C.CDLL(p)
    if hasattr(lib, 'straps_abi_version'):
        lib.straps_abi_version.restype = C.c_int
        got = lib.straps_abi_version()
        if got != ABI_VERSION:
            raise RuntimeError('%s is ABI version %d, this package binds version %d: rebuild it (`python -c "import __graft_entry__ as g; g.build()"`)'
                               % (p, got, ABI_VERSION))
    for name, (res, args) in SIGNATURES.items():
        if not hasattr(lib, name):
            continue
        fn = getattr(lib, name)
        fn.restype = res
        fn.argtypes = args
    if path is None:
        _lib = lib
    return lib


def lib():
    return load()


def use_library(path):
    global _lib
    _lib = load(path)
    return _lib


_TRACE = os.environ.get('STRAPS_TRACE_CALLS')
_trace_fh = None


def check(rc, what):
    if rc != 0:
        raise RuntimeError('%s failed (code %d): %s' % (what, rc, lib().straps_last_error().decode()))
    if _TRACE:
        import torch
        global _trace_fh
        if _trace_fh is None:
            _trace_fh = open(_TRACE, 'a', buffering=1)
        if not torch.cuda.is_current_stream_capturing():
            _trace_fh.write(what + '\n')
            _trace_fh.flush()
            os.fsync(_trace_fh.fileno())
            torch.cuda.synchronize()


def stream_ptr():
    import torch
    return C.c_void_p(torch.cuda.current_stream().cuda_stream)


def _first_cuda_tensor(values):
    import torch
    for v in values:
        if isinstance(v, torch.Tensor):
            if v.is_cuda:
# ... 39 lines not shown
```

Baseline: 8000.

## Fuse downsample projection dgrad into strided 3x3 dgrad of ResNet transition blocks

In ResNet transition units, the 1x1 stride-2 projection's data gradient is folded into the 3x3 stride-2 conv's data-gradient kernel. It runs as extra K-chunks in the centre-tap parity class, accumulated into a separate accumulator and summed in the BN-backward epilogue. This removes one dgrad launch and the fp32 dskip tensor write and read, at the cost of writing the projection gradient's bf16 planes. It adds a new SC kernel instantiation with a launch-bounds occupancy hint, extra registers for the second accumulator, and more load imbalance across parity classes.

```diff
diff --git a/include/straps_hip.h b/include/straps_hip.h
--- a/include/straps_hip.h
+++ b/include/straps_hip.h
@@ -261,6 +261,12 @@
                                  const float* bn_mask_scale, const float* bn_mask_shift, const float* bn_mean,
                                  const float* bn_invstd, double* bn_partials, const unsigned* addend_bits,
                                  const unsigned* bn_out_bits, void* stream);
+int straps_conv_dgrad_x3_bn_sc(const unsigned short* dy3, long long dy_plane_stride, const unsigned short* w3_crsk,
+                               long long w_plane_stride, const unsigned short* sc_dy3, long long sc_dy_plane_stride,
+                               const unsigned short* sc_w3_crsk, long long sc_w_plane_stride, float* dx_nhwc, int batch, int h,
+                               int w, int cin, int cout, int tile_cfg, const float* bn_raw, const unsigned* bn_out_bits,
+                               const float* bn_mask_scale, const float* bn_mask_shift, const float* bn_mean,
+                               const float* bn_invstd, double* bn_partials, void* stream);
 int straps_conv_wgrad_x3_on_planes(int batch, int h, int w, int cin, int cout, int kh, int kw,
                                    int stride, int pad);
 int straps_conv_wgrad_x3(const float* x_nhwc, const float* dy_nhwc, const unsigned short* x3,
diff --git a/straps-3dhumanshapepose_amd/autograd_ops.py b/straps-3dhumanshapepose_amd/autograd_ops.py
--- a/straps-3dhumanshapepose_amd/autograd_ops.py
+++ b/straps-3dhumanshapepose_amd/autograd_ops.py
@@ -44,6 +44,7 @@
 
 _FUSE_BN_SUMS = True
 _SPARSE_STEM_TAIL = True
+_FUSE_TRANSITION = True
 
 
 def _packed_dgrad_weight(net, conv):
@@ -199,6 +200,39 @@
     return dx
 
 
+def _transition_fused(unit, rec0, recd, sink, bn_next):
+    if sink is None or not _FUSE_TRANSITION or not _FUSE_BN_SUMS or unit.downsample is None or bn_next is None or bn_next.get('bits') is None:
+        return False
+    B, H, W, Cin, Cout, k, stride, pad, Ho, Wo = rec0['geom']
+    Bd, Hd, Wd, Cind, Coutd, kd, strided, padd, _, _ = recd['geom']
+    return (k, stride, pad, kd, strided, padd) == (3, 2, 1, 1, 2, 0) and rec0['x'] is recd['x'] and (B, H, W, Cin, Cout) == (Bd, Hd, Wd, Cind, Coutd) \
+        and Cin % 64 == 0 and H >= 2 and W >= 2
+
+
+def _conv_dgrad_sc(L, net, rec0, draw, recd, drawd, planes_sink, bn_next):
+    B, H, W, Cin, Cout, k, stride, pad, Ho, Wo = rec0['geom']
+    hit = planes_sink.get(id(draw))
+    if hit is not None and hit[0] is draw:
+        g3, gps = hit[1], hit[2]
+    else:
+        from .encoder_exec import split3
+        g3, gps = split3(L, draw)
+    hd = planes_sink.get(id(drawd))
+    if hd is None or hd[0] is not drawd:
+        raise RuntimeError('transition data gradient: the planes of the projection\'s gradient were not written')
+    w3, wps = net._packed_weight_x3(rec0['conv'], dgrad=True)
+    wd3, wdps = net._packed_weight_x3(recd['conv'], dgrad=True)
+    ssn = bn_next['stats']
+    dx = torch.empty(B, H, W, Cin, device=drawd.device, dtype=torch.float32)
+    nblk = L.straps_conv_dgrad_x3_bn_blocks(B, H, W, Cin, Cout, k, k, stride, pad, 0)
+    part = torch.empty(nblk, Cin, 2, device=dx.device, dtype=torch.float64)
+    hipabi.check(L.straps_conv_dgrad_x3_bn_sc(hipabi.ptr(g3), gps, hipabi.ptr(w3), wps, hipabi.ptr(hd[1]), hd[2], hipabi.ptr(wd3), wdps, hipabi.ptr(dx), B, H, W,
+                                              Cin, Cout, 0, hipabi.ptr(bn_next['raw']), hipabi.ptr(bn_next['bits']), None, None, hipabi.ptr(ssn[2]),
+                                              hipabi.ptr(ssn[3]), hipabi.ptr(part), hipabi.stream_ptr()), 'straps_conv_dgrad_x3_bn_sc')
+    bn_next['bwd_partials'] = (part, nblk, dx)
+    return dx
+
+
 def encoder_backward(net, tape, dfeat, views=None, side_stream=None, after_layer3=None, want_dx=False, param_grads=True):
     L = hipabi.lib()
     grads = GradSink(views)
@@ -226,6 +260,8 @@
             rec = tape[id(pairs[-1][0])]
             ubits = rec.get('bits') if sink is not None else None
             dskip_bits = None
+            recd = tape[id(unit.downsample[0])] if unit.downsample is not None else None
+            fuse = recd is not None and _transition_fused(unit, tape[id(pairs[0][0])], recd, sink, prev_last)
             if ubits is not None:
                 draw, _ = _bn_bwd(L, rec, dy, True, False, grads, sink_of(rec), keep(rec))
                 dz = dy
@@ -234,11 +270,11 @@
             if param_grads:
                 side.run(lambda rec=rec, draw=draw: _conv_wgrad(L, rec, draw, grads, sink), draw)
             if unit.downsample is not None:
-                recd = tape[id(unit.downsample[0])]
-                drawd, _ = _bn_bwd(L, recd, dz, False, False, grads, sink_of(recd), keep(recd), mask_bits=ubits)
+                drawd, _ = _bn_bwd(L, recd, dz, False, False, grads, sink if fuse else sink_of(recd), keep(recd) or bool(recd.get('fmode')),
+                                   mask_bits=ubits)
                 if param_grads:
                     side.run(lambda recd=recd, drawd=drawd: _conv_wgrad(L, recd, drawd, grads, sink), drawd)
-                dskip = _conv_dgrad(L, net, recd, drawd, None, sink)
+                dskip = None if fuse else _conv_dgrad(L, net, recd, drawd, None, sink)
             else:
                 dskip, dskip_bits = dz, ubits
             for ci in range(len(pairs) - 1, 0, -1):
@@ -248,8 +284,11 @@
                 draw, _ = _bn_bwd(L, rec, dt, True, False, grads, sink_of(rec), keep(rec))
                 if param_grads:
                     side.run(lambda rec=rec, draw=draw: _conv_wgrad(L, rec, draw, grads, sink), draw)
-            dy = _conv_dgrad(L, net, tape[id(pairs[0][0])], draw, dskip, sink, bn_next=prev_last if sink is not None else None,
-                             addend_bits=dskip_bits)
+            if fuse:
+                dy = _conv_dgrad_sc(L, net, tape[id(pairs[0][0])], draw, recd, drawd, sink, prev_last)
+            else:
+                dy = _conv_dgrad(L, net, tape[id(pairs[0][0])], draw, dskip, sink, bn_next=prev_last if sink is not None else None,
+                                 addend_bits=dskip_bits)
         if li == 3 and after_layer3 is not None:
             side.join()
             after_layer3()
diff --git a/straps-3dhumanshapepose_amd/csrc/conv_igemm.h b/straps-3dhumanshapepose_amd/csrc/conv_igemm.h
--- a/straps-3dhumanshapepose_amd/csrc/conv_igemm.h
+++ b/straps-3dhumanshapepose_amd/csrc/conv_igemm.h
@@ -45,6 +45,9 @@
         int tap_w[9], tap_dh[9], tap_dw[9];
     } cls[4];
     int ncls;
+    const float* sc_x;
+    const float* sc_w;
+    long long sc_xps, sc_wps;
 };
 
 struct ClkSample { unsigned long long c0, w0; };
@@ -611,6 +614,13 @@
     template <bool PRE = true>
     __device__ __forceinline__ void finish(const ConvP& p, const ConvP::Class&, const f32x16 (&acc)[MI][NI], float (&)[NI], float (&)[NI], double (&d1)[NI],
                                            double (&d2)[NI]) {
+        finish_impl<false>(p, acc, acc, d1, d2);
+    }
+    __device__ __forceinline__ void finish_sc(const ConvP& p, const f32x16 (&acc)[MI][NI], const f32x16 (&asc)[MI][NI], double (&d1)[NI], double (&d2)[NI]) {
+        finish_impl<true>(p, acc, asc, d1, d2);
+    }
+    template <bool SC>
+    __device__ __forceinline__ void finish_impl(const ConvP& p, const f32x16 (&acc)[MI][NI], const f32x16 (&asc)[MI][NI], double (&d1)[NI], double (&d2)[NI]) {
         float bmu[NI], bsc[NI], bsh[NI];
 #pragma unroll
         for (int j = 0; j < NI; ++j) {
@@ -635,7 +645,7 @@
                 constexpr int r = decltype(rc)::value, rr = (r & 3) + 8 * (r >> 2);
                 const unsigned long long am = (unsigned long long)(unsigned)__builtin_amdgcn_readlane((int)un.aw, rr) |
                                               ((unsigned long long)(unsigned)__builtin_amdgcn_readlane((int)un.aw, rr + 4) << 32);
-                const float v = acc[i][j][r] + lane_masked(un.rv[r], am);
+                const float v = SC ? acc[i][j][r] + asc[i][j][r] : acc[i][j][r] + lane_masked(un.rv[r], am);
                 const bool ok = full || mrow + rr + half4 < M;
                 if (bnr) {
                     float gq;
@@ -774,6 +784,7 @@
     p.bnr_raw = p.bnr_out = p.bnr_sc = p.bnr_sh = p.bnr_mean = p.bnr_invstd = nullptr; p.bnr_part = nullptr; p.bnr_bits = p.res_bits = nullptr;
     p.yplanes = nullptr; p.yps = 0; p.clk = straps_clk_acc_current(); p.epi = STRAPS_TOOL_ENV_INT("STRAPS_EPI", 1);
     p.a_scale = p.a_shift = nullptr; p.a_relu = 0; p.abl = 0;
+    p.sc_x = p.sc_w = nullptr; p.sc_xps = p.sc_wps = 0;
     p.H = h; p.W = wdt; p.Cin = cin; p.Cout = cout; p.relu = relu; p.stride = stride;
     ConvP::Class& c = p.cls[0];
     p.ncls = 1;
@@ -800,6 +811,7 @@
     p.bnr_raw = p.bnr_out = p.bnr_sc = p.bnr_sh = p.bnr_mean = p.bnr_invstd = nullptr; p.bnr_part = nullptr; p.bnr_bits = p.res_bits = nullptr;
     p.yplanes = nullptr; p.yps = 0; p.clk = straps_clk_acc_current(); p.epi = STRAPS_TOOL_ENV_INT("STRAPS_EPI", 1);
     p.a_scale = p.a_shift = nullptr; p.a_relu = 0; p.abl = 0;
+    p.sc_x = p.sc_w = nullptr; p.sc_xps = p.sc_wps = 0;
     p.H = ho; p.W = wo; p.Cin = cout; p.Cout = cin; p.relu = 0; p.stride = 1;
     p.OH = h; p.OW = wdt; p.wtaps = kh * kw;
     p.omul = stride;
diff --git a/straps-3dhumanshapepose_amd/csrc/conv_x3.hip b/straps-3dhumanshapepose_amd/csrc/conv_x3.hip
--- a/straps-3dhumanshapepose_amd/csrc/conv_x3.hip
+++ b/straps-3dhumanshapepose_amd/csrc/conv_x3.hip
@@ -1,6 +1,7 @@
 #include "conv_x3_kernels.h"
 
 int straps_internal_dispatch_x3_lean(const void* p, int halo, int cfg, int epi, hipStream_t st);
+int straps_internal_dispatch_x3_sc(const void* p, int cfg, hipStream_t st);
 
 namespace {
 
@@ -265,6 +266,53 @@
                                  tile_cfg, bn_raw, bn_out, bn_out_bits, bn_mask_scale, bn_mask_shift, bn_mean, bn_invstd, bn_partials, stream);
 }
 
+extern "C" int straps_conv_dgrad_x3_bn_sc(const unsigned short* dy3, long long dy_plane_stride, const unsigned short* w3_crsk, long long w_plane_stride,
+                                          const unsigned short* sc_dy3, long long sc_dy_plane_stride, const unsigned short* sc_w3_crsk,
+                                          long long sc_w_plane_stride, float* dx, int batch, int h, int wdt, int cin, int cout, int tile_cfg,
+                                          const float* bn_raw, const unsigned* bn_out_bits, const float* bn_mask_scale, const float* bn_mask_shift,
+                                          const float* bn_mean, const float* bn_invstd, double* bn_partials, void* stream) {
+    STRAPS_REQUIRE(dy3 && w3_crsk && sc_dy3 && sc_w3_crsk && dx, "straps_conv_dgrad_x3_bn_sc: null pointer");
+    STRAPS_REQUIRE(bn_raw && bn_mean && bn_invstd && bn_partials && (bn_out_bits || (bn_mask_scale && bn_mask_shift)),
+                   "straps_conv_dgrad_x3_bn_sc: the BatchNorm tensors (raw, mean, invstd, partials, and the output's bits or mask scale / shift) are required");
+    STRAPS_REQUIRE(tile_cfg == 0, "straps_conv_dgrad_x3_bn_sc: automatic tiles only (tile_cfg = 0: the tiles of straps_conv_dgrad_x3_bn_blocks)");
+    STRAPS_REQUIRE(cout % 32 == 0 && cin % 64 == 0, "straps_conv_dgrad_x3_bn_sc: need cout%%32==0 and cin%%64==0 (cin=%d cout=%d)", cin, cout);
+    STRAPS_REQUIRE(h >= 2 && wdt >= 2, "straps_conv_dgrad_x3_bn_sc: the input needs all four parity classes (h=%d w=%d)", h, wdt);
+    STRAPS_REQUIRE(dy_plane_stride % 8 == 0 && w_plane_stride % 8 == 0 && sc_dy_plane_stride % 8 == 0 && sc_w_plane_stride % 8 == 0,
+                   "straps_conv_dgrad_x3_bn_sc: plane strides must be multiples of 8 elements");
+    ConvP p;
+    p.x = reinterpret_cast<const float*>(dy3); p.w = reinterpret_cast<const float*>(w3_crsk);
+    p.xps = dy_plane_stride; p.wps = w_plane_stride;
+    const int rc = conv_dgrad_problem(p, nullptr, dx, batch, h, wdt, cin, cout, 3, 3, 2, 1);
+    if (rc != STRAPS_OK) return rc;
+    STRAPS_REQUIRE(dy_plane_stride >= (long long)p.xrows * cout && sc_dy_plane_stride >= (long long)p.xrows * cout,
+                   "straps_conv_dgrad_x3_bn_sc: a plane stride is smaller than the gradient it holds");
+    {
+        bool found = false;
+        for (int i = 0; i < p.ncls; ++i) {
+            const ConvP::Class& c = p.cls[i];
+            STRAPS_REQUIRE(c.ntaps > 0, "straps_conv_dgrad_x3_bn_sc: a parity class without taps");
+            if (c.oah == 0 && c.oaw == 0) {
+                STRAPS_REQUIRE(c.ntaps == 1 && c.tap_dh[0] == 0 && c.tap_dw[0] == 0, "straps_conv_dgrad_x3_bn_sc: class (0, 0) is not the centre tap");
+                found = true;
+            }
+        }
+        STRAPS_REQUIRE(found && p.ncls == 4, "straps_conv_dgrad_x3_bn_sc: expected four parity classes");
+    }
+    p.bnr_raw = bn_raw; p.bnr_out = nullptr; p.bnr_sc = bn_mask_scale; p.bnr_sh = bn_mask_shift; p.bnr_mean = bn_mean; p.bnr_invstd = bn_invstd;
+    p.bnr_part = bn_partials; p.bnr_bits = bn_out_bits;
+    p.sc_x = reinterpret_cast<const float*>(sc_dy3); p.sc_w = reinterpret_cast<const float*>(sc_w3_crsk);
+    p.sc_xps = sc_dy_plane_stride; p.sc_wps = sc_w_plane_stride;
+    STRAPS_REQUIRE(lean_epilogue_choice(p) == 2, "straps_conv_dgrad_x3_bn_sc: the lean data-gradient epilogue does not cover these operands");
+    int bm, bn, kdim = 0;
+    long long M = 0;
+    for (int i = 0; i < p.ncls; ++i) {
+        M += p.cls[i].M;
+        if (p.cls[i].ntaps * p.Cin > kdim) kdim = p.cls[i].ntaps * p.Cin;
+    }
+    const int cfg = pick_tile_x3(0, M, p.Cout, kdim, bm, bn, p.ncls, kdim == p.Cin);
+    return straps_internal_dispatch_x3_sc(&p, cfg, (hipStream_t)stream);
+}
+
 extern "C" int straps_conv_x3_stat_blocks(int batch, int h, int w, int cin, int cout, int kh, int kw, int stride, int pad, int tile_cfg) {
     ConvP p;
     p.x = nullptr; p.w = nullptr; p.xps = p.wps = 0;
diff --git a/straps-3dhumanshapepose_amd/csrc/conv_x3_kernels.h b/straps-3dhumanshapepose_amd/csrc/conv_x3_kernels.h
--- a/straps-3dhumanshapepose_amd/csrc/conv_x3_kernels.h
+++ b/straps-3dhumanshapepose_amd/csrc/conv_x3_kernels.h
@@ -11,8 +11,9 @@
 
 __device__ __forceinline__ int swz3(int r) { return (r >> 3) & 3; }
 
-template <int BM, int BN, int WGM, int WGN, int NST, int ABL = 0, bool PIPE = false, int EPI = 0, int PL = 0>
-__global__ __launch_bounds__(64 * WGM * WGN) void conv_igemm_x3_kernel(ConvP p) {
+template <int BM, int BN, int WGM, int WGN, int NST, int ABL = 0, bool PIPE = false, int EPI = 0, int PL = 0, bool SC = false>
+__global__ __launch_bounds__(64 * WGM * WGN, SC ? 2 : 0) void conv_igemm_x3_kernel(ConvP p) {
+    static_assert(!SC || (EPI == 2 && PL == 0 && ABL == 0), "the shortcut segment exists for the lean data-gradient epilogue of the bf16x3 kernels");
     const ConvP::Class& c = p.cls[blockIdx.y];
     const int cMh = c.Mh, cMw = c.Mw, cM = c.M, cMT = c.MT, cntaps = c.ntaps;
     if ((int)blockIdx.x >= cMT * p.NT) return;
@@ -67,7 +68,9 @@
     for (int q = 0; q < BP; ++q) wrow[q] = wg + (n0 + lr + RPP * q) * 32 + lc * 8;
 
     const int cchunks = (p.Cin >> 5) / KD;
-    const int nchunks = cntaps * cchunks;
+    const bool has_sc = SC && c.oah == 0 && c.oaw == 0;
+    const int nchunks_sc = has_sc ? cchunks : 0;
+    const int nchunks = cntaps * cchunks + nchunks_sc;
     const int wave_u = __builtin_amdgcn_readfirstlane(wave);
     const int a_cstep = p.xrows * 32 * KD, b_cstep = p.Cout * 32 * KD;
 
@@ -75,12 +78,29 @@
     long long a_ps[AP];
     int a_inc[AP];
     const u16* b_src[BP];
+    long long b_ps = p.wps;
     int n_tap = 0, n_cc = 0;
     const int tl = lane < 9 ? lane : 0;
     const int v_dh = c.tap_dh[tl], v_dw = c.tap_dw[tl], v_tw = c.tap_w[tl];
     const u16* zsrc = reinterpret_cast<const u16*>(k_zero16_x3);
     asm volatile("" : "+s"(zsrc));
     auto setup_tap = [&](int tap) {
+        if constexpr (SC) {
+            b_ps = p.wps;
+            if (has_sc && tap-- == 0) {
+#pragma unroll
+                for (int i = 0; i < AP; ++i) {
+                    const bool ok = (unsigned)a_hi0[i] < (unsigned)p.H && (unsigned)a_wi0[i] < (unsigned)p.W;
+                    a_src[i] = ok ? reinterpret_cast<const u16*>(p.sc_x) + a_base[i] : zsrc;
+                    a_ps[i] = ok ? p.sc_xps : 0;
+                    a_inc[i] = ok ? a_cstep : 0;
+                }
+#pragma unroll
+                for (int i = 0; i < BP; ++i) b_src[i] = reinterpret_cast<const u16*>(p.sc_w) + (wrow[i] - wg);
+                b_ps = p.sc_wps;
+                return;
+            }
+        }
         const int dh = __builtin_amdgcn_readlane(v_dh, tap), dw = __builtin_amdgcn_readlane(v_dw, tap), tw = __builtin_amdgcn_readlane(v_tw, tap);
         const int toff = (dh * p.W + dw) * 32;
 #pragma unroll
@@ -101,7 +121,7 @@
             __builtin_amdgcn_global_load_lds((const __attribute__((address_space(1))) void*)(a_src[r] + plane * a_ps[r]),
                                              (__attribute__((address_space(3))) void*)(As + ((stage * NSB + plane) * BM + RPP * r + 16 * wave_u) * 32), 16, 0, 0);
         } else {
-            __builtin_amdgcn_global_load_lds((const __attribute__((address_space(1))) void*)(b_src[r - AP] + plane * p.wps),
+            __builtin_amdgcn_global_load_lds((const __attribute__((address_space(1))) void*)(b_src[r - AP] + plane * (SC ? b_ps : p.wps)),
                                              (__attribute__((address_space(3))) void*)(Bs + ((stage * NSB + plane) * BN + RPP * (r - AP) + 16 * wave_u) * 32), 16, 0, 0);
         }
     };
@@ -112,17 +132,33 @@
         for (int i = 0; i < BP; ++i) b_src[i] += b_cstep;
         if (++n_cc == cchunks) {
             n_cc = 0;
-            if (++n_tap < cntaps) setup_tap(n_tap);
+            if (++n_tap < cntaps + (nchunks_sc ? 1 : 0)) setup_tap(n_tap);
         }
     };
 
     f32x16 acc[MI][NI];
+    [[maybe_unused]] f32x16 acc_sc[MI][NI];
 #pragma unroll
     for (int i = 0; i < MI; ++i)
 #pragma unroll
         for (int j = 0; j < NI; ++j)
 #pragma unroll
-            for (int r = 0; r < 16; ++r) acc[i][j][r] = 0.f;
+            for (int r = 0; r < 16; ++r) {
+                acc[i][j][r] = 0.f;
+                if constexpr (SC) acc_sc[i][j][r] = 0.f;
+            }
+    [[maybe_unused]] auto sc_handover = [&]() {
+        if (!has_sc) return;
+#pragma unroll
+        for (int i = 0; i < MI; ++i)
+#pragma unroll
+            for (int j = 0; j < NI; ++j)
+#pragma unroll
+                for (int r = 0; r < 16; ++r) {
+                    acc_sc[i][j][r] = acc[i][j][r];
+                    acc[i][j][r] = 0.f;
+                }
+    };
 
     if (nchunks > 0) setup_tap(0);
 #pragma unroll
@@ -248,9 +284,20 @@
             stage = nxt;
         };
         int q = 0;
-        for (; q + NST < nchunks; ++q) body(q, std::true_type{}, std::false_type{});
-        for (; q + 1 < nchunks; ++q) body(q, std::false_type{}, std::false_type{});
-        if (q < nchunks) body(q, std::false_type{}, std::true_type{});
+        if constexpr (!SC) {
+            for (; q + NST < nchunks; ++q) body(q, std::true_type{}, std::false_type{});
+            for (; q + 1 < nchunks; ++q) body(q, std::false_type{}, std::false_type{});
+            if (q < nchunks) body(q, std::false_type{}, std::true_type{});
+        } else {
+            auto run = [&](int qend) {
+                for (; q < qend && q + NST < nchunks; ++q) body(q, std::true_type{}, std::false_type{});
+                for (; q < qend && q + 1 < nchunks; ++q) body(q, std::false_type{}, std::false_type{});
+                if (q < qend) { body(q, std::false_type{}, std::true_type{}); ++q; }
+            };
+            run(nchunks_sc);
+            sc_handover();
+            run(nchunks);
+        }
     } else {
     int stage = 0, nstage = NST - 1;
     auto next = [&]() {
@@ -258,11 +305,24 @@
         nstage = nstage + 1 == NST ? 0 : nstage + 1;
     };
     int q = 0;
+    if constexpr (!SC) {
     for (; q + NST - 1 < nchunks; ++q) { chunk(stage, nstage, std::true_type{}, std::integral_constant<int, (NST - 2) * NPIECE>{}, std::false_type{}); next(); }
     if constexpr (NST == 3) {
         if (q + 1 < nchunks) { chunk(stage, nstage, std::false_type{}, std::integral_constant<int, NPIECE>{}, std::false_type{}); next(); ++q; }
     }
     if (q < nchunks) chunk(stage, nstage, std::false_type{}, std::integral_constant<int, 0>{}, std::true_type{});
+    } else {
+    auto run = [&](int qend) {
+        for (; q < qend && q + NST - 1 < nchunks; ++q) { chunk(stage, nstage, std::true_type{}, std::integral_constant<int, (NST - 2) * NPIECE>{}, std::false_type{}); next(); }
+        if constexpr (NST == 3) {
+            if (q < qend && q + 1 < nchunks) { chunk(stage, nstage, std::false_type{}, std::integral_constant<int, NPIECE>{}, std::false_type{}); next(); ++q; }
+        }
+        if (q < qend) { chunk(stage, nstage, std::false_type{}, std::integral_constant<int, 0>{}, std::true_type{}); ++q; }
+    };
+    run(nchunks_sc);
+    sc_handover();
+    run(nchunks);
+    }
     }
 
     float s1[NI], s2[NI];
@@ -271,7 +331,8 @@
         lean_epilogue_fwd<BM, BN, WGM, WGN>(p, acc, m0, n0, c.M, s1, s2);
         igemm_store_stats<BM, BN, WGM, WGN>(p, s1, s2, mt, n0, smem);
     } else if constexpr (EPI == 2) {
-        ep.finish(p, c, acc, s1, s2, bd1, bd2);
+        if constexpr (SC) ep.finish_sc(p, acc, acc_sc, bd1, bd2);
+        else ep.finish(p, c, acc, s1, s2, bd1, bd2);
         igemm_store_bnr<BM, BN, WGM, WGN>(p, bd1, bd2, p.bnr_base[blockIdx.y] + mt, n0, smem);
     } else {
         ep.finish(p, c, acc, s1, s2, bd1, bd2);
@@ -512,7 +573,7 @@
     return (BM / p.W + 2) * (p.W + 2);
 }
 
-template <int BM, int BN, int WGM, int WGN, int NST, int ABL = 0, bool PIPE = false, int EPI = 0, int PL = 0>
+template <int BM, int BN, int WGM, int WGN, int NST, int ABL = 0, bool PIPE = false, int EPI = 0, int PL = 0, bool SC = false>
 int launch_x3(const ConvP& p0, hipStream_t st) {
     ConvP p = p0;
     p.NT = p.Cout / BN;
@@ -525,8 +586,8 @@
         base += p.cls[i].MT;
     }
     const size_t lds = (size_t)NST * (PL ? PL : 3) * (BM + BN) * 32 * sizeof(u16);
-    STRAPS_RAISE_LDS((conv_igemm_x3_kernel<BM, BN, WGM, WGN, NST, ABL, PIPE, EPI, PL>), lds, "conv_igemm_x3_kernel");
-    hipLaunchKernelGGL((conv_igemm_x3_kernel<BM, BN, WGM, WGN, NST, ABL, PIPE, EPI, PL>), dim3(maxblk, p.ncls), dim3(64 * WGM * WGN), lds, st, p);
+    STRAPS_RAISE_LDS((conv_igemm_x3_kernel<BM, BN, WGM, WGN, NST, ABL, PIPE, EPI, PL, SC>), lds, "conv_igemm_x3_kernel");
+    hipLaunchKernelGGL((conv_igemm_x3_kernel<BM, BN, WGM, WGN, NST, ABL, PIPE, EPI, PL, SC>), dim3(maxblk, p.ncls), dim3(64 * WGM * WGN), lds, st, p);
     STRAPS_CHECK_LAUNCH("conv_igemm_x3_kernel");
     return STRAPS_OK;
 }
diff --git a/straps-3dhumanshapepose_amd/csrc/conv_x3_sc.hip b/straps-3dhumanshapepose_amd/csrc/conv_x3_sc.hip
--- /dev/null
+++ b/straps-3dhumanshapepose_amd/csrc/conv_x3_sc.hip
@@ -0,0 +1,19 @@
+#include "conv_x3_kernels.h"
+
+namespace {
+
+int dispatch_sc(const ConvP& p, int cfg, hipStream_t st) {
+    switch (cfg) {
+        case 3: return launch_x3<64, 64, 2, 2, 3, 0, false, 2, 0, true>(p, st);
+        case 9: return launch_x3<128, 128, 4, 2, 3, 0, true, 2, 0, true>(p, st);
+        case 11: return launch_x3<128, 64, 2, 2, 2, 0, true, 2, 0, true>(p, st);
+        case 12: return launch_x3<256, 128, 4, 2, 2, 0, true, 2, 0, true>(p, st);
+        default: break;
+    }
+    straps_set_error("straps_conv_dgrad_x3_bn_sc: tile configuration %d has no shortcut instantiation", cfg);
+    return STRAPS_EUNSUPPORTED;
+}
+
+}
+
+int straps_internal_dispatch_x3_sc(const void* p, int cfg, hipStream_t st) { return dispatch_sc(*static_cast<const ConvP*>(p), cfg, st); }
diff --git a/straps-3dhumanshapepose_amd/csrc/regressor_train.hip b/straps-3dhumanshapepose_amd/csrc/regressor_train.hip
--- a/straps-3dhumanshapepose_amd/csrc/regressor_train.hip
+++ b/straps-3dhumanshapepose_amd/csrc/regressor_train.hip
@@ -40,6 +40,14 @@
 bool x3f_mode(const Plan& p, const Layer& cv) {
     if (!p.x3 || !straps_conv_x3f_supported(cv.cin, cv.cout, cv.k, cv.k, cv.stride, cv.pad)) return false;
     return (long long)p.B * cv.Ho * cv.Wo >= kX3fMinRows;
+}
+
+bool transition_fused(const Plan& p, const Unit& u, const Layer* prev_last) {
+    if (!p.x3 || !u.has_ds || !prev_last || !prev_last->last) return false;
+    const Layer& c0 = p.lay[u.c[0]];
+    const Layer& ds = p.lay[u.ds];
+    return c0.k == 3 && c0.stride == 2 && c0.pad == 1 && ds.k == 1 && ds.stride == 2 && ds.pad == 0 && c0.x == ds.x && c0.cin == ds.cin &&
+           c0.cout == ds.cout && c0.cin % 64 == 0 && c0.H >= 2 && c0.W >= 2;
 }
 
 void needs(const Plan& p, const Layer& cv, bool& f32, bool& planes) {
@@ -421,10 +429,11 @@
     int cur = 0;
     RG_CALL(straps_gap_bwd(dfeat, ws.f(p.g[cur]), B, p.geo.Hf * p.geo.Wf, F, stream));
 
-    auto bn_bwd = [&](const Layer& cv, const float* dy, bool masked, float* dz, const unsigned* mask_bits, size_t out_off, size_t out3_off) -> int {
+    auto bn_bwd = [&](const Layer& cv, const float* dy, bool masked, float* dz, const unsigned* mask_bits, size_t out_off, size_t out3_off,
+                      bool want_planes = false) -> int {
         const float* ss = ws.f(cv.ss);
         const int c = cv.cout;
-        const bool sink = x3 && !cv.fmode;
+        const bool sink = x3 && (!cv.fmode || want_planes);
         float* draw = (cv.keep_grad || !sink) ? ws.f(out_off) : nullptr;
         unsigned short* planes = sink ? ws.h(out3_off) : nullptr;
         const long long ps = sink ? round8(cv.rows * c) : 0;
@@ -531,12 +540,15 @@
         RG_CALL(wgrad(lc, p.draw, p.draw3));
         const float* dskip = dz;
         const unsigned* dskip_bits = nullptr;
+        const bool fuse = transition_fused(p, u, prev_last);
         if (u.has_ds) {
             const Layer& ds = p.lay[u.ds];
-            RG_CALL(bn_bwd(ds, dz, false, nullptr, ubits, p.drawd, p.drawd3));
+            RG_CALL(bn_bwd(ds, dz, false, nullptr, ubits, p.drawd, p.drawd3, fuse));
             RG_CALL(wgrad(ds, p.drawd, p.drawd3));
-            RG_CALL(dgrad(ds, p.drawd, p.drawd3, nullptr, nullptr, nullptr, ws.f(p.dskip)));
-            dskip = ws.f(p.dskip);
+            if (!fuse) {
+                RG_CALL(dgrad(ds, p.drawd, p.drawd3, nullptr, nullptr, nullptr, ws.f(p.dskip)));
+                dskip = ws.f(p.dskip);
+            }
         } else {
             dskip_bits = ubits;
         }
@@ -546,7 +558,20 @@
             RG_CALL(bn_bwd(prev, ws.f(p.dt), true, nullptr, nullptr, p.draw, p.draw3));
             RG_CALL(wgrad(prev, p.draw, p.draw3));
         }
-        RG_CALL(dgrad(p.lay[u.c[0]], p.draw, p.draw3, dskip, dskip_bits, x3 ? prev_last : nullptr, ws.f(p.g[cur ^ 1])));
+        if (fuse) {
+            const Layer& c0 = p.lay[u.c[0]];
+            const Layer& ds = p.lay[u.ds];
+            const float* ssn = ws.f(prev_last->ss);
+            const int cn = prev_last->cout;
+            const int nblk = straps_conv_dgrad_x3_bn_blocks(B, c0.H, c0.W, c0.cin, c0.cout, c0.k, c0.k, c0.stride, c0.pad, 0);
+            RG_CALL(straps_conv_dgrad_x3_bn_sc(ws.h(p.draw3), round8(c0.rows * c0.cout), crsk3 + c0.first, p.ps, ws.h(p.drawd3), round8(ds.rows * ds.cout),
+                                               crsk3 + ds.first, p.ps, ws.f(p.g[cur ^ 1]), B, c0.H, c0.W, c0.cin, c0.cout, 0, ws.f(prev_last->raw),
+                                               ws.u(prev_last->bitsb), nullptr, nullptr, ssn + 2 * cn, ssn + 3 * cn, part, stream));
+            pending = prev_last;
+            pending_nblk = nblk;
+        } else {
+            RG_CALL(dgrad(p.lay[u.c[0]], p.draw, p.draw3, dskip, dskip_bits, x3 ? prev_last : nullptr, ws.f(p.g[cur ^ 1])));
+        }
         cur ^= 1;
     }
 
diff --git a/straps-3dhumanshapepose_amd/hipabi.py b/straps-3dhumanshapepose_amd/hipabi.py
--- a/straps-3dhumanshapepose_amd/hipabi.py
+++ b/straps-3dhumanshapepose_amd/hipabi.py
@@ -6,7 +6,7 @@
 CSRC = os.path.join(_HERE, 'csrc')
 LIB_PATH = os.path.join(CSRC, 'libstraps_hip.so')
 HEADER = os.path.join(os.path.dirname(_HERE), 'include', 'straps_hip.h')
-SOURCES = ['abi.hip', 'augment.hip', 'pose.hip', 'ief.hip', 'elementwise.hip', 'conv.hip', 'conv_x3.hip', 'conv_x3_lean.hip', 'conv_bf16.hip', 'conv_x3f.hip', 'conv_wgrad_x3f.hip', 'stem.hip', 'stem_dgrad.hip', 'smpl.hip',
+SOURCES = ['abi.hip', 'augment.hip', 'pose.hip', 'ief.hip', 'elementwise.hip', 'conv.hip', 'conv_x3.hip', 'conv_x3_lean.hip', 'conv_x3_sc.hip', 'conv_bf16.hip', 'conv_x3f.hip', 'conv_wgrad_x3f.hip', 'stem.hip', 'stem_dgrad.hip', 'smpl.hip',
            'smpl_bwd.hip', 'backward.hip', 'train.hip', 'metrics.hip', 'image.hip', 'raster.hip', 'exchange.hip',
            'regressor.hip', 'regressor_train.hip']
 
@@ -172,6 +172,7 @@
     'straps_bn_bwd_finish_bits_x3': (_I, [_P] * 10 + [_L, _P, _I, _P, _L, _I, _I, _P]),
     'straps_conv_dgrad_x3_bits': (_I, [_P, _L, _P, _L, _P, _P, _I, _I, _I, _I, _I, _I, _I, _I, _I, _I, _P, _P]),
     'straps_conv_dgrad_x3_bn_bits': (_I, [_P, _L, _P, _L, _P, _P, _I, _I, _I, _I, _I, _I, _I, _I, _I, _I, _P, _P, _P, _P, _P, _P, _P, _P, _P, _P]),
+    'straps_conv_dgrad_x3_bn_sc': (_I, [_P, _L, _P, _L, _P, _L, _P, _L, _P, _I, _I, _I, _I, _I, _I, _P, _P, _P, _P, _P, _P, _P, _P]),
     'straps_conv_stat_blocks': (_I, [_I, _I, _I, _I, _I, _I]),
     'straps_conv_fwd': (_I, [_P, _P, _P, _P, _P, _I, _P, _P, _I, _I, _I, _I, _I, _I, _I, _I, _I, _I, _P]),
     'straps_maxpool_fwd': (_I, [_P, _P, _I, _I, _I, _I, _P]),
```

Result: no change. 8056, median of 6 (+0.7%).
